# gau-nernst/llama-x

Hardware: AMD Instinct MI355X
Metric: train tokens/sec Llama-3.1-8B seq4096 at 1/2/4/8 MI355X; p50 step ms (higher is better)
Workload: dtype bf16; 1 GPU; Llama-3.1-8B text-only LoRA r=16 bf16, seq=4096, 1 sequence per GPU, causal mask, base+LM head frozen (BASELINE.json configs[1]); random-init weights at 8B dimensions; seq_len=4096, parallelism=dp1, launch=hipGraph replay (fwd+bwd+AdamW), lm_head_rows=labelled only

## Files before the change

include/llx.h:

```cpp
#ifndef LLX_H
#define LLX_H

#include <stdint.h>

#ifdef __cplusplus
extern "C" {
#endif

typedef void* llx_stream_t;

int llx_version(void);
const char* llx_last_error_string(void);
int llx_device_info(int device, char* name, int len);

int llx_rmsnorm_fwd(const void* x, const void* w, void* y, float* rstd, int64_t rows, int64_t dim, float eps, llx_stream_t s);
int llx_rmsnorm_fwd_quant(const void* x, const void* w, void* y, float* rstd, void* q, int64_t ldq, void* qscale, int64_t rows, int64_t dim,
                          float eps, llx_stream_t s);
int64_t llx_rmsnorm_bwd_workspace_bytes(int64_t rows, int64_t dim);
int llx_rmsnorm_bwd(const void* dy, const void* x, const void* w, const float* rstd, void* dx, void* dw ,
                    int dw_accumulate, void* workspace, const void* dres ,
                    int64_t rows, int64_t dim, llx_stream_t s);

int llx_gemm_nt_bf16(const void* A, int64_t lda, const void* B, int64_t ldb, void* C, int64_t ldc, int64_t M, int64_t N, int64_t K,
                     const void* A2, int64_t lda2, const void* B2, int64_t ldb2, int64_t K2, int epilogue, const void* E, int64_t lde,
                     llx_stream_t s);
int llx_gemm_nt_bf16_rows(const void* A, int64_t lda, const void* B, int64_t ldb, void* C, int64_t ldc, int64_t M, int64_t N, int64_t K,
                          const void* A2, int64_t lda2, const void* B2, int64_t ldb2, int64_t K2, int epilogue, const void* E, int64_t lde,
                          const int32_t* m_valid, llx_stream_t s);
int llx_gemm_nt_bf16_splitk(const void* A, int64_t lda, const void* B, int64_t ldb, float* partial, int64_t M, int64_t N, int64_t K, int splits,
                            const int32_t* m_valid, llx_stream_t s);
int llx_splitk_combine(const float* partial, int splits, int64_t M, int64_t N, const int32_t* inv, const float* scale, void* out, int64_t ld_out,
                       llx_stream_t s);
int llx_gemm_nt_bf16_rope(const void* A, int64_t lda, const void* B, int64_t ldb, void* C, int64_t ldc, int64_t M, int64_t N, int64_t K,
                          const void* A2, int64_t lda2, const void* B2, int64_t ldb2, int64_t K2, const float* rope_table, int64_t rope_S,
                          int64_t rope_cols, llx_stream_t s);

int llx_gemm_tn_bf16(const void* A, int64_t lda, const void* B, int64_t ldb, void* C, int64_t ldc, int64_t M, int64_t N1, int64_t N2,
                     llx_stream_t s);
int llx_gemm_tn_bf16_rows(const void* A, int64_t lda, const void* B, int64_t ldb, void* C, int64_t ldc, int64_t M, int64_t N1, int64_t N2,
                          const int32_t* m_valid, llx_stream_t s);

int llx_int8_mm_dequant(const void* A, int64_t lda, const void* B, int64_t ldb, void* C, int64_t ldc, int64_t M, int64_t N, int64_t K,
                        const void* a_scale, const void* b_scale, llx_stream_t s);
int llx_int8_mm_dequant_f32(const void* A, int64_t lda, const void* B, int64_t ldb, float* C, int64_t ldc, int64_t M, int64_t N, int64_t K,
                            const float* a_scale, const float* b_scale, llx_stream_t s);
int llx_int8_mm_dequant_ext(const void* A, int64_t lda, const void* B, int64_t ldb, void* C, int64_t ldc, int64_t M, int64_t N, int64_t K,
                            const void* a_scale, const void* b_scale, const void* A2, int64_t lda2, const void* B2, int64_t ldb2, int64_t K2,
                            int epilogue, const void* E, int64_t lde, const float* rope_table, int64_t rope_S, int64_t rope_cols,
                            llx_stream_t s);

int llx_quantize_int8_rowwise(const void* x, int64_t ldx, void* q, int64_t ldq, void* scale, int64_t rows, int64_t cols, int is_f32,
                              llx_stream_t s);

int64_t llx_attn_flags_bytes(int64_t B, int64_t S);
int llx_attn_tile_flags(const int* doc_ids, const int* prefix_len, void* flags, int64_t B, int64_t S, llx_stream_t s);
int llx_attn_fwd(const void* q, int64_t q_sb, int64_t q_ss, const void* k, int64_t k_sb, int64_t k_ss, const void* v, int64_t v_sb,
                 int64_t v_ss, void* o, int64_t o_sb, int64_t o_ss, float* lse, const int* doc_ids, const int* prefix_len,
                 const void* flags, int64_t B, int64_t S, int64_t H, int64_t KVH, int64_t head_dim, float scale, llx_stream_t s);
int64_t llx_attn_bwd_workspace_bytes(int64_t B, int64_t S, int64_t H, int64_t KVH);
int64_t llx_attn_bwd_ds_bytes(int64_t B, int64_t S, int64_t H);
int llx_attn_bwd(const void* q, int64_t q_sb, int64_t q_ss, const void* k, int64_t k_sb, int64_t k_ss, const void* v, int64_t v_sb,
                 int64_t v_ss, const void* o, int64_t o_sb, int64_t o_ss, const void* d_o, int64_t do_sb, int64_t do_ss, const float* lse,
                 float* delta , void* dq, int64_t dq_sb, int64_t dq_ss, void* dk, int64_t dk_sb, int64_t dk_ss,
                 void* dv, int64_t dv_sb, int64_t dv_ss, const int* doc_ids, const int* prefix_len, const void* flags,
                 const float* rope ,
                 void* ds ,
                 int64_t B, int64_t S, int64_t H, int64_t KVH, int64_t head_dim, float scale, llx_stream_t s);

int llx_attn_dense_fwd(const void* q, int64_t q_sb, int64_t q_sh, int64_t q_ss, const void* k, int64_t k_sb, int64_t k_sh, int64_t k_ss,
                       const void* v, int64_t v_sb, int64_t v_sh, int64_t v_ss, void* o, int64_t o_sb, int64_t o_sh, int64_t o_ss,
                       const void* mask, int64_t m_sb, int64_t m_sh, int64_t m_sq, int64_t B, int64_t H, int64_t KVH, int64_t Sq, int64_t Skv,
                       int64_t head_dim, float scale, llx_stream_t s);

int llx_gemv_bf16(const void* w0, int64_t ldw0, int64_t n0, const void* w1, int64_t ldw1, int64_t n1, const void* w2, int64_t ldw2, int64_t n2,
                  const void* x, int64_t ldx, int64_t M, int64_t K, const void* norm_w, float eps, int epilogue, void* out, int64_t ldo,
                  const void* res, int64_t ldr, const float* rope, int64_t n_q, int64_t n_k, void* k_cache, void* v_cache, int64_t c_sh,
                  int64_t c_ss, const int64_t* input_pos, const void* bext0, const void* bext1, const void* bext2, int64_t rank0, int64_t rank1,
                  int64_t rank2, const void* t, int64_t ldt, float lora_scale, llx_stream_t s);
int llx_mask_extent(const void* mask, int64_t row_stride, int64_t rows, int64_t Skv, int* extent, llx_stream_t s);
int llx_kv_scatter(const void* k, const void* v, int64_t s_sb, int64_t s_sh, int64_t s_ss, void* k_cache, void* v_cache, int64_t c_sb, int64_t c_sh,
                   int64_t c_ss, const int64_t* input_pos, int64_t B, int64_t KVH, int64_t L, int64_t Smax, int64_t head_dim, llx_stream_t s);
int64_t llx_attn_decode_workspace_bytes(int64_t B, int64_t H, int64_t M, int64_t nsplit);
int llx_attn_decode(const void* q, int64_t q_sb, int64_t q_sh, int64_t q_ss, const void* k_cache, const void* v_cache, int64_t c_sb, int64_t c_sh,
                    int64_t c_ss, void* o, int64_t o_sb, int64_t o_sh, int64_t o_ss, const void* mask, int64_t m_sb, int64_t m_sh, int64_t m_sq,
                    const int* extent, float* workspace, int64_t B, int64_t H, int64_t KVH, int64_t M, int64_t Skv, int64_t nsplit,
                    int64_t head_dim, float scale, llx_stream_t s);

int llx_rope(const void* x, int64_t x_sb, int64_t x_ss, void* y, int64_t y_sb, int64_t y_ss, const float* table, int64_t B, int64_t S,
             int64_t nheads, int64_t head_dim, int backward, llx_stream_t s);

int llx_swiglu_fwd(const void* g, int64_t g_ld, const void* u, int64_t u_ld, void* h, int64_t h_ld, int64_t rows, int64_t cols, llx_stream_t s);
int llx_swiglu_bwd(const void* dh, int64_t dh_ld, const void* g, int64_t g_ld, const void* u, int64_t u_ld, void* dg, int64_t dg_ld,
                   void* du, int64_t du_ld, int64_t rows, int64_t cols, llx_stream_t s);

int llx_embedding_fwd(const int64_t* ids, const void* table, void* out, int64_t n_tok, int64_t dim, int64_t vocab, int64_t tok_per_batch,
                      int64_t out_sb, int64_t out_ss, llx_stream_t s);
int llx_embedding_bwd(const int64_t* ids, const void* dy, float* dtable_f32, int64_t n_tok, int64_t dim, int64_t vocab,
                      int64_t tok_per_batch, int64_t dy_sb, int64_t dy_ss, llx_stream_t s);

int64_t llx_ce_workspace_bytes(int64_t T);
int llx_ce_fwd_bwd(const void* logits, int64_t ld, void* dlogits, int64_t dld, const int64_t* labels, float* loss, void* workspace,
                   int64_t T, int64_t V, llx_stream_t s);
int llx_head_compact_index(const int64_t* labels, int32_t* idx, int32_t* inv, int64_t* labels_c, int32_t* count, int64_t T, llx_stream_t s);
int llx_gather_rows(const void* src, int64_t ld_src, const int32_t* idx, const int32_t* count, void* dst, int64_t ld_dst, int64_t T, int64_t D,
                    llx_stream_t s);
int llx_scatter_rows(const void* src, int64_t ld_src, const int32_t* inv, const float* scale , void* dst, int64_t ld_dst,
                     int64_t T, int64_t D, llx_stream_t s);
int llx_ce_fwd_bwd_rows(const void* logits, int64_t ld, void* dlogits, int64_t dld, const int64_t* labels, float* loss, void* workspace,
                        int64_t T, int64_t V, const int32_t* rows, llx_stream_t s);
int llx_ce_fwd_bwd_part(const void* logits, int64_t ld, void* dlogits, int64_t dld, const int64_t* labels, float* loss, void* workspace, int64_t T,
                        int64_t V, int64_t row0, int64_t nrows, const int32_t* rows, int phase, llx_stream_t s);

int llx_skinny_nt(const void* X, int64_t ldx, const void* W, int64_t ldw, void* out, int64_t M, int64_t K, int64_t R,
                  const int32_t* kranges , llx_stream_t s);
int llx_skinny_nt_scaled(const void* X, int64_t ldx, const void* W, int64_t ldw, void* out, int64_t M, int64_t K, int64_t R,
                         const int32_t* kranges, const void* colscale, void* G, int64_t ldg, llx_stream_t s);
int llx_rmsnorm_skinny_nt(const void* x, const void* g, const void* W, int64_t ldw, void* y, float* rstd, void* t, int64_t M, int64_t D,
                          int64_t R, float eps, llx_stream_t s);
int64_t llx_skinny_tn_workspace_bytes(int64_t M, int64_t N, int64_t R);
int llx_skinny_tn(const void* U, const void* Y, int64_t ldy, void* out, int64_t out_ld, int64_t M, int64_t N, int64_t R, float scale,
                  int transpose_out, int accumulate, void* workspace,
                  const int32_t* segs , int seg_count, llx_stream_t s);
int llx_skinny_tn_partial(const void* U, const void* Y, int64_t ldy, int64_t M, int64_t N, int64_t R, void* workspace, const int32_t* segs,
                          int seg_count, llx_stream_t s);
int llx_skinny_tn_partial_many(int n, const void* const* U, const void* const* Y, const int64_t* ldy, const int64_t* M, const int64_t* N,
                               const int64_t* R, void* const* workspaces, const int32_t* const* segs, const int* seg_count, llx_stream_t s);
int64_t llx_skinny_u_workspace_bytes(int64_t M, int64_t N);
int llx_skinny_tn_partial_many_u(int n, const void* const* U, const void* const* Y, const int64_t* ldy, const int64_t* M, const int64_t* N,
                                 const int64_t* R, void* const* workspaces, const int32_t* const* segs, const int* seg_count,
                                 const void* const* Bt, const int64_t* ldb, void* const* upart, llx_stream_t s);
int llx_skinny_u_reduce(const void* upart, void* out, int64_t M, int64_t N, int64_t R, const int32_t* segs, int seg_count, llx_stream_t s);
int llx_skinny_tn_partial_many_us(int n, const void* const* U, const void* const* Y, const int64_t* ldy, const int64_t* M, const int64_t* N,
                                  const int64_t* R, void* const* workspaces, const int32_t* const* segs, const int* seg_count,
                                  const void* const* Bt, const int64_t* ldb, void* const* upart, const void* const* colscale,
                                  void* const* G, const int64_t* ldg, llx_stream_t s);
int llx_skinny_tn_reduce_many(int n, const void* const* workspaces, void* const* outs, const int64_t* out_ld, const int64_t* M, const int64_t* N,
                              const int64_t* R, const float* scale, const int* transpose_out, const int* accumulate,
                              const int32_t* const* segs, const int* seg_count, llx_stream_t s);
int llx_pad64(const void* in, int64_t ld, void* out, int64_t R, int64_t C, float scale, int transpose, llx_stream_t s);
int llx_lora_group_pack(const void* const* lora_a, const void* const* lora_b, const int64_t* Ns, const int64_t* ranks, int nm, int64_t K,
                        float scale, void* a_cat, void* b2, void* bT, void* a2t, llx_stream_t s);
int llx_lora_groups_pack(const void* const* lora_a, const void* const* lora_b, const int64_t* Ns, const int64_t* ranks, const int* nm,
                         const int64_t* K, const float* scale, void* const* a_cat, void* const* b2, void* const* bT, void* const* a2t, int ng,
                         llx_stream_t s);
int llx_lora_pack(const void* in, int64_t ld, void* out, int64_t out_ld, int64_t R, int64_t C, int64_t row_off, int64_t col_off, float scale,
                  int transpose, llx_stream_t s);

int llx_rownorm2(const void* W, int64_t ld, float* out, int64_t rows, int64_t cols, llx_stream_t s);
int llx_dora_colscale(const float* wn2, const void* G , const void* b2 , const void* AAt ,
                      const void* m , void* c , float* inv_norm , int64_t N, int64_t R, llx_stream_t s);
int64_t llx_colsum_mul_workspace_bytes(int64_t N);
int llx_colsum_mul(const void* a, int64_t lda, const void* b, int64_t ldb, const float* colscale , void* out ,
                   void* workspace, int64_t M, int64_t N, llx_stream_t s);
int llx_colscale_bias(const void* x, int64_t x_ld, void* y, int64_t y_ld, const void* colscale , const void* bias ,
                      int64_t rows, int64_t cols, llx_stream_t s);

int llx_mel_spectrogram(const float* audio, int64_t B, int64_t L, const float* twiddle, const float* window, const float* fbank, float* mel,
                        int64_t n_frames, int64_t hop, int64_t n_mels, llx_stream_t s);
int llx_logmel_cmn(const float* mel, void* feat , int64_t B, int64_t n_frames, int64_t n_mels, llx_stream_t s);
int llx_gelu_fwd(const void* z, int64_t z_ld, void* y, int64_t y_ld, int64_t rows, int64_t cols, llx_stream_t s);
int llx_gelu_bwd(const void* dy, int64_t dy_ld, const void* z, int64_t z_ld, void* dz, int64_t dz_ld, int64_t rows, int64_t cols, llx_stream_t s);
int llx_col2im3(const void* dA, void* dpad, int64_t M, int64_t C, int64_t P, int64_t stride, llx_stream_t s);
int llx_conv_w_reorder(const void* in, void* out, int64_t D, int64_t C, int to_gemm, llx_stream_t s);

int llx_scale(const void* x, int64_t x_ld, void* y, int64_t y_ld, const float* dev_scalar, float host_scale, const void* colscale,
              int64_t rows, int64_t cols, llx_stream_t s);
int llx_add(const void* x, const void* y, void* z, int64_t n, llx_stream_t s);
int llx_transpose(const void* in, int64_t in_ld, void* out, int64_t out_ld, int64_t R, int64_t C, int src_is_i8, llx_stream_t s);
int llx_i8_to_bf16(const void* in, void* out, int64_t n, llx_stream_t s);

#ifdef __cplusplus
}
#endif
#endif
```

llama-x_amd/csrc/common.h:

```cpp
#pragma once
#include <hip/hip_runtime.h>
#include <stdint.h>
#include <stdarg.h>
#include <stdio.h>

#define LLX_OK 0
#define LLX_ERR_ARG -1
#define LLX_ERR_LAUNCH -2
#define LLX_ERR_UNSUPPORTED -3

void llx_set_error(const char* fmt, ...);

#define LLX_REQUIRE(cond, ...)            \
  do {                                    \
    if (!(cond)) {                        \
      llx_set_error(__VA_ARGS__);         \
      return LLX_ERR_ARG;                 \
    }                                     \
  } while (0)

#define LLX_LAUNCH_CHECK(name)                                              \
  do {                                                                      \
    hipError_t e__ = hipGetLastError();                                     \
    if (e__ != hipSuccess) {                                                \
      llx_set_error("%s: launch failed: %s", name, hipGetErrorString(e__)); \
      return LLX_ERR_LAUNCH;                                                \
    }                                                                       \
  } while (0)

typedef uint16_t bf16_t;

typedef __attribute__((ext_vector_type(8))) __bf16 bf16x8_t;
typedef __attribute__((ext_vector_type(4))) float f32x4_t;
typedef __attribute__((ext_vector_type(16))) float f32x16_t;
typedef __attribute__((ext_vector_type(4))) int i32x4_t;
typedef __attribute__((ext_vector_type(16))) int i32x16_t;
typedef __attribute__((ext_vector_type(4))) short s16x4_t;
typedef __attribute__((ext_vector_type(4))) uint32_t u32x4_t;
typedef __attribute__((ext_vector_type(2))) uint32_t u32x2_t;

#define LLX_WAVE 64

__device__ __forceinline__ float bf2f(bf16_t v) { return __uint_as_float(((uint32_t)v) << 16); }
__device__ __forceinline__ bf16_t f2bf(float f) {
  __bf16 b = (__bf16)f;
  return __builtin_bit_cast(bf16_t, b);
}
__device__ __forceinline__ uint32_t pack_bf2(float lo, float hi) {
  return (uint32_t)f2bf(lo) | ((uint32_t)f2bf(hi) << 16);
}
__device__ __forceinline__ float bflo(uint32_t w) { return __uint_as_float(w << 16); }
__device__ __forceinline__ float bfhi(uint32_t w) { return __uint_as_float(w & 0xffff0000u); }

__device__ __forceinline__ float wave_sum(float v) {
#pragma unroll
  for (int o = 32; o > 0; o >>= 1) v += __shfl_xor(v, o, 64);
  return v;
}
__device__ __forceinline__ float wave_max(float v) {
#pragma unroll
  for (int o = 32; o > 0; o >>= 1) v = fmaxf(v, __shfl_xor(v, o, 64));
  return v;
}

__device__ __forceinline__ float block_sum(float v, float* red) {
  v = wave_sum(v);
  const int lane = threadIdx.x & 63, w = threadIdx.x >> 6, nw = (blockDim.x + 63) >> 6;
  __syncthreads();
  if (lane == 0) red[w] = v;
  __syncthreads();
  float t = 0.f;
  for (int i = 0; i < nw; ++i) t += red[i];
  return t;
}
__device__ __forceinline__ float block_max(float v, float* red) {
  v = wave_max(v);
  const int lane = threadIdx.x & 63, w = threadIdx.x >> 6, nw = (blockDim.x + 63) >> 6;
  __syncthreads();
  if (lane == 0) red[w] = v;
  __syncthreads();
  float t = red[0];
  for (int i = 1; i < nw; ++i) t = fmaxf(t, red[i]);
  return t;
}

static inline int64_t cdiv64(int64_t a, int64_t b) { return (a + b - 1) / b; }

__device__ __forceinline__ float sigmoidf_(float x) { return __builtin_amdgcn_rcpf(1.f + __expf(-x)); }
__device__ __forceinline__ u32x4_t swiglu_fwd8(const u32x4_t& gv, const u32x4_t& uv) {
  u32x4_t o;
#pragma unroll
  for (int e = 0; e < 4; ++e) {
    const float g0 = bflo(gv[e]), g1 = bfhi(gv[e]);
    const float s0 = bf2f(f2bf(g0 * sigmoidf_(g0))), s1 = bf2f(f2bf(g1 * sigmoidf_(g1)));
    o[e] = pack_bf2(s0 * bflo(uv[e]), s1 * bfhi(uv[e]));
  }
  return o;
}
__device__ __forceinline__ void swiglu_bwd8(const u32x4_t& dv, const u32x4_t& gv, const u32x4_t& uv, u32x4_t& og, u32x4_t& ou) {
#pragma unroll
  for (int e = 0; e < 4; ++e) {
    float dgs[2], dus[2];
#pragma unroll
    for (int p = 0; p < 2; ++p) {
      const float gg = p ? bfhi(gv[e]) : bflo(gv[e]);
      const float uu = p ? bfhi(uv[e]) : bflo(uv[e]);
      const float dd = p ? bfhi(dv[e]) : bflo(dv[e]);
      const float sg = sigmoidf_(gg);
      const float silu = bf2f(f2bf(gg * sg));
      dus[p] = dd * silu;
      const float ds = bf2f(f2bf(dd * uu));
      dgs[p] = ds * (sg * (1.f + gg * (1.f - sg)));
    }
    og[e] = pack_bf2(dgs[0], dgs[1]);
    ou[e] = pack_bf2(dus[0], dus[1]);
  }
}

__device__ __forceinline__ u32x4_t rope8(const u32x4_t& v, const f32x4_t& t0, const f32x4_t& t1, float sign) {
  const float cs[4] = {t0[0], t0[2], t1[0], t1[2]};
  const float sn[4] = {t0[1] * sign, t0[3] * sign, t1[1] * sign, t1[3] * sign};
  u32x4_t o;
#pragma unroll
  for (int e = 0; e < 4; ++e) {
    const float x0 = bflo(v[e]), x1 = bfhi(v[e]);
    o[e] = pack_bf2(x0 * cs[e] - x1 * sn[e], x1 * cs[e] + x0 * sn[e]);
  }
  return o;
}

__device__ __forceinline__ u32x4_t rope8(const u32x4_t& v, const float* __restrict__ tp, float sign) {
  const f32x4_t t0 = *reinterpret_cast<const f32x4_t*>(tp);
  const f32x4_t t1 = *reinterpret_cast<const f32x4_t*>(tp + 4);
  const float cs[4] = {t0[0], t0[2], t1[0], t1[2]};
  const float sn[4] = {t0[1] * sign, t0[3] * sign, t1[1] * sign, t1[3] * sign};
  u32x4_t o;
#pragma unroll
  for (int e = 0; e < 4; ++e) {
    const float x0 = bflo(v[e]), x1 = bfhi(v[e]);
    o[e] = pack_bf2(x0 * cs[e] - x1 * sn[e], x1 * cs[e] + x0 * sn[e]);
  }
  return o;
}

typedef __attribute__((ext_vector_type(8))) short llx_s16x8_t;
template <int OFF>
__device__ __forceinline__ void lds_tr_read(s16x4_t& dst, uint32_t addr) {
  asm volatile("ds_read_b64_tr_b16 %0, %1 offset:%2" : "=v"(dst) : "v"(addr), "n"(OFF));
}
__device__ __forceinline__ void lds_tr_read_rt(s16x4_t& dst, uint32_t addr, int off) {
  asm volatile("ds_read_b64_tr_b16 %0, %1 offset:%2" : "=v"(dst) : "v"(addr), "n"(off));
}
template <int N>
__device__ __forceinline__ void lds_tr_wait4(s16x4_t& a, s16x4_t& b, s16x4_t& c, s16x4_t& d) {
  asm volatile("s_waitcnt lgkmcnt(%4)" : "+v"(a), "+v"(b), "+v"(c), "+v"(d) : "n"(N));
  __builtin_amdgcn_sched_barrier(0);
}
template <int N>
__device__ __forceinline__ void lds_tr_wait8(s16x4_t (&c)[4], s16x4_t (&d)[4]) {
  asm volatile("s_waitcnt lgkmcnt(%8)" : "+v"(c[0]), "+v"(c[1]), "+v"(c[2]), "+v"(c[3]), "+v"(d[0]), "+v"(d[1]), "+v"(d[2]), "+v"(d[3]) : "n"(N));
  __builtin_amdgcn_sched_barrier(0);
}
__device__ __forceinline__ bf16x8_t frag_of(const s16x4_t& lo, const s16x4_t& hi) {
  const llx_s16x8_t v = {lo[0], lo[1], lo[2], lo[3], hi[0], hi[1], hi[2], hi[3]};
  return __builtin_bit_cast(bf16x8_t, v);
}
```

llama-x_amd/csrc/rmsnorm.hip:

```cpp
#include "common.h"

template <int NCH, bool QUANT = false, bool FULL = false>
__global__ __launch_bounds__(256) void rmsnorm_fwd_kernel(const bf16_t* __restrict__ x, const bf16_t* __restrict__ w,
                                                          bf16_t* __restrict__ y, float* __restrict__ rstd_out,
                                                          int64_t rows, int dim, float eps, int8_t* __restrict__ q = nullptr,
                                                          int64_t ldq = 0, bf16_t* __restrict__ qscale = nullptr) {
  const int lane = threadIdx.x & 63;
  const int64_t row = (int64_t)blockIdx.x * 4 + (threadIdx.x >> 6);
  if (row >= rows) return;
  const bf16_t* xr = x + row * dim;
  u32x4_t v[NCH];
  float ss = 0.f;
#pragma unroll
  for (int c = 0; c < NCH; ++c) {
    const int col = c * 512 + lane * 8;
    if (FULL || col < dim) {
      v[c] = *reinterpret_cast<const u32x4_t*>(xr + col);
#pragma unroll
      for (int e = 0; e < 4; ++e) {
        float a = bflo(v[c][e]), b = bfhi(v[c][e]);
        ss += a * a + b * b;
      }
    }
  }
// ... 8 lines not shown
    if (FULL || col < dim) {
      u32x4_t wv = *reinterpret_cast<const u32x4_t*>(w + col);
      u32x4_t o;
#pragma unroll
      for (int e = 0; e < 4; ++e) {
        float a = bflo(v[c][e]) * rstd * bflo(wv[e]);
        float b = bfhi(v[c][e]) * rstd * bfhi(wv[e]);
        o[e] = pack_bf2(a, b);
        if constexpr (QUANT) amax = fmaxf(amax, fmaxf(fabsf(bflo(o[e])), fabsf(bfhi(o[e]))));
      }
      *reinterpret_cast<u32x4_t*>(yr + col) = o;
      if constexpr (QUANT) v[c] = o;
    }
  }
  if constexpr (QUANT) {
    amax = wave_max(amax);
    const float scale = amax / 127.0f;
    const float div = fmaxf(scale, 1e-12f);
    if (lane == 0) qscale[row] = f2bf(scale);
    int8_t* qr = q + row * ldq;
#pragma unroll
    for (int c = 0; c < NCH; ++c) {
      const int col = c * 512 + lane * 8;
      if (FULL || col < dim) {
        u32x2_t o = {0u, 0u};
#pragma unroll
        for (int e = 0; e < 4; ++e) {
          const int a = (int)rintf(bflo(v[c][e]) / div), b = (int)rintf(bfhi(v[c][e]) / div);
          o[e >> 1] |= ((uint32_t)(a & 0xff) | ((uint32_t)(b & 0xff) << 8)) << ((e & 1) * 16);
        }
        *reinterpret_cast<u32x2_t*>(qr + col) = o;
      }
    }
  }
}

template <int NCH, bool FULL = false, int RES = -1>
__global__ __launch_bounds__(256) void rmsnorm_bwd_kernel(const bf16_t* __restrict__ dy, const bf16_t* __restrict__ x,
                                                          const bf16_t* __restrict__ w, const float* __restrict__ rstd,
                                                          bf16_t* __restrict__ dx, float* __restrict__ dw_partial,
                                                          const bf16_t* __restrict__ dres, int64_t rows, int dim, int rows_per_block) {
  extern __shared__ __attribute__((aligned(16))) float dwsh[];
  const bool has_res = RES < 0 ? dres != nullptr : RES == 1;
  const int lane = threadIdx.x & 63, wave = threadIdx.x >> 6;
  u32x4_t wp[NCH];
  float dwacc[NCH][8];
#pragma unroll
  for (int c = 0; c < NCH; ++c) {
    const int col = c * 512 + lane * 8;
#pragma unroll
    for (int e = 0; e < 8; ++e) dwacc[c][e] = 0.f;
    wp[c] = u32x4_t{0u, 0u, 0u, 0u};
    if (FULL || col < dim) wp[c] = *reinterpret_cast<const u32x4_t*>(w + col);
  }
  const int64_t r0 = (int64_t)blockIdx.x * rows_per_block;
  const int64_t r_end = (r0 + rows_per_block < rows) ? r0 + rows_per_block : rows;
  constexpr bool PIPE = NCH <= 8;
  struct RowRegs { u32x4_t x[NCH], d[NCH], r[NCH]; float rs; };
  auto load_row = [&](RowRegs& R, int64_t row) {
    R.rs = rstd[row];
#pragma unroll
    for (int c = 0; c < NCH; ++c) {
      const int col = c * 512 + lane * 8;
      if (FULL || col < dim) {
        R.x[c] = *reinterpret_cast<const u32x4_t*>(x + row * dim + col);
        R.d[c] = *reinterpret_cast<const u32x4_t*>(dy + row * dim + col);
        if (has_res) R.r[c] = *reinterpret_cast<const u32x4_t*>(dres + row * dim + col);
      }
    }
  };
  auto process_row = [&](RowRegs& R, int64_t row) {
    const float rs = R.rs;
    float dot = 0.f;
#pragma unroll
    for (int c = 0; c < NCH; ++c) {
      const int col = c * 512 + lane * 8;
      if (FULL || col < dim) {
#pragma unroll
        for (int e = 0; e < 4; ++e) {
          const float x0 = bflo(R.x[c][e]) * rs, x1 = bfhi(R.x[c][e]) * rs;
          const float d0 = bflo(R.d[c][e]), d1 = bfhi(R.d[c][e]);
          dwacc[c][2 * e] += d0 * x0; dwacc[c][2 * e + 1] += d1 * x1;
          dot += d0 * bflo(wp[c][e]) * x0 + d1 * bfhi(wp[c][e]) * x1;
        }
      }
    }
    dot = wave_sum(dot);
    const float m = dot / (float)dim;
#pragma unroll
    for (int c = 0; c < NCH; ++c) {
      const int col = c * 512 + lane * 8;
      if (FULL || col < dim) {
        u32x4_t o;
        asm volatile("" : "+v"(R.x[c]), "+v"(R.d[c]));
#pragma unroll
        for (int e = 0; e < 4; ++e) {
          const float x0 = bflo(R.x[c][e]) * rs, x1 = bfhi(R.x[c][e]) * rs;
          float a = rs * (bflo(R.d[c][e]) * bflo(wp[c][e]) - x0 * m);
          float b = rs * (bfhi(R.d[c][e]) * bfhi(wp[c][e]) - x1 * m);
          if (has_res) {
            a = bf2f(f2bf(a)) + bflo(R.r[c][e]);
            b = bf2f(f2bf(b)) + bfhi(R.r[c][e]);
          }
          o[e] = pack_bf2(a, b);
        }
        *reinterpret_cast<u32x4_t*>(dx + row * dim + col) = o;
      }
    }
  };
  {
    RowRegs A;
    int64_t row = r0 + wave;
    if constexpr (PIPE) {
      RowRegs B;
      if (row < r_end) load_row(A, row);
      while (row < r_end) {
        const bool n1 = row + 4 < r_end;
        if (n1) load_row(B, row + 4);
        process_row(A, row);
        if (!n1) break;
        row += 4;
        const bool n2 = row + 4 < r_end;
        if (n2) load_row(A, row + 4);
        process_row(B, row);
        if (!n2) break;
        row += 4;
      }
    } else {
      for (; row < r_end; row += 4) { load_row(A, row); process_row(A, row); }
    }
  }
  if (dw_partial) {
    for (int wsel = 0; wsel < 4; ++wsel) {
      if (wave == wsel) {
#pragma unroll
        for (int c = 0; c < NCH; ++c) {
          const int col = c * 512 + lane * 8;
          if (FULL || col < dim) {
#pragma unroll
            for (int e = 0; e < 8; ++e) dwsh[col + e] = (wsel == 0 ? 0.f : dwsh[col + e]) + dwacc[c][e];
          }
        }
      }
      __syncthreads();
    }
    for (int col = threadIdx.x * 4; col < dim; col += 256 * 4)
      *reinterpret_cast<f32x4_t*>(dw_partial + (int64_t)blockIdx.x * dim + col) = *reinterpret_cast<const f32x4_t*>(dwsh + col);
  }
}

__global__ __launch_bounds__(256) void colsum_partials_kernel(const float* __restrict__ partial, bf16_t* __restrict__ out, int nparts, int dim,
                                                              int accumulate) {
  __shared__ float red[16][17];
  const int c = threadIdx.x & 15, grp = threadIdx.x >> 4;
  const int col = blockIdx.x * 16 + c;
  float s = 0.f;
  if (col < dim)
    for (int p = grp; p < nparts; p += 16) s += partial[(int64_t)p * dim + col];
  red[grp][c] = s;
  __syncthreads();
  if (grp == 0 && col < dim) {
    s = 0.f;
#pragma unroll
    for (int g = 0; g < 16; ++g) s += red[g][c];
    if (accumulate) s += bf2f(out[col]);
    out[col] = f2bf(s);
  }
}

extern "C" int llx_rmsnorm_fwd(const void* x, const void* w, void* y, float* rstd, int64_t rows, int64_t dim, float eps,
                               hipStream_t stream) {
  LLX_REQUIRE(x && w && y, "llx_rmsnorm_fwd: null pointer");
  LLX_REQUIRE(rows >= 0 && dim > 0 && dim % 8 == 0 && dim <= 8192, "llx_rmsnorm_fwd: dim=%lld must be a multiple of 8 and <= 8192",
              (long long)dim);
  if (rows == 0) return LLX_OK;
  const dim3 grid((unsigned)cdiv64(rows, 4)), block(256);
  const int nch = (int)cdiv64(dim, 512);
#define L(N) hipLaunchKernelGGL((rmsnorm_fwd_kernel<N, false>), grid, block, 0, stream, (const bf16_t*)x, (const bf16_t*)w, (bf16_t*)y, rstd, rows, (int)dim, eps, (int8_t*)nullptr, (int64_t)0, (bf16_t*)nullptr)
#define LF(N) hipLaunchKernelGGL((rmsnorm_fwd_kernel<N, false, true>), grid, block, 0, stream, (const bf16_t*)x, (const bf16_t*)w, (bf16_t*)y, rstd, rows, (int)dim, eps, (int8_t*)nullptr, (int64_t)0, (bf16_t*)nullptr)
  if (dim == 4096) LF(8); else if (dim == 2048) LF(4); else if (dim == 8192) LF(16);
  else if (nch <= 1) L(1); else if (nch <= 2) L(2); else if (nch <= 4) L(4); else if (nch <= 8) L(8); else L(16);
#undef LF
#undef L
  LLX_LAUNCH_CHECK("llx_rmsnorm_fwd");
  return LLX_OK;
}

extern "C" int llx_rmsnorm_fwd_quant(const void* x, const void* w, void* y, float* rstd, void* q, int64_t ldq, void* qscale, int64_t rows,
                                     int64_t dim, float eps, hipStream_t stream) {
  LLX_REQUIRE(x && w && y && q && qscale, "llx_rmsnorm_fwd_quant: null pointer");
  LLX_REQUIRE(rows >= 0 && dim > 0 && dim % 8 == 0 && dim <= 8192 && ldq % 8 == 0 && (uintptr_t)q % 8 == 0,
              "llx_rmsnorm_fwd_quant: dim=%lld must be a multiple of 8 and <= 8192, q rows 8-byte aligned", (long long)dim);
  if (rows == 0) return LLX_OK;
  const dim3 grid((unsigned)cdiv64(rows, 4)), block(256);
  const int nch = (int)cdiv64(dim, 512);
#define L(N) hipLaunchKernelGGL((rmsnorm_fwd_kernel<N, true>), grid, block, 0, stream, (const bf16_t*)x, (const bf16_t*)w, (bf16_t*)y, rstd, rows, (int)dim, eps, (int8_t*)q, ldq, (bf16_t*)qscale)
#define LF(N) hipLaunchKernelGGL((rmsnorm_fwd_kernel<N, true, true>), grid, block, 0, stream, (const bf16_t*)x, (const bf16_t*)w, (bf16_t*)y, rstd, rows, (int)dim, eps, (int8_t*)q, ldq, (bf16_t*)qscale)
  if (dim == 4096) LF(8); else if (dim == 2048) LF(4); else if (dim == 8192) LF(16);
  else if (nch <= 1) L(1); else if (nch <= 2) L(2); else if (nch <= 4) L(4); else if (nch <= 8) L(8); else L(16);
#undef LF
#undef L
  LLX_LAUNCH_CHECK("llx_rmsnorm_fwd_quant");
  return LLX_OK;
}

#ifndef RMS_BWD_RPB
#define RMS_BWD_RPB 16
#endif
extern "C" int64_t llx_rmsnorm_bwd_workspace_bytes(int64_t rows, int64_t dim) {
  const int64_t rpb = RMS_BWD_RPB;
  return cdiv64(rows, rpb) * dim * 4;
}

extern "C" int llx_rmsnorm_bwd(const void* dy, const void* x, const void* w, const float* rstd, void* dx, void* dw,
                               int dw_accumulate, void* workspace, const void* dres, int64_t rows, int64_t dim, hipStream_t stream) {
  LLX_REQUIRE(dy && x && w && rstd && dx, "llx_rmsnorm_bwd: null pointer");
  LLX_REQUIRE(dim > 0 && dim % 8 == 0 && dim <= 8192, "llx_rmsnorm_bwd: dim=%lld must be a multiple of 8 and <= 8192", (long long)dim);
  LLX_REQUIRE(!dw || workspace, "llx_rmsnorm_bwd: workspace required when dw is requested");
  if (rows == 0) return LLX_OK;
  const int rpb = RMS_BWD_RPB;
  const int nblk = (int)cdiv64(rows, rpb);
  const int nch = (int)cdiv64(dim, 512);
  float* part = dw ? (float*)workspace : nullptr;
  const size_t lds = dw ? (size_t)dim * 4 : 0;
#define L(N) hipLaunchKernelGGL(rmsnorm_bwd_kernel<N>, dim3(nblk), dim3(256), lds, stream, (const bf16_t*)dy, (const bf16_t*)x, (const bf16_t*)w, rstd, (bf16_t*)dx, part, (const bf16_t*)dres, rows, (int)dim, rpb)
#define LF(N) if (dres) LFR(N, 1); else LFR(N, 0)
#define LFR(N, R) hipLaunchKernelGGL((rmsnorm_bwd_kernel<N, true, R>), dim3(nblk), dim3(256), lds, stream, (const bf16_t*)dy, (const bf16_t*)x, (const bf16_t*)w, rstd, (bf16_t*)dx, part, (const bf16_t*)dres, rows, (int)dim, rpb)
  if (dim == 4096) { LF(8); } else if (dim == 2048) { LF(4); } else if (dim == 8192) { LF(16); }
  else if (nch <= 1) L(1); else if (nch <= 2) L(2); else if (nch <= 4) L(4); else if (nch <= 8) L(8); else L(16);
#undef LFR
#undef LF
#undef L
  LLX_LAUNCH_CHECK("llx_rmsnorm_bwd");
  if (dw) {
    hipLaunchKernelGGL(colsum_partials_kernel, dim3((unsigned)cdiv64(dim, 16)), dim3(256), 0, stream, part, (bf16_t*)dw, nblk,
                       (int)dim, dw_accumulate);
    LLX_LAUNCH_CHECK("llx_rmsnorm_bwd(colsum)");
  }
  return LLX_OK;
}
```

llama-x_amd/csrc/skinny.hip:

```cpp
#include "common.h"

typedef __attribute__((address_space(3))) s16x4_t lds_s16x4;
typedef __attribute__((ext_vector_type(8))) short s16x8_t;

#define SK_PAD 64

#define SNT_WAVES 8
#define SNT_UNROLL 8

struct SkinnyRanges { int lo[4], hi[4]; };

__device__ __forceinline__ void snt_scaled_store(const bf16x8_t& a, const bf16_t* cs, bf16_t* g) {
  const u32x4_t x = __builtin_bit_cast(u32x4_t, a);
  const u32x4_t c = *reinterpret_cast<const u32x4_t*>(cs);
  u32x4_t o;
#pragma unroll
  for (int e = 0; e < 4; ++e) o[e] = pack_bf2(bflo(x[e]) * bflo(c[e]), bfhi(x[e]) * bfhi(c[e]));
  *reinterpret_cast<u32x4_t*>(g) = o;
}

template <int NB, bool RANGED, bool SCALE = false>
__global__ __launch_bounds__(SNT_WAVES * 64) void skinny_nt_kernel(const bf16_t* __restrict__ X, int64_t ldx, const bf16_t* __restrict__ W,
                                                                   int64_t ldw, bf16_t* __restrict__ out, int M, int K, int R, SkinnyRanges kr,
                                                                   const bf16_t* __restrict__ cs = nullptr, bf16_t* __restrict__ G = nullptr,
// ... 101 lines not shown
  else { if (nb == 1) L(1, false); else if (nb == 2) L(2, false); else L(4, false); }
#undef L
  LLX_LAUNCH_CHECK("llx_skinny_nt");
  return LLX_OK;
}

extern "C" int llx_skinny_nt_scaled(const void* X, int64_t ldx, const void* W, int64_t ldw, void* out, int64_t M, int64_t K, int64_t R,
                                    const int32_t* kranges, const void* colscale, void* G, int64_t ldg, hipStream_t stream) {
  LLX_REQUIRE(X && W && out && colscale && G, "llx_skinny_nt_scaled: null pointer");
  LLX_REQUIRE(M > 0 && K > 0 && K % 32 == 0 && R > 0 && R <= 64, "llx_skinny_nt_scaled: need K%%32==0 and 0<R<=64 (K=%lld R=%lld)", (long long)K, (long long)R);
  LLX_REQUIRE(ldx % 8 == 0 && ldw % 8 == 0 && ldg % 8 == 0 && ((uintptr_t)X | (uintptr_t)W | (uintptr_t)colscale | (uintptr_t)G) % 16 == 0 && (uintptr_t)out % 8 == 0,
              "llx_skinny_nt_scaled: alignment");
  const dim3 grid((unsigned)cdiv64(M, 16)), block(SNT_WAVES * 64);
  const int nb = (int)cdiv64(R, 16);
  SkinnyRanges kr;
  for (int i = 0; i < 4; ++i) {
    kr.lo[i] = kranges ? kranges[2 * i] : 0;
    kr.hi[i] = kranges ? kranges[2 * i + 1] : (int)K;
    LLX_REQUIRE(kr.lo[i] % 64 == 0 && (kr.hi[i] % 64 == 0 || kr.hi[i] == (int)K) && kr.lo[i] >= 0 && kr.hi[i] <= (int)K,
                "llx_skinny_nt_scaled: k range %d of a block-diagonal W must be a multiple of 64 inside [0, K]", i);
  }
#define L(N, RG) hipLaunchKernelGGL((skinny_nt_kernel<N, RG, true>), grid, block, 0, stream, (const bf16_t*)X, ldx, (const bf16_t*)W, ldw, (bf16_t*)out, (int)M, (int)K, (int)R, kr, (const bf16_t*)colscale, (bf16_t*)G, ldg)
  if (kranges) { if (nb == 1) L(1, true); else if (nb == 2) L(2, true); else L(4, true); }
  else { if (nb == 1) L(1, false); else if (nb == 2) L(2, false); else L(4, false); }
#undef L
  LLX_LAUNCH_CHECK("llx_skinny_nt_scaled");
  return LLX_OK;
}

#define TN_NT 256
#define TN_MS 32
#define TN_YROW (TN_NT * 2 + 16)
#define TN_UROW (SK_PAD * 2 + 16)

__device__ __forceinline__ bf16x8_t tr16_frag(const char* tile, int rowbytes, int c0, int lane) {
  const int g = lane >> 4, i = lane & 15, q = i >> 2, p = i & 3;
  const char* base = tile + (8 * g + q) * rowbytes + (c0 + 4 * p) * 2;
  s16x4_t lo = __builtin_amdgcn_ds_read_tr16_b64_v4i16((lds_s16x4*)base);
  s16x4_t hi = __builtin_amdgcn_ds_read_tr16_b64_v4i16((lds_s16x4*)(base + 4 * rowbytes));
  s16x8_t v = {lo[0], lo[1], lo[2], lo[3], hi[0], hi[1], hi[2], hi[3]};
  return __builtin_bit_cast(bf16x8_t, v);
}

struct TnSegs { int n_lo[4], n_hi[4], r_lo[4], r_hi[4]; int64_t off[4]; int count; int rb_lo[4], rb_hi[4]; };

template <int NB>
__device__ __forceinline__ void skinny_tn_block(const bf16_t* __restrict__ U, const bf16_t* __restrict__ Y, int64_t ldy, float* __restrict__ partial,
                                                int M, int N, int rows_per_split, const TnSegs& sg, int ctile, int split, int nbl, char* sY, char* sU,
                                                const bf16_t* __restrict__ Bt = nullptr, int64_t ldb = 0, float* __restrict__ upart = nullptr, int brows = 0,
                                                const bf16_t* __restrict__ cs = nullptr, bf16_t* __restrict__ G = nullptr, int64_t ldg = 0) {
  const int tid = threadIdx.x, lane = tid & 63;
  const int wave = __builtin_amdgcn_readfirstlane(tid >> 6);
  const int n0 = ctile * TN_NT;
  const int m_begin = split * rows_per_split, m_end = min(M, m_begin + rows_per_split);
  const bool u_on = upart != nullptr && wave < nbl && n0 + TN_NT > sg.rb_lo[wave] && n0 < sg.rb_hi[wave];
  bf16x8_t ub[8];
  if (u_on) {
    const bf16_t* brow = Bt + (int64_t)min(wave * 16 + (lane & 15), brows - 1) * ldb;
#pragma unroll
    for (int ks = 0; ks < 8; ++ks) ub[ks] = *reinterpret_cast<const bf16x8_t*>(brow + min(n0 + ks * 32 + 8 * (lane >> 4), N - 8));
  }
  f32x4_t acc[NB][4];
#pragma unroll
  for (int rb = 0; rb < NB; ++rb)
#pragma unroll
    for (int cb = 0; cb < 4; ++cb) acc[rb][cb] = f32x4_t{0.f, 0.f, 0.f, 0.f};

  u32x4_t yv[2][4], uv[2];
  auto load_step = [&](int set, int ms) {
#pragma unroll
    for (int i = 0; i < 4; ++i) {
      const int q = i * 256 + tid;
      const int row = ms + (q >> 5), col = n0 + (q & 31) * 8;
      yv[set][i] = (row < m_end && col < N) ? *reinterpret_cast<const u32x4_t*>(Y + (int64_t)row * ldy + col) : u32x4_t{0u, 0u, 0u, 0u};
    }
    const int row = ms + (tid >> 3);
    uv[set] = (row < m_end) ? *reinterpret_cast<const u32x4_t*>(U + (int64_t)row * SK_PAD + (tid & 7) * 8) : u32x4_t{0u, 0u, 0u, 0u};
  };
  auto step = [&](int set, int ms) {
    __syncthreads();
#pragma unroll
    for (int i = 0; i < 4; ++i) {
      const int q = i * 256 + tid;
      *reinterpret_cast<u32x4_t*>(sY + (q >> 5) * TN_YROW + (q & 31) * 16) = yv[set][i];
      if (G) {
        const int row = ms + (q >> 5), col = n0 + (q & 31) * 8;
        if (row < m_end && col < N) {
          const u32x4_t c = *reinterpret_cast<const u32x4_t*>(cs + col);
          u32x4_t o;
#pragma unroll
          for (int e = 0; e < 4; ++e) o[e] = pack_bf2(bflo(yv[set][i][e]) * bflo(c[e]), bfhi(yv[set][i][e]) * bfhi(c[e]));
          *reinterpret_cast<u32x4_t*>(G + (int64_t)row * ldg + col) = o;
        }
      }
    }
    *reinterpret_cast<u32x4_t*>(sU + (tid >> 3) * TN_UROW + (tid & 7) * 16) = uv[set];
    __syncthreads();
    if (ms + 2 * TN_MS < m_end) load_step(set, ms + 2 * TN_MS);
    bf16x8_t a[NB];
#pragma unroll
    for (int rb = 0; rb < NB; ++rb) a[rb] = tr16_frag(sU, TN_UROW, rb * 16, lane);
#pragma unroll
    for (int cb = 0; cb < 4; ++cb) {
      const bf16x8_t b = tr16_frag(sY, TN_YROW, wave * 64 + cb * 16, lane);
#pragma unroll
      for (int rb = 0; rb < NB; ++rb)
        if (n0 + TN_NT > sg.rb_lo[rb] && n0 < sg.rb_hi[rb]) acc[rb][cb] = __builtin_amdgcn_mfma_f32_16x16x32_bf16(a[rb], b, acc[rb][cb], 0, 0, 0);
    }
    if (u_on) {
#pragma unroll
      for (int rf = 0; rf < 2; ++rf) {
        f32x4_t ua0 = {0.f, 0.f, 0.f, 0.f}, ua1 = {0.f, 0.f, 0.f, 0.f};
        const char* yrow = sY + (rf * 16 + (lane & 15)) * TN_YROW + (lane >> 4) * 16;
#pragma unroll
        for (int ks = 0; ks < 8; ks += 2) {
          ua0 = __builtin_amdgcn_mfma_f32_16x16x32_bf16(ub[ks], *reinterpret_cast<const bf16x8_t*>(yrow + ks * 64), ua0, 0, 0, 0);
          ua1 = __builtin_amdgcn_mfma_f32_16x16x32_bf16(ub[ks + 1], *reinterpret_cast<const bf16x8_t*>(yrow + (ks + 1) * 64), ua1, 0, 0, 0);
        }
        const int row = ms + rf * 16 + (lane & 15);
        if (row < m_end) {
#pragma unroll
          for (int e = 0; e < 4; ++e) upart[((int64_t)ctile * SK_PAD + wave * 16 + (lane >> 4) * 4 + e) * M + row] = ua0[e] + ua1[e];
        }
      }
    }
  };
  if (m_begin < m_end) load_step(0, m_begin);
  if (m_begin + TN_MS < m_end) load_step(1, m_begin + TN_MS);
  for (int ms = m_begin; ms < m_end; ms += 2 * TN_MS) {
    step(0, ms);
    if (ms + TN_MS < m_end) step(1, ms + TN_MS);
  }
  const int fr = lane & 15, fq = lane >> 4;
#pragma unroll
  for (int rb = 0; rb < NB; ++rb)
#pragma unroll
    for (int cb = 0; cb < 4; ++cb) {
      const int n = n0 + wave * 64 + cb * 16 + fr;
      if (n < N && n0 + TN_NT > sg.rb_lo[rb] && n0 < sg.rb_hi[rb]) {
#pragma unroll
        for (int e = 0; e < 4; ++e) partial[((int64_t)split * (nbl * 16) + rb * 16 + fq * 4 + e) * N + n] = acc[rb][cb][e];
      }
    }
}

template <int NB>
__global__ __launch_bounds__(256) void skinny_tn_kernel(const bf16_t* __restrict__ U, const bf16_t* __restrict__ Y, int64_t ldy,
                                                        float* __restrict__ partial, int M, int N, int rows_per_split, TnSegs sg) {
  __shared__ __attribute__((aligned(16))) char sY[TN_MS * TN_YROW];
  __shared__ __attribute__((aligned(16))) char sU[TN_MS * TN_UROW];
  skinny_tn_block<NB>(U, Y, ldy, partial, M, N, rows_per_split, sg, blockIdx.x, blockIdx.y, NB, sY, sU);
}

#define TN_MANY 4
struct TnPart { const bf16_t* U; const bf16_t* Y; int64_t ldy; float* partial; int M, N, rows_per_split, ctiles, nblocks, nbl; TnSegs sg;
                const bf16_t* Bt; int64_t ldb; float* upart; int brows; const bf16_t* cs; bf16_t* G; int64_t ldg; };
struct TnPartMany { TnPart d[TN_MANY]; int n; };

template <int NB>
__global__ __launch_bounds__(256) void skinny_tn_many_kernel(const TnPartMany m) {
  __shared__ __attribute__((aligned(16))) char sY[TN_MS * TN_YROW];
  __shared__ __attribute__((aligned(16))) char sU[TN_MS * TN_UROW];
  int b = blockIdx.x, i = 0;
  while (i < m.n - 1 && b >= m.d[i].nblocks) { b -= m.d[i].nblocks; ++i; }
  const TnPart& d = m.d[i];
  skinny_tn_block<NB>(d.U, d.Y, d.ldy, d.partial, d.M, d.N, d.rows_per_split, d.sg, b % d.ctiles, b / d.ctiles, d.nbl, sY, sU, d.Bt, d.ldb, d.upart, d.brows, d.cs, d.G, d.ldg);
}


static int tn_splits(int64_t M, int64_t N) {
  const int64_t ntiles = cdiv64(N, TN_NT);
  constexpr int target = 384;
  int64_t want = cdiv64(target, ntiles);
  const int64_t max_split = cdiv64(M, 4 * TN_MS);
  if (want > max_split) want = max_split;
  if (want < 1) want = 1;
  return (int)want;
}

extern "C" int64_t llx_skinny_tn_workspace_bytes(int64_t M, int64_t N, int64_t R) {
  return (int64_t)tn_splits(M, N) * cdiv64(R, 16) * 16 * N * 4;
}

static int tn_fill_segs(TnSegs& sg, const int32_t* segs, int seg_count, int64_t N, int64_t R, int64_t* total_out) {
  sg.count = 0;
  for (int rb = 0; rb < 4; ++rb) { sg.rb_lo[rb] = 0; sg.rb_hi[rb] = (int)N; }
  int64_t total = 0;
  if (segs) {
    LLX_REQUIRE(seg_count >= 1 && seg_count <= 4, "llx_skinny_tn: 1..4 segments");
    for (int rb = 0; rb < 4; ++rb) { sg.rb_lo[rb] = (int)N; sg.rb_hi[rb] = 0; }
    for (int i = 0; i < seg_count; ++i) {
      sg.n_lo[i] = segs[4 * i]; sg.n_hi[i] = segs[4 * i + 1]; sg.r_lo[i] = segs[4 * i + 2]; sg.r_hi[i] = segs[4 * i + 3];
      LLX_REQUIRE(sg.n_lo[i] >= 0 && sg.n_lo[i] < sg.n_hi[i] && sg.n_hi[i] <= N && sg.r_lo[i] >= 0 && sg.r_lo[i] < sg.r_hi[i] && sg.r_hi[i] <= R,
                  "llx_skinny_tn: bad segment %d", i);
      LLX_REQUIRE(sg.n_lo[i] % TN_NT == 0 && (sg.n_hi[i] % TN_NT == 0 || sg.n_hi[i] == N), "llx_skinny_tn: segment %d: n bounds must be multiples of 256", i);
      sg.off[i] = total;
      total += (int64_t)(sg.n_hi[i] - sg.n_lo[i]) * (sg.r_hi[i] - sg.r_lo[i]);
      for (int rb = sg.r_lo[i] / 16; rb <= (sg.r_hi[i] - 1) / 16; ++rb) {
        if (sg.n_lo[i] < sg.rb_lo[rb]) sg.rb_lo[rb] = sg.n_lo[i];
        if (sg.n_hi[i] > sg.rb_hi[rb]) sg.rb_hi[rb] = sg.n_hi[i];
      }
    }
    sg.count = seg_count;
  }
  *total_out = total;
  return LLX_OK;
}

extern "C" int llx_skinny_tn_partial(const void* U, const void* Y, int64_t ldy, int64_t M, int64_t N, int64_t R, void* workspace,
                                     const int32_t* segs, int seg_count, hipStream_t stream) {
  LLX_REQUIRE(U && Y && workspace, "llx_skinny_tn: null pointer");
  LLX_REQUIRE(M > 0 && N > 0 && N % 8 == 0 && R > 0 && R <= 64 && ldy % 8 == 0, "llx_skinny_tn: need N%%8==0, ldy%%8==0, 0<R<=64");
  LLX_REQUIRE(((uintptr_t)U | (uintptr_t)Y) % 16 == 0, "llx_skinny_tn: unaligned pointer");
  const int nsplit = tn_splits(M, N);
  int rows_per_split = (int)cdiv64(cdiv64(M, nsplit), TN_MS) * TN_MS;
  const int nb = (int)cdiv64(R, 16);
  TnSegs sg;
  int64_t total = 0;
  const int rc = tn_fill_segs(sg, segs, seg_count, N, R, &total);
  if (rc != LLX_OK) return rc;
  const dim3 grid((unsigned)cdiv64(N, TN_NT), (unsigned)nsplit), block(256);
#define L(NBV) hipLaunchKernelGGL(skinny_tn_kernel<NBV>, grid, block, 0, stream, (const bf16_t*)U, (const bf16_t*)Y, ldy, (float*)workspace, (int)M, (int)N, rows_per_split, sg)
  if (nb == 1) L(1); else if (nb == 2) L(2); else if (nb == 3) L(3); else L(4);
#undef L
  LLX_LAUNCH_CHECK("llx_skinny_tn");
  return LLX_OK;
}

extern "C" int llx_skinny_tn_partial_many_u(int n, const void* const* U, const void* const* Y, const int64_t* ldy, const int64_t* M, const int64_t* N,
                                            const int64_t* R, void* const* workspaces, const int32_t* const* segs, const int* seg_count,
                                            const void* const* Bt, const int64_t* ldb, void* const* upart, hipStream_t stream);
extern "C" int llx_skinny_tn_partial_many(int n, const void* const* U, const void* const* Y, const int64_t* ldy, const int64_t* M, const int64_t* N,
                                          const int64_t* R, void* const* workspaces, const int32_t* const* segs, const int* seg_count,
                                          hipStream_t stream) {
  return llx_skinny_tn_partial_many_u(n, U, Y, ldy, M, N, R, workspaces, segs, seg_count, nullptr, nullptr, nullptr, stream);
}
extern "C" int64_t llx_skinny_u_workspace_bytes(int64_t M, int64_t N) { return cdiv64(N, TN_NT) * M * SK_PAD * 4; }
extern "C" int llx_skinny_tn_partial_many_us(int n, const void* const* U, const void* const* Y, const int64_t* ldy, const int64_t* M, const int64_t* N,
                                             const int64_t* R, void* const* workspaces, const int32_t* const* segs, const int* seg_count,
                                             const void* const* Bt, const int64_t* ldb, void* const* upart, const void* const* colscale,
                                             void* const* G, const int64_t* ldg, hipStream_t stream);
extern "C" int llx_skinny_tn_partial_many_u(int n, const void* const* U, const void* const* Y, const int64_t* ldy, const int64_t* M, const int64_t* N,
                                            const int64_t* R, void* const* workspaces, const int32_t* const* segs, const int* seg_count,
                                            const void* const* Bt, const int64_t* ldb, void* const* upart, hipStream_t stream) {
  return llx_skinny_tn_partial_many_us(n, U, Y, ldy, M, N, R, workspaces, segs, seg_count, Bt, ldb, upart, nullptr, nullptr, nullptr, stream);
}
extern "C" int llx_skinny_tn_partial_many_us(int n, const void* const* U, const void* const* Y, const int64_t* ldy, const int64_t* M, const int64_t* N,
                                             const int64_t* R, void* const* workspaces, const int32_t* const* segs, const int* seg_count,
                                             const void* const* Bt, const int64_t* ldb, void* const* upart, const void* const* colscale,
                                             void* const* G, const int64_t* ldg, hipStream_t stream) {
  LLX_REQUIRE(n >= 1 && n <= TN_MANY && U && Y && ldy && M && N && R && workspaces && segs && seg_count, "llx_skinny_tn_partial_many: bad arguments (1..4 products)");
  TnPartMany m;
  m.n = n;
  int total_blocks = 0;
  for (int i = 0; i < n; ++i) {
    TnPart& d = m.d[i];
    LLX_REQUIRE(U[i] && Y[i] && workspaces[i], "llx_skinny_tn_partial_many: null pointer (product %d)", i);
    LLX_REQUIRE(M[i] > 0 && N[i] > 0 && N[i] % 8 == 0 && R[i] > 0 && R[i] <= 64 && ldy[i] % 8 == 0, "llx_skinny_tn_partial_many: need N%%8==0, ldy%%8==0, 0<R<=64 (product %d)", i);
    LLX_REQUIRE(((uintptr_t)U[i] | (uintptr_t)Y[i]) % 16 == 0, "llx_skinny_tn_partial_many: unaligned pointer (product %d)", i);
    const int nsplit = tn_splits(M[i], N[i]);
    d.U = (const bf16_t*)U[i]; d.Y = (const bf16_t*)Y[i]; d.ldy = ldy[i]; d.partial = (float*)workspaces[i];
    d.M = (int)M[i]; d.N = (int)N[i];
    d.rows_per_split = (int)cdiv64(cdiv64(M[i], nsplit), TN_MS) * TN_MS;
    d.ctiles = (int)cdiv64(N[i], TN_NT);
    d.nblocks = d.ctiles * nsplit;
    d.nbl = (int)cdiv64(R[i], 16);
    int64_t total = 0;
    const int rc = tn_fill_segs(d.sg, segs[i], seg_count[i], N[i], R[i], &total);
    if (rc != LLX_OK) return rc;
    for (int rb = d.nbl; rb < 4; ++rb) { d.sg.rb_lo[rb] = d.N; d.sg.rb_hi[rb] = 0; }
    d.Bt = nullptr; d.ldb = 0; d.upart = nullptr; d.brows = (int)R[i];
    if (upart && upart[i]) {
      LLX_REQUIRE(Bt && ldb && Bt[i] && ldb[i] % 8 == 0 && (uintptr_t)Bt[i] % 16 == 0 && N[i] >= 8, "llx_skinny_tn_partial_many_u: Bt of product %d", i);
      d.Bt = (const bf16_t*)Bt[i]; d.ldb = ldb[i]; d.upart = (float*)upart[i];
    }
    d.cs = nullptr; d.G = nullptr; d.ldg = 0;
    if (G && G[i]) {
      LLX_REQUIRE(colscale && ldg && colscale[i] && ldg[i] % 8 == 0 && ((uintptr_t)colscale[i] | (uintptr_t)G[i]) % 16 == 0, "llx_skinny_tn_partial_many_us: scaled copy of product %d", i);
      d.cs = (const bf16_t*)colscale[i]; d.G = (bf16_t*)G[i]; d.ldg = ldg[i];
    }
    total_blocks += d.nblocks;
  }
  int nbmax = 1;
  for (int i = 0; i < n; ++i) nbmax = m.d[i].nbl > nbmax ? m.d[i].nbl : nbmax;
  const dim3 grid((unsigned)total_blocks), block(256);
  if (nbmax == 1) hipLaunchKernelGGL(skinny_tn_many_kernel<1>, grid, block, 0, stream, m);
  else if (nbmax == 2) hipLaunchKernelGGL(skinny_tn_many_kernel<2>, grid, block, 0, stream, m);
  else if (nbmax == 3) hipLaunchKernelGGL(skinny_tn_many_kernel<3>, grid, block, 0, stream, m);
  else hipLaunchKernelGGL(skinny_tn_many_kernel<4>, grid, block, 0, stream, m);
  LLX_LAUNCH_CHECK("llx_skinny_tn_partial_many");
  return LLX_OK;
}

__global__ __launch_bounds__(256) void skinny_u_reduce_kernel(const float* __restrict__ upart, bf16_t* __restrict__ out, int M, int R, TnSegs sg) {
  __shared__ float tile[4][65];
  const int m0 = blockIdx.x * 64, ml = threadIdx.x & 63, cl = threadIdx.x >> 6;
  const int c = blockIdx.y * 4 + cl;
  float sum = 0.f;
  if (c < R) {
    const int rb = c >> 4;
    const int t_lo = sg.rb_lo[rb] / TN_NT, t_hi = (sg.rb_hi[rb] + TN_NT - 1) / TN_NT;
    const int64_t stride = (int64_t)SK_PAD * M;
    const float* src = upart + (int64_t)c * M + min(m0 + ml, M - 1);
    int t = t_lo;
    for (; t + 8 <= t_hi; t += 8) {
      float v[8];
#pragma unroll
      for (int j = 0; j < 8; ++j) v[j] = src[(t + j) * stride];
#pragma unroll
      for (int j = 0; j < 8; ++j) sum += v[j];
    }
    for (; t < t_hi; ++t) sum += src[t * stride];
  }
  tile[cl][ml] = sum;
  __syncthreads();
  if (threadIdx.x < 64 && m0 + threadIdx.x < M) {
    u32x2_t pk;
    pk[0] = pack_bf2(tile[0][threadIdx.x], tile[1][threadIdx.x]);
    pk[1] = pack_bf2(tile[2][threadIdx.x], tile[3][threadIdx.x]);
    *reinterpret_cast<u32x2_t*>(out + (int64_t)(m0 + threadIdx.x) * SK_PAD + blockIdx.y * 4) = pk;
  }
}

extern "C" int llx_skinny_u_reduce(const void* upart, void* out, int64_t M, int64_t N, int64_t R, const int32_t* segs, int seg_count, hipStream_t stream) {
  LLX_REQUIRE(upart && out && M > 0 && N > 0 && R > 0 && R <= 64, "llx_skinny_u_reduce: bad arguments");
  TnSegs sg;
  int64_t total = 0;
  const int rc = tn_fill_segs(sg, segs, seg_count, N, R, &total);
  if (rc != LLX_OK) return rc;
  hipLaunchKernelGGL(skinny_u_reduce_kernel, dim3((unsigned)cdiv64(M, 64), SK_PAD / 4), dim3(256), 0, stream, (const float*)upart, (bf16_t*)out, (int)M, (int)R, sg);
  LLX_LAUNCH_CHECK("llx_skinny_u_reduce");
  return LLX_OK;
}

struct TnRed { const float* partial; bf16_t* out; int64_t out_ld, total; int nsplit, RP, R, N, transpose_out, accumulate, use_segs; float scale; TnSegs sg; };
struct TnRedMany { TnRed d[TN_MANY]; };

__global__ void skinny_tn_reduce_many_kernel(const TnRedMany m) {
  const TnRed& d = m.d[blockIdx.y];
  int64_t idx = (int64_t)blockIdx.x * blockDim.x + threadIdx.x;
  if (idx >= d.total) return;
  int r, n;
  bf16_t* dst;
  if (d.use_segs) {
    int s = 0;
    for (; s < d.sg.count; ++s) {
      const int64_t cnt = (int64_t)(d.sg.n_hi[s] - d.sg.n_lo[s]) * (d.sg.r_hi[s] - d.sg.r_lo[s]);
      if (idx < cnt) break;
      idx -= cnt;
    }
    if (s >= d.sg.count) return;
    const int rw = d.sg.r_hi[s] - d.sg.r_lo[s];
    n = d.sg.n_lo[s] + (int)(idx / rw);
    r = d.sg.r_lo[s] + (int)(idx % rw);
    dst = d.out + d.sg.off[s] + idx;
  } else {
    r = (int)(idx / d.N);
    n = (int)(idx % d.N);
    dst = d.transpose_out ? d.out + (int64_t)n * d.out_ld + r : d.out + (int64_t)r * d.out_ld + n;
  }
  float sum = 0.f;
  const float* src = d.partial + (int64_t)r * d.N + n;
  const int64_t stride = (int64_t)d.RP * d.N;
  int p = 0;
  for (; p + 8 <= d.nsplit; p += 8) {
    float v[8];
#pragma unroll
    for (int j = 0; j < 8; ++j) v[j] = src[(p + j) * stride];
#pragma unroll
    for (int j = 0; j < 8; ++j) sum += v[j];
  }
  if (p + 4 <= d.nsplit) {
    float v[4];
#pragma unroll
    for (int j = 0; j < 4; ++j) v[j] = src[(p + j) * stride];
#pragma unroll
    for (int j = 0; j < 4; ++j) sum += v[j];
    p += 4;
  }
  for (; p < d.nsplit; ++p) sum += src[p * stride];
  sum *= d.scale;
  if (d.accumulate) sum += bf2f(*dst);
  *dst = f2bf(sum);
}

extern "C" int llx_skinny_tn_reduce_many(int n, const void* const* workspaces, void* const* outs, const int64_t* out_ld, const int64_t* M,
                                         const int64_t* N, const int64_t* R, const float* scale, const int* transpose_out, const int* accumulate,
                                         const int32_t* const* segs, const int* seg_count, hipStream_t stream) {
  LLX_REQUIRE(n >= 1 && n <= TN_MANY && workspaces && outs && out_ld && M && N && R && scale && transpose_out && accumulate && segs && seg_count,
              "llx_skinny_tn_reduce_many: bad arguments (1..4 products)");
  TnRedMany m;
  int64_t most = 0;
  for (int i = 0; i < n; ++i) {
    TnRed& d = m.d[i];
    LLX_REQUIRE(workspaces[i] && outs[i] && M[i] > 0 && N[i] > 0 && R[i] > 0 && R[i] <= 64, "llx_skinny_tn_reduce_many: bad product %d", i);
    d.partial = (const float*)workspaces[i]; d.out = (bf16_t*)outs[i]; d.out_ld = out_ld[i];
    d.nsplit = tn_splits(M[i], N[i]); d.RP = (int)cdiv64(R[i], 16) * 16; d.R = (int)R[i]; d.N = (int)N[i];
    d.transpose_out = transpose_out[i]; d.accumulate = accumulate[i]; d.scale = scale[i];
    d.use_segs = segs[i] != nullptr;
    int64_t total = 0;
    const int rc = tn_fill_segs(d.sg, segs[i], seg_count[i], N[i], R[i], &total);
    if (rc != LLX_OK) return rc;
    d.total = d.use_segs ? total : R[i] * N[i];
    if (d.total > most) most = d.total;
  }
  hipLaunchKernelGGL(skinny_tn_reduce_many_kernel, dim3((unsigned)cdiv64(most, 256), (unsigned)n), dim3(256), 0, stream, m);
  LLX_LAUNCH_CHECK("llx_skinny_tn_reduce_many");
  return LLX_OK;
}

extern "C" int llx_skinny_tn(const void* U, const void* Y, int64_t ldy, void* out, int64_t out_ld, int64_t M, int64_t N, int64_t R,
                             float scale, int transpose_out, int accumulate, void* workspace, const int32_t* segs, int seg_count,
                             hipStream_t stream) {
  LLX_REQUIRE(out, "llx_skinny_tn: null pointer");
  int rc = llx_skinny_tn_partial(U, Y, ldy, M, N, R, workspace, segs, seg_count, stream);
  if (rc != LLX_OK) return rc;
  const void* ws[1] = {workspace};
  void* outs[1] = {out};
  return llx_skinny_tn_reduce_many(1, ws, outs, &out_ld, &M, &N, &R, &scale, &transpose_out, &accumulate, &segs, &seg_count, stream);
}

#define RSN_MAXPAIRS 8

template <int NB>
__global__ __launch_bounds__(SNT_WAVES * 64) void rmsnorm_skinny_nt_kernel(const bf16_t* __restrict__ X, const bf16_t* __restrict__ G,
                                                                           const bf16_t* __restrict__ W, int64_t ldw, bf16_t* __restrict__ Y,
                                                                           float* __restrict__ rstd_out, bf16_t* __restrict__ T, int M, int D,
                                                                           int R, float eps) {
  __shared__ float part[SNT_WAVES][16][SK_PAD];
  __shared__ float ssq[SNT_WAVES][16];
  const int lane = threadIdx.x & 63, wave = threadIdx.x >> 6;
  const int m0 = blockIdx.x * 16;
  const int fr = lane & 15, fq = lane >> 4;
  const int row = min(m0 + fr, M - 1);
  const int npw = D / (SNT_WAVES * 64);
  const bf16_t* xrow = X + (int64_t)row * D + wave * npw * 64 + 16 * fq;
  bf16x8_t a[RSN_MAXPAIRS][2];
  float ss = 0.f;
#pragma unroll
  for (int p = 0; p < RSN_MAXPAIRS; ++p) {
    if (p < npw) {
#pragma unroll
      for (int h = 0; h < 2; ++h) {
        a[p][h] = *reinterpret_cast<const bf16x8_t*>(xrow + p * 64 + 8 * h);
#pragma unroll
        for (int j = 0; j < 8; ++j) {
          const float v = (float)a[p][h][j];
          ss += v * v;
        }
      }
    }
  }
  const bf16_t* grow = G + wave * npw * 64 + 16 * fq;
  const bf16_t* wrow[NB];
#pragma unroll
  for (int nb = 0; nb < NB; ++nb) wrow[nb] = W + (int64_t)min(nb * 16 + fr, R - 1) * ldw + wave * npw * 64 + 16 * fq;
  bf16x8_t gv[RSN_MAXPAIRS][2];
#pragma unroll
  for (int p = 0; p < RSN_MAXPAIRS; ++p)
    if (p < npw) {
#pragma unroll
      for (int h = 0; h < 2; ++h) gv[p][h] = *reinterpret_cast<const bf16x8_t*>(grow + p * 64 + 8 * h);
    }
  constexpr int RSN_PRE = NB >= 3 ? 2 : 4;
  bf16x8_t bpre[RSN_PRE][2][NB];
#pragma unroll
  for (int p = 0; p < RSN_PRE; ++p)
    if (p < npw) {
#pragma unroll
      for (int h = 0; h < 2; ++h)
#pragma unroll
        for (int nb = 0; nb < NB; ++nb) bpre[p][h][nb] = *reinterpret_cast<const bf16x8_t*>(wrow[nb] + p * 64 + 8 * h);
    }
  ss += __shfl_xor(ss, 16, 64);
  ss += __shfl_xor(ss, 32, 64);
  if (fq == 0) ssq[wave][fr] = ss;
  __syncthreads();
  float tot = 0.f;
#pragma unroll
  for (int w = 0; w < SNT_WAVES; ++w) tot += ssq[w][fr];
  const float rstd = rsqrtf(tot / (float)D + eps);
  if (wave == 0 && fq == 0 && m0 + fr < M && rstd_out) rstd_out[m0 + fr] = rstd;
  bf16_t* yrow = Y + (int64_t)row * D + wave * npw * 64 + 16 * fq;
  f32x4_t acc[NB];
#pragma unroll
  for (int nb = 0; nb < NB; ++nb) acc[nb] = f32x4_t{0.f, 0.f, 0.f, 0.f};
#pragma unroll
  for (int p = 0; p < RSN_MAXPAIRS; ++p) {
    if (p < npw) {
#pragma unroll
      for (int h = 0; h < 2; ++h) {
        bf16x8_t y;
#pragma unroll
        for (int j = 0; j < 8; ++j) y[j] = (__bf16)((float)a[p][h][j] * rstd * (float)gv[p][h][j]);
        if (m0 + fr < M) *reinterpret_cast<bf16x8_t*>(yrow + p * 64 + 8 * h) = y;
#pragma unroll
        for (int nb = 0; nb < NB; ++nb) {
          bf16x8_t b;
          if (p < RSN_PRE) b = bpre[p < RSN_PRE ? p : 0][h][nb];
          else b = *reinterpret_cast<const bf16x8_t*>(wrow[nb] + p * 64 + 8 * h);
          acc[nb] = __builtin_amdgcn_mfma_f32_16x16x32_bf16(y, b, acc[nb], 0, 0, 0);
        }
      }
    }
  }
#pragma unroll
  for (int nb = 0; nb < NB; ++nb)
#pragma unroll
    for (int e = 0; e < 4; ++e) part[wave][fq * 4 + e][nb * 16 + fr] = acc[nb][e];
  __syncthreads();
  const int orow = threadIdx.x >> 5, c0 = (threadIdx.x & 31) * 2;
  if (m0 + orow < M) {
    float v[2];
#pragma unroll
    for (int e = 0; e < 2; ++e) {
      const int c = c0 + e;
      float s = 0.f;
      if (c < NB * 16 && c < R) {
#pragma unroll
        for (int w = 0; w < SNT_WAVES; ++w) s += part[w][orow][c];
      }
      v[e] = s;
    }
    *reinterpret_cast<uint32_t*>(T + (int64_t)(m0 + orow) * SK_PAD + c0) = pack_bf2(v[0], v[1]);
  }
}

extern "C" int llx_rmsnorm_skinny_nt(const void* x, const void* g, const void* W, int64_t ldw, void* y, float* rstd, void* t, int64_t M,
                                     int64_t D, int64_t R, float eps, hipStream_t stream) {
  LLX_REQUIRE(x && g && W && y && t, "llx_rmsnorm_skinny_nt: null pointer");
  LLX_REQUIRE(M > 0 && D > 0 && D % (SNT_WAVES * 64) == 0 && D <= SNT_WAVES * 64 * RSN_MAXPAIRS && R > 0 && R <= 64,
              "llx_rmsnorm_skinny_nt: need D a multiple of 512 and <= 4096, 0 < R <= 64 (D=%lld R=%lld)", (long long)D, (long long)R);
  LLX_REQUIRE(ldw % 8 == 0 && ((uintptr_t)x | (uintptr_t)g | (uintptr_t)W | (uintptr_t)y) % 16 == 0 && (uintptr_t)t % 8 == 0, "llx_rmsnorm_skinny_nt: alignment");
  const dim3 grid((unsigned)cdiv64(M, 16)), block(SNT_WAVES * 64);
  const int nb = (int)cdiv64(R, 16);
#define L(N) hipLaunchKernelGGL((rmsnorm_skinny_nt_kernel<N>), grid, block, 0, stream, (const bf16_t*)x, (const bf16_t*)g, (const bf16_t*)W, ldw, (bf16_t*)y, rstd, (bf16_t*)t, (int)M, (int)D, (int)R, eps)
  if (nb == 1) L(1); else if (nb == 2) L(2); else if (nb == 3) L(3); else L(4);
#undef L
  LLX_LAUNCH_CHECK("llx_rmsnorm_skinny_nt");
  return LLX_OK;
}
```

llama-x_amd/llx/_lib.py:

```python
from __future__ import annotations

import ctypes
import os
from ctypes import c_char_p, c_float, c_int, c_int64, c_void_p

import torch

_HERE = os.path.dirname(os.path.abspath(__file__))
LIB_PATH = os.environ.get("LLX_LIB_PATH") or os.path.join(_HERE, "libllx_hip.so")

_lib = None

_P, _I, _L, _F = c_void_p, c_int, c_int64, c_float
SIGNATURES: dict[str, tuple] = {
    "llx_version": (c_int, []),
    "llx_last_error_string": (c_char_p, []),
    "llx_device_info": (c_int, [c_int, c_char_p, c_int]),
    "llx_rmsnorm_fwd": (c_int, [_P, _P, _P, _P, _L, _L, _F, _P]),
    "llx_rmsnorm_fwd_quant": (c_int, [_P, _P, _P, _P, _P, _L, _P, _L, _L, _F, _P]),
    "llx_rmsnorm_bwd_workspace_bytes": (c_int64, [_L, _L]),
    "llx_rmsnorm_bwd": (c_int, [_P, _P, _P, _P, _P, _P, _I, _P, _P, _L, _L, _P]),
    "llx_attn_flags_bytes": (c_int64, [_L, _L]),
    "llx_attn_tile_flags": (c_int, [_P, _P, _P, _L, _L, _P]),
    "llx_attn_fwd": (c_int, [_P, _L, _L, _P, _L, _L, _P, _L, _L, _P, _L, _L, _P, _P, _P, _P, _L, _L, _L, _L, _L, _F, _P]),
    "llx_attn_dense_fwd": (c_int, [_P, _L, _L, _L, _P, _L, _L, _L, _P, _L, _L, _L, _P, _L, _L, _L, _P, _L, _L, _L, _L, _L, _L, _L, _L, _L, _F, _P]),
    "llx_gemv_bf16": (c_int, [_P, _L, _L, _P, _L, _L, _P, _L, _L, _P, _L, _L, _L, _P, _F, _I, _P, _L, _P, _L, _P, _L, _L, _P, _P, _L, _L, _P,
                              _P, _P, _P, _L, _L, _L, _P, _L, _F, _P]),
    "llx_mask_extent": (c_int, [_P, _L, _L, _L, _P, _P]),
    "llx_kv_scatter": (c_int, [_P, _P, _L, _L, _L, _P, _P, _L, _L, _L, _P, _L, _L, _L, _L, _L, _P]),
    "llx_attn_decode_workspace_bytes": (c_int64, [_L, _L, _L, _L]),
    "llx_attn_decode": (c_int, [_P, _L, _L, _L, _P, _P, _L, _L, _L, _P, _L, _L, _L, _P, _L, _L, _L, _P, _P, _L, _L, _L, _L, _L, _L, _L, _F, _P]),
    "llx_attn_bwd_workspace_bytes": (c_int64, [_L, _L, _L, _L]),
    "llx_attn_bwd_ds_bytes": (c_int64, [_L, _L, _L]),
    "llx_attn_bwd": (c_int, [_P, _L, _L, _P, _L, _L, _P, _L, _L, _P, _L, _L, _P, _L, _L, _P, _P, _P, _L, _L, _P, _L, _L, _P, _L, _L,
                             _P, _P, _P, _P, _P, _L, _L, _L, _L, _L, _F, _P]),
    "llx_embedding_fwd": (c_int, [_P, _P, _P, _L, _L, _L, _L, _L, _L, _P]),
    "llx_embedding_bwd": (c_int, [_P, _P, _P, _L, _L, _L, _L, _L, _L, _P]),
    "llx_rope": (c_int, [_P, _L, _L, _P, _L, _L, _P, _L, _L, _L, _L, _I, _P]),
    "llx_swiglu_fwd": (c_int, [_P, _L, _P, _L, _P, _L, _L, _L, _P]),
    "llx_swiglu_bwd": (c_int, [_P, _L, _P, _L, _P, _L, _P, _L, _P, _L, _L, _L, _P]),
    "llx_scale": (c_int, [_P, _L, _P, _L, _P, _F, _P, _L, _L, _P]),
    "llx_add": (c_int, [_P, _P, _P, _L, _P]),
    "llx_transpose": (c_int, [_P, _L, _P, _L, _L, _L, _I, _P]),
    "llx_i8_to_bf16": (c_int, [_P, _P, _L, _P]),
    "llx_quantize_int8_rowwise": (c_int, [_P, _L, _P, _L, _P, _L, _L, _I, _P]),
    "llx_int8_mm_dequant": (c_int, [_P, _L, _P, _L, _P, _L, _L, _L, _L, _P, _P, _P]),
    "llx_int8_mm_dequant_f32": (c_int, [_P, _L, _P, _L, _P, _L, _L, _L, _L, _P, _P, _P]),
    "llx_int8_mm_dequant_ext": (c_int, [_P, _L, _P, _L, _P, _L, _L, _L, _L, _P, _P, _P, _L, _P, _L, _L, _I, _P, _L, _P, _L, _L, _P]),
    "llx_mel_spectrogram": (c_int, [_P, _L, _L, _P, _P, _P, _P, _L, _L, _L, _P]),
    "llx_logmel_cmn": (c_int, [_P, _P, _L, _L, _L, _P]),
    "llx_gelu_fwd": (c_int, [_P, _L, _P, _L, _L, _L, _P]),
    "llx_gelu_bwd": (c_int, [_P, _L, _P, _L, _P, _L, _L, _L, _P]),
    "llx_col2im3": (c_int, [_P, _P, _L, _L, _L, _L, _P]),
    "llx_conv_w_reorder": (c_int, [_P, _P, _L, _L, _I, _P]),
    "llx_lora_group_pack": (c_int, [_P, _P, _P, _P, _I, _L, _F, _P, _P, _P, _P, _P]),
    "llx_lora_groups_pack": (c_int, [_P, _P, _P, _P, _P, _P, _P, _P, _P, _P, _P, _I, _P]),
    "llx_lora_pack": (c_int, [_P, _L, _P, _L, _L, _L, _L, _L, _F, _I, _P]),
    "llx_pad64": (c_int, [_P, _L, _P, _L, _L, _F, _I, _P]),
    "llx_rownorm2": (c_int, [_P, _L, _P, _L, _L, _P]),
    "llx_dora_colscale": (c_int, [_P, _P, _P, _P, _P, _P, _P, _L, _L, _P]),
    "llx_colsum_mul_workspace_bytes": (c_int64, [_L]),
    "llx_colsum_mul": (c_int, [_P, _L, _P, _L, _P, _P, _P, _L, _L, _P]),
    "llx_colscale_bias": (c_int, [_P, _L, _P, _L, _P, _P, _L, _L, _P]),
    "llx_ce_workspace_bytes": (c_int64, [_L]),
    "llx_ce_fwd_bwd": (c_int, [_P, _L, _P, _L, _P, _P, _P, _L, _L, _P]),
    "llx_ce_fwd_bwd_rows": (c_int, [_P, _L, _P, _L, _P, _P, _P, _L, _L, _P, _P]),
    "llx_ce_fwd_bwd_part": (c_int, [_P, _L, _P, _L, _P, _P, _P, _L, _L, _L, _L, _P, _I, _P]),
    "llx_head_compact_index": (c_int, [_P, _P, _P, _P, _P, _L, _P]),
    "llx_gather_rows": (c_int, [_P, _L, _P, _P, _P, _L, _L, _L, _P]),
    "llx_scatter_rows": (c_int, [_P, _L, _P, _P, _P, _L, _L, _L, _P]),
    "llx_skinny_nt": (c_int, [_P, _L, _P, _L, _P, _L, _L, _L, _P, _P]),
    "llx_skinny_nt_scaled": (c_int, [_P, _L, _P, _L, _P, _L, _L, _L, _P, _P, _P, _L, _P]),
    "llx_rmsnorm_skinny_nt": (c_int, [_P, _P, _P, _L, _P, _P, _P, _L, _L, _L, _F, _P]),
    "llx_skinny_tn_workspace_bytes": (c_int64, [_L, _L, _L]),
    "llx_skinny_tn": (c_int, [_P, _P, _L, _P, _L, _L, _L, _L, _F, _I, _I, _P, _P, _I, _P]),
    "llx_skinny_tn_partial": (c_int, [_P, _P, _L, _L, _L, _L, _P, _P, _I, _P]),
    "llx_skinny_tn_partial_many": (c_int, [_I, _P, _P, _P, _P, _P, _P, _P, _P, _P, _P]),
    "llx_skinny_u_workspace_bytes": (_L, [_L, _L]),
    "llx_skinny_tn_partial_many_u": (c_int, [_I, _P, _P, _P, _P, _P, _P, _P, _P, _P, _P, _P, _P, _P]),
    "llx_skinny_u_reduce": (c_int, [_P, _P, _L, _L, _L, _P, _I, _P]),
    "llx_skinny_tn_partial_many_us": (c_int, [_I, _P, _P, _P, _P, _P, _P, _P, _P, _P, _P, _P, _P, _P, _P, _P, _P]),
    "llx_skinny_tn_reduce_many": (c_int, [_I, _P, _P, _P, _P, _P, _P, _P, _P, _P, _P, _P, _P]),
    "llx_gemm_nt_bf16": (c_int, [_P, _L, _P, _L, _P, _L, _L, _L, _L, _P, _L, _P, _L, _L, _I, _P, _L, _P]),
    "llx_gemm_nt_bf16_splitk": (c_int, [_P, _L, _P, _L, _P, _L, _L, _L, _I, _P, _P]),
    "llx_splitk_combine": (c_int, [_P, _I, _L, _L, _P, _P, _P, _L, _P]),
    "llx_gemm_nt_bf16_rows": (c_int, [_P, _L, _P, _L, _P, _L, _L, _L, _L, _P, _L, _P, _L, _L, _I, _P, _L, _P, _P]),
    "llx_gemm_tn_bf16": (c_int, [_P, _L, _P, _L, _P, _L, _L, _L, _L, _P]),
    "llx_gemm_tn_bf16_rows": (c_int, [_P, _L, _P, _L, _P, _L, _L, _L, _L, _P, _P]),
    "llx_gemm_nt_bf16_rope": (c_int, [_P, _L, _P, _L, _P, _L, _L, _L, _L, _P, _L, _P, _L, _L, _P, _L, _L, _P]),
}

DEBUG_SIGNATURES: dict[str, tuple] = {
    "llx_debug_attn_fwd_occupancy": (c_int, []),
    "llx_debug_attn_bwd_set_stamps": (c_int, [_P]),
    "llx_debug_attn_fwd_stamps": (c_int, [_P, _P, _P, _P, _L, _L, _L, _P, _P]),
}


class LlxError(RuntimeError):
    pass


def load():
    global _lib
    if _lib is not None:
        return _lib
    if not os.path.exists(LIB_PATH):
        raise LlxError(
            f"{LIB_PATH} is missing: build it with `python -c 'import __graft_entry__ as g; g.build()'` "
            "(or `make -C llama-x_amd/csrc`). There is no fallback path."
        )
    lib = ctypes.CDLL(LIB_PATH)
    for name, (res, args) in {**SIGNATURES, **DEBUG_SIGNATURES}.items():
        fn = getattr(lib, name)
        fn.restype = res
        fn.argtypes = args
    _lib = lib
    return lib


def check(rc: int, what: str = ""):
    if rc != 0:
        msg = load().llx_last_error_string()
        raise LlxError(f"{what} failed (code {rc}): {msg.decode() if msg else '?'}")


_raw_stream = getattr(torch._C, "_cuda_getCurrentRawStream", None)


def stream() -> c_void_p:
    if _raw_stream is not None:
        return c_void_p(_raw_stream(torch.cuda.current_device()))
    return c_void_p(torch.cuda.current_stream().cuda_stream)


def ptr(t) -> c_void_p:
    if t is None:
        return c_void_p(0)
    return c_void_p(t.data_ptr())


def require_cuda(*tensors):
    for t in tensors:
        if t is not None and not t.is_cuda:
            raise LlxError("llx ops run on the HIP device only (tensor on %s); there is no CPU path" % t.device)
```

llama-x_amd/llx/dp.py:

```python
from __future__ import annotations

import torch
import torch.distributed as dist
from torch import nn


class GradBuckets:
    def __init__(self, model: nn.Module, n_buckets: int = 4, process_group=None, force: bool = False, overlap: bool = True,
                 groups: "list[list[nn.Parameter]] | None" = None):
        self.pg = process_group
        self.world = dist.get_world_size(process_group) if dist.is_initialized() else 1
        self.active = self.world > 1 or force
        self.arena = getattr(model, "_llx_arena", None)
        params = [p for p in model.parameters() if p.requires_grad]
        self._params = params
        if not self.active:
            self.buckets, self._handles, self._hooks, self.sync_enabled, self.hook_launches = [], [], [], True, 0
            self.group_of_bucket = []
            return
        self.buckets: list[dict] = []
        self.group_of_bucket: list[int] = []
        if groups is not None:
            seen = {id(p) for g in groups for p in g}
            assert seen == {id(p) for p in params}, "groups must cover exactly the trainable parameters"
            for gi, g in enumerate(groups):
                by_kind: dict = {}
                for p in g:
                    by_kind.setdefault((p.dtype, self._in_arena(p)), []).append(p)
                for ps in by_kind.values():
                    self.buckets.append(self._make(ps))
                    self.group_of_bucket.append(gi)
        else:
            params = list(reversed(params))
            total = sum(p.numel() for p in params)
            target = (total + n_buckets - 1) // max(1, n_buckets)
            cur, cur_n = [], 0
            for p in params:
                if cur and (p.dtype != cur[0].dtype or self._in_arena(p) != self._in_arena(cur[0])
                            or (cur_n + p.numel() > target and len(self.buckets) < n_buckets - 1)):
                    self.buckets.append(self._make(cur))
                    cur, cur_n = [], 0
                cur.append(p)
                cur_n += p.numel()
            if cur:
                self.buckets.append(self._make(cur))
        self._handles = []
        self._hooks = []
        self.hook_launches = 0
        if overlap:
            for bi, b in enumerate(self.buckets):
                for p in b["params"]:
                    self._hooks.append(p.register_post_accumulate_grad_hook(self._make_hook(bi)))
        self.sync_enabled = True

    def _in_arena(self, p) -> bool:
        return self.arena is not None and self.arena.contains(p)

    def _make(self, params):
        dtype, device = params[0].dtype, params[0].device
        assert all(p.dtype == dtype for p in params), "a bucket holds one dtype"
        if self._in_arena(params[0]):
            flats = self.arena.ranges(params)
            return {"params": params, "flat": flats[0], "flats": flats, "pending": len(params), "arena": True}
        flat = torch.zeros(sum(p.numel() for p in params), dtype=dtype, device=device)
        off = 0
        for p in params:
            p.grad = flat[off : off + p.numel()].view_as(p)
            off += p.numel()
        return {"params": params, "flat": flat, "flats": [flat], "pending": len(params), "arena": False}

    def _make_hook(self, bi: int):
        def hook(param):
            if not self.sync_enabled:
                return
            b = self.buckets[bi]
            b["pending"] -= 1
            if b["pending"] == 0 and not (b["flat"].is_cuda and torch.cuda.is_current_stream_capturing()):
                self.hook_launches += 1
                self._launch(b)

        return hook

    def prescale(self, b):
        if not b.get("scaled"):
            if b["arena"]:
                self.arena.settle(b["params"])
            if self.world > 1:
                for f in b["flats"]:
                    f.div_(self.world)
        b["scaled"] = True

    def _launch(self, b):
        b["launched"] = True
        self.prescale(b)
        if dist.is_initialized():
            for f in b["flats"]:
                self._handles.append(dist.all_reduce(f, op=dist.ReduceOp.SUM, group=self.pg, async_op=True))

    def launch_group(self, gi: int):
        if not (self.active and self.sync_enabled):
            return
        for b, g in zip(self.buckets, self.group_of_bucket):
            if g == gi and not b.get("launched"):
                self._launch(b)

    def finish(self):
        if self.active and self.sync_enabled:
            for b in self.buckets:
                if not b.get("launched"):
                    self._launch(b)
        elif self.arena is not None and not self.active:
            self.arena.settle()
        for h in self._handles:
            h.wait()
        self._handles.clear()
        for b in self.buckets:
            b["pending"] = len(b["params"])
            b["launched"] = False
            b["scaled"] = False

    def zero_grad(self):
        if not self.active:
            for p in self._params:
                p.grad = None
            return
        for b in self.buckets:
            if b["arena"]:
                for p in b["params"]:
                    p.grad = None
            else:
                b["flat"].zero_()


class StagedStep:

    def __init__(self, model: nn.Module, stages, stage_params, optim, *, graph: bool = True, process_group=None, force: bool = False):
        self.stages, self.optim, self.use_graph = list(stages), optim, graph
        groups = [list(ps) for ps in reversed(list(stage_params))]
        self.buckets = GradBuckets(model, groups=groups, process_group=process_group, force=force, overlap=False)
        self.n = len(self.stages)
        self._graphs = None

    def _forward(self, inputs):
        self._ins, self._outs = [], []
        h = self.stages[0](*inputs)
        self._outs.append(h)
        for st in self.stages[1:]:
            hin = h.detach().requires_grad_(h.requires_grad)
            self._ins.append(hin)
            h = st(hin)
            self._outs.append(h)
        return h

    def _backward_stage(self, i: int):
        out = self._outs[i]
        if i == self.n - 1:
            out.backward()
        elif out.requires_grad:
            out.backward(self._ins[i].grad)
        if self.buckets.active:
            for b, g in zip(self.buckets.buckets, self.buckets.group_of_bucket):
                if g == self.n - 1 - i:
                    self.buckets.prescale(b)

    def _eager(self, inputs):
        self.buckets.zero_grad()
        loss = self._forward(inputs)
        for i in reversed(range(self.n)):
            self._backward_stage(i)
            self.buckets.launch_group(self.n - 1 - i)
        self.buckets.finish()
        self.optim.step()
        return loss.detach()

    def capture(self, *static_inputs):
        if not self.use_graph:
            return
        side = torch.cuda.Stream()
        side.wait_stream(torch.cuda.current_stream())
        with torch.cuda.stream(side):
            for _ in range(2):
                self._eager(static_inputs)
        torch.cuda.current_stream().wait_stream(side)
        kw = dict(capture_error_mode="thread_local")
        gf = torch.cuda.CUDAGraph()
        with torch.cuda.graph(gf, **kw):
            self.buckets.zero_grad()
            self._loss = self._forward(static_inputs)
        pool = gf.pool()
        gb = []
        for i in reversed(range(self.n)):
            for b in self.buckets.buckets:
                b["scaled"] = False
            g = torch.cuda.CUDAGraph()
            with torch.cuda.graph(g, pool=pool, **kw):
                self._backward_stage(i)
            gb.append(g)
        go = torch.cuda.CUDAGraph()
        with torch.cuda.graph(go, pool=pool, **kw):
            self.optim.step()
        self._graphs = (gf, gb, go)

    def __call__(self, *inputs):
        if self._graphs is None:
            return self._eager(inputs)
        gf, gb, go = self._graphs
        gf.replay()
        for k, g in enumerate(gb):
            g.replay()
            for b, gi in zip(self.buckets.buckets, self.buckets.group_of_bucket):
                if gi == k:
                    b["scaled"] = True
            self.buckets.launch_group(k)
        self.buckets.finish()
        go.replay()
        return self._loss


def llama_stages(model, n_stages: int, *, labels, block_mask=None, audio=None):
    L = len(model.layers)
    n_stages = max(1, min(n_stages, L))
    bounds = [round(i * L / n_stages) for i in range(n_stages + 1)]
    state = {}

    def first(tokens):
        x, n_drop = model._embed(tokens, audio) if audio is not None else model._embed(tokens)
        state["rope"], state["drop"] = model.rope[: x.shape[1]], n_drop
        x = model._run_layers(x, state["rope"], bounds[0], bounds[1], block_mask=block_mask)
        return head(x) if n_stages == 1 else x

    def head(x):
        if state["drop"]:
            x = x[:, state["drop"] :]
        return model._head(x, labels)

    def middle(lo, hi, last):
        def run(x):
# ... 18 lines not shown
```

llama-x_amd/llx/kernels.py:

```python
from __future__ import annotations

import ctypes
import math
import os
from dataclasses import dataclass
from typing import Optional, Sequence

import torch
from torch import Tensor

from . import _lib as L

BF16 = torch.bfloat16
EPI_NONE, EPI_RESIDUAL, EPI_BIAS, EPI_BIAS_GELU, EPI_COLSCALE = 0, 1, 2, 3, 4
EPI_SWIGLU_BWD = 6
EPI_SWIGLU_FWD = 7
SK_PAD = 64
GEMM_TRACE = None
ATTN_TRACE = None


def _lib():
    return L.load()


def gemm_kernel_launches(M: int, N: int, epilogue: int) -> int:
    gm, gn = -(-M // 256), -(-N // 256)
    tail = (gm * gn) % 256
    split = epilogue != EPI_SWIGLU_FWD and N % 256 == 0 and gm * gn > 256 and 0 < tail <= 128 and tail % gm == 0
    return 2 if split else 1


def _rows2d(x: Tensor) -> Tensor:
    if x.dim() == 2:
        return x if x.stride(1) == 1 else x.contiguous()
    y = x.reshape(-1, x.shape[-1])
    return y if y.stride(1) == 1 else y.contiguous()


def _chk_bf16(*ts):
    for t in ts:
        if t is not None:
            assert t.dtype is BF16, f"llx kernels compute in bf16 (got {t.dtype})"
    L.require_cuda(*ts)


def rmsnorm_fwd(x: Tensor, w: Tensor, eps: float, quant: bool = False):
    _chk_bf16(x, w)
    x2 = _rows2d(x)
    assert x2.stride(0) == x2.shape[1], "rmsnorm input rows must be dense"
    rows, dim = x2.shape
    assert w.shape == (dim,) and w.is_contiguous()
    y = torch.empty_like(x2)
    rstd = torch.empty(rows, device=x.device, dtype=torch.float32)
    if quant:
        q = torch.empty(rows, dim, device=x.device, dtype=torch.int8)
        qs = torch.empty(rows, device=x.device, dtype=BF16)
        L.check(_lib().llx_rmsnorm_fwd_quant(L.ptr(x2), L.ptr(w), L.ptr(y), L.ptr(rstd), L.ptr(q), dim, L.ptr(qs), rows, dim, eps, L.stream()),
                "llx_rmsnorm_fwd_quant")
        return y.view(x.shape), rstd, q, qs
    L.check(_lib().llx_rmsnorm_fwd(L.ptr(x2), L.ptr(w), L.ptr(y), L.ptr(rstd), rows, dim, eps, L.stream()), "llx_rmsnorm_fwd")
    return y.view(x.shape), rstd


def rmsnorm_skinny_ok(dim: int) -> bool:
    return dim % 512 == 0 and dim <= 4096


def rmsnorm_skinny_nt(x: Tensor, w: Tensor, eps: float, a_cat: Tensor) -> tuple[Tensor, Tensor, Tensor]:
    _chk_bf16(x, w, a_cat)
    x2 = _rows2d(x)
    rows, dim = x2.shape
    assert x2.stride(0) == dim and w.shape == (dim,) and w.is_contiguous() and rmsnorm_skinny_ok(dim)
    assert a_cat.dim() == 2 and a_cat.shape[1] == dim and a_cat.stride(1) == 1 and a_cat.shape[0] <= SK_PAD
    y = torch.empty_like(x2)
    rstd = torch.empty(rows, device=x.device, dtype=torch.float32)
    t = torch.empty(rows, SK_PAD, device=x.device, dtype=BF16)
    L.check(_lib().llx_rmsnorm_skinny_nt(L.ptr(x2), L.ptr(w), L.ptr(a_cat), a_cat.stride(0), L.ptr(y), L.ptr(rstd), L.ptr(t), rows, dim,
                                         a_cat.shape[0], eps, L.stream()), "llx_rmsnorm_skinny_nt")
    return y.view(x.shape), rstd, t


def rmsnorm_bwd(dy: Tensor, x: Tensor, w: Tensor, rstd: Tensor, need_dw: bool, dres: Optional[Tensor] = None,
                dw_out: Optional[Tensor] = None) -> tuple[Tensor, Optional[Tensor]]:
    _chk_bf16(dy, x, w, dres)
    x2, dy2 = _rows2d(x), _rows2d(dy)
    if dy2.stride(0) != dy2.shape[1]:
        dy2 = dy2.contiguous()
    rows, dim = x2.shape
    dx = torch.empty_like(x2)
    dw = ws = None
    if need_dw:
        dw = dw_out if dw_out is not None else torch.empty(dim, device=x.device, dtype=BF16)
        assert dw.shape == (dim,) and dw.is_contiguous() and dw.dtype is BF16
        ws = torch.empty(_lib().llx_rmsnorm_bwd_workspace_bytes(rows, dim), device=x.device, dtype=torch.uint8)
    if dres is not None:
        dres = _rows2d(dres)
        assert dres.shape == x2.shape and dres.stride(0) == dim
    L.check(_lib().llx_rmsnorm_bwd(L.ptr(dy2), L.ptr(x2), L.ptr(w), L.ptr(rstd), L.ptr(dx), L.ptr(dw), 0, L.ptr(ws), L.ptr(dres), rows, dim,
                                   L.stream()), "llx_rmsnorm_bwd")
    return dx.view(x.shape), dw


def gemm_nt(a: Tensor, b: Tensor, *, out: Optional[Tensor] = None, a2: Optional[Tensor] = None, b2: Optional[Tensor] = None,
            epilogue: int = EPI_NONE, e: Optional[Tensor] = None, rope: Optional[tuple[Tensor, int, int]] = None,
            k2_eff: Optional[float] = None, m_valid: Optional[Tensor] = None, m_expect: Optional[float] = None) -> Tensor:
    _chk_bf16(a, b, a2, b2, e, out)
    assert a.dim() == 2 and b.dim() == 2 and a.shape[1] == b.shape[1], (a.shape, b.shape)
    assert a.stride(1) == 1 and b.stride(1) == 1
    M, K = a.shape
    N = b.shape[0]
    if epilogue == EPI_SWIGLU_BWD:
        assert out is not None and e is not None and out.shape == (M, 2 * N) and e.shape == (M, 2 * N) and out.stride(1) == 1 and e.stride(1) == 1
    else:
        if out is None:
            out = torch.empty(M, N, device=a.device, dtype=BF16)
        assert out.shape == (M, N) and out.stride(1) == 1
    K2 = 0
    if a2 is not None:
        assert b2 is not None and a2.shape[0] == M and b2.shape[0] == N and a2.shape[1] == b2.shape[1]
        assert a2.stride(1) == 1 and b2.stride(1) == 1
        K2 = a2.shape[1]
    lde = 0
    if epilogue == EPI_RESIDUAL:
        assert e is not None and e.shape == (M, N) and e.stride(1) == 1
        lde = e.stride(0)
    elif epilogue == EPI_SWIGLU_BWD:
        lde = e.stride(0)
    elif epilogue == EPI_SWIGLU_FWD:
        assert e is not None and N % 256 == 0 and e.shape == (M, N // 2) and e.stride(1) == 1
        lde = e.stride(0)
    elif epilogue != EPI_NONE:
        assert e is not None and e.shape == (N,) and e.is_contiguous()
    ev = None
    if GEMM_TRACE is not None:
        ev = (torch.cuda.Event(enable_timing=True), torch.cuda.Event(enable_timing=True))
        ev[0].record()
    if rope is not None:
        table, rs, rc = rope
        assert epilogue == EPI_NONE and table.dtype is torch.float32 and table.is_contiguous() and table.shape[0] >= rs and table.shape[1:] == (64, 2)
        L.check(_lib().llx_gemm_nt_bf16_rope(L.ptr(a), a.stride(0), L.ptr(b), b.stride(0), L.ptr(out), out.stride(0), M, N, K,
                                             L.ptr(a2), a2.stride(0) if a2 is not None else 0, L.ptr(b2), b2.stride(0) if b2 is not None else 0, K2,
                                             L.ptr(table), rs, rc, L.stream()), "llx_gemm_nt_bf16_rope")
    elif m_valid is not None:
        assert m_valid.dtype is torch.int32 and m_valid.numel() == 1 and m_valid.device == a.device
        L.check(_lib().llx_gemm_nt_bf16_rows(L.ptr(a), a.stride(0), L.ptr(b), b.stride(0), L.ptr(out), out.stride(0), M, N, K,
                                             L.ptr(a2), a2.stride(0) if a2 is not None else 0, L.ptr(b2), b2.stride(0) if b2 is not None else 0, K2,
                                             epilogue, L.ptr(e), lde, L.ptr(m_valid), L.stream()), "llx_gemm_nt_bf16_rows")
    else:
        L.check(_lib().llx_gemm_nt_bf16(L.ptr(a), a.stride(0), L.ptr(b), b.stride(0), L.ptr(out), out.stride(0), M, N, K,
                                        L.ptr(a2), a2.stride(0) if a2 is not None else 0, L.ptr(b2), b2.stride(0) if b2 is not None else 0, K2,
                                        epilogue, L.ptr(e), lde, L.stream()), "llx_gemm_nt_bf16")
    if ev is not None:
        ev[1].record()
        kk = K + (K2 if k2_eff is None else min(float(k2_eff), K2))
        Mw = M if m_expect is None else float(m_expect)
        GEMM_TRACE.append((ev[0], ev[1], 2.0 * Mw * N * kk, 2.0 * (Mw * kk + N * kk + Mw * N * (2 if epilogue == EPI_RESIDUAL else 1)), "bf16",
                           gemm_kernel_launches(M, N, 8 if rope is not None else epilogue)))
    return out


def gemm_nt_splitk(a: Tensor, b: Tensor, splits: int, *, m_valid: Optional[Tensor] = None, inv: Optional[Tensor] = None,
                   dev_scalar: Optional[Tensor] = None, m_expect: Optional[float] = None) -> Tensor:
    _chk_bf16(a, b)
    assert a.dim() == 2 and b.dim() == 2 and a.shape[1] == b.shape[1] and a.stride(1) == 1 and b.stride(1) == 1
    M, K = a.shape
    N = b.shape[0]
    part = torch.empty(splits, M, N, device=a.device, dtype=torch.float32)
    ev = None
    if GEMM_TRACE is not None:
        ev = (torch.cuda.Event(enable_timing=True), torch.cuda.Event(enable_timing=True))
        ev[0].record()
    L.check(_lib().llx_gemm_nt_bf16_splitk(L.ptr(a), a.stride(0), L.ptr(b), b.stride(0), L.ptr(part), M, N, K, splits, L.ptr(m_valid), L.stream()),
            "llx_gemm_nt_bf16_splitk")
    if ev is not None:
        ev[1].record()
        Mw = M if m_expect is None else float(m_expect)
        GEMM_TRACE.append((ev[0], ev[1], 2.0 * Mw * N * K, 2.0 * (Mw * K + N * K) + 4.0 * splits * Mw * N, "bf16", 1))
    out = torch.empty(M, N, device=a.device, dtype=BF16)
    assert inv is None or (inv.dtype is torch.int32 and inv.numel() == M)
    assert dev_scalar is None or (dev_scalar.dtype is torch.float32 and dev_scalar.numel() == 1)
    L.check(_lib().llx_splitk_combine(L.ptr(part), splits, M, N, L.ptr(inv), L.ptr(dev_scalar), L.ptr(out), N, L.stream()), "llx_splitk_combine")
    return out


def transpose(x: Tensor, pad_to: int = 1) -> Tensor:
    L.require_cuda(x)
    assert x.dim() == 2 and x.stride(1) == 1 and x.dtype in (BF16, torch.int8)
    R, C = x.shape
    Rp = (R + pad_to - 1) // pad_to * pad_to
    out = (torch.zeros if Rp != R else torch.empty)(C, Rp, device=x.device, dtype=BF16)
    L.check(_lib().llx_transpose(L.ptr(x), x.stride(0), L.ptr(out), Rp, R, C, int(x.dtype is torch.int8), L.stream()), "llx_transpose")
    return out


def pad64(x: Tensor, scale_: float = 1.0, transposed: bool = False) -> Tensor:
    _chk_bf16(x)
    assert x.dim() == 2 and x.stride(1) == 1
    R, C = (x.shape[1], x.shape[0]) if transposed else x.shape
    out = torch.empty(R, SK_PAD, device=x.device, dtype=BF16)
    L.check(_lib().llx_pad64(L.ptr(x), x.stride(0), L.ptr(out), R, C, scale_, int(transposed), L.stream()), "llx_pad64")
    return out


def lora_pack(x: Tensor, out: Tensor, row_off: int, col_off: int, scale_: float = 1.0, transposed: bool = False) -> None:
    _chk_bf16(x, out)
    assert x.dim() == 2 and x.stride(1) == 1 and out.dim() == 2 and out.stride(1) == 1
    R, C = x.shape
    rr, cc = (C, R) if transposed else (R, C)
    assert row_off + rr <= out.shape[0] and col_off + cc <= out.shape[1], (x.shape, out.shape, row_off, col_off, transposed)
    L.check(_lib().llx_lora_pack(L.ptr(x), x.stride(0), L.ptr(out), out.stride(0), R, C, row_off, col_off, scale_, int(transposed), L.stream()),
            "llx_lora_pack")


def lora_group_pack(lora_as: list, lora_bs: list, K_in: int, scale_: float):
    nm = len(lora_as)
    Ns = [b.shape[0] for b in lora_bs]
    ranks = [a.shape[0] for a in lora_as]
    for a, b in zip(lora_as, lora_bs):
        _chk_bf16(a, b)
        assert a.is_contiguous() and b.is_contiguous() and a.shape[1] == K_in and b.shape[1] == a.shape[0]
    N, R = sum(Ns), sum(ranks)
    dev = lora_as[0].device
    buf = torch.empty(R * K_in + N * SK_PAD + R * N + K_in * SK_PAD, device=dev, dtype=BF16)
    a_cat = buf[: R * K_in].view(R, K_in)
    o = R * K_in
    b2 = buf[o : o + N * SK_PAD].view(N, SK_PAD)
    o += N * SK_PAD
    bT = buf[o : o + R * N].view(R, N)
    o += R * N
    a2t = buf[o:].view(K_in, SK_PAD)
    PA = (ctypes.c_void_p * nm)(*[a.data_ptr() for a in lora_as])
    PB = (ctypes.c_void_p * nm)(*[b.data_ptr() for b in lora_bs])
    NS = (ctypes.c_int64 * nm)(*Ns)
    RS = (ctypes.c_int64 * nm)(*ranks)
    L.check(_lib().llx_lora_group_pack(PA, PB, NS, RS, nm, K_in, scale_, L.ptr(a_cat), L.ptr(b2), L.ptr(bT), L.ptr(a2t), L.stream()),
            "llx_lora_group_pack")
    return a_cat, b2, bT, a2t


def lora_groups_pack(groups: list) -> list:
    ng = len(groups)
    assert 1 <= ng <= 4
    sizes, metas = [], []
    for las, lbs, K_in, _ in groups:
        for a, b in zip(las, lbs):
            _chk_bf16(a, b)
            assert a.is_contiguous() and b.is_contiguous() and a.shape[1] == K_in and b.shape[1] == a.shape[0]
        N, R = sum(b.shape[0] for b in lbs), sum(a.shape[0] for a in las)
        metas.append((N, R, K_in))
        sizes.append(R * K_in + N * SK_PAD + R * N + K_in * SK_PAD)
# ... 377 lines not shown
    if epilogue == GV_RESIDUAL:
        assert res is not None and res.shape == (M, N) and res.stride(1) == 1 and res.dtype is BF16
    bs, ranks, t, ldt, lscale = [None] * 3, [0] * 3, None, 0, 0.0
    if lora is not None:
        b_list, t, lscale = lora
        assert len(b_list) == len(ws) and t.dtype is BF16 and t.shape[0] == M and t.stride(1) == 1
        for i, b in enumerate(b_list):
            assert b.dtype is BF16 and b.is_contiguous() and b.shape[0] == ns[i]
            bs[i], ranks[i] = b, b.shape[1]
        assert t.shape[1] == sum(ranks)
        ldt = t.stride(0)
    L.check(_lib().llx_gemv_bf16(wp[0], lw[0], ns[0], wp[1], lw[1], ns[1], wp[2], lw[2], ns[2], L.ptr(x), x.stride(0), M, Kd, L.ptr(nw), eps, epilogue,
                                 L.ptr(out), out.stride(0), L.ptr(res), res.stride(0) if res is not None else 0, L.ptr(rope), n_q, n_k, L.ptr(kc), L.ptr(vc),
                                 c_sh, c_ss, L.ptr(pos), L.ptr(bs[0]), L.ptr(bs[1]), L.ptr(bs[2]), ranks[0], ranks[1], ranks[2], L.ptr(t), ldt, float(lscale),
                                 L.stream()), "llx_gemv_bf16")
    return out


def mask_extent(mask: Tensor) -> Tensor:
    L.require_cuda(mask)
    assert mask.dtype is torch.bool
    m2 = mask.reshape(-1, mask.shape[-1])
    if m2.stride(1) != 1:
        m2 = m2.contiguous()
    ext = torch.empty(1, device=mask.device, dtype=torch.int32)
    L.check(_lib().llx_mask_extent(L.ptr(m2), m2.stride(0), m2.shape[0], m2.shape[1], L.ptr(ext), L.stream()), "llx_mask_extent")
    return ext


def kv_scatter(k: Tensor, v: Tensor, k_cache: Tensor, v_cache: Tensor, input_pos: Tensor) -> None:
    _chk_bf16(k, v, k_cache, v_cache)
    L.require_cuda(input_pos)
    B, KVH, Lq, hd = k.shape
    assert v.shape == k.shape and k.stride() == v.stride() and k.stride(3) == 1 and k_cache.stride() == v_cache.stride() and k_cache.stride(3) == 1
    assert k_cache.shape[0] == B and k_cache.shape[1] == KVH and k_cache.shape[3] == hd and input_pos.shape == (Lq,)
    pos = input_pos.to(torch.int64).contiguous()
    L.check(_lib().llx_kv_scatter(L.ptr(k), L.ptr(v), k.stride(0), k.stride(1), k.stride(2), L.ptr(k_cache), L.ptr(v_cache), k_cache.stride(0),
                                  k_cache.stride(1), k_cache.stride(2), L.ptr(pos), B, KVH, Lq, k_cache.shape[2], hd, L.stream()), "llx_kv_scatter")


_DECODE_WS: dict = {}
_DECODE_WGS = 512


def attn_decode(q: Tensor, k_cache: Tensor, v_cache: Tensor, mask: Tensor, extent: Optional[Tensor] = None, out: Optional[Tensor] = None) -> Tensor:
    _chk_bf16(q, k_cache, v_cache)
    L.require_cuda(mask)
    B, H, M, hd = q.shape
    KVH, Skv = k_cache.shape[1], k_cache.shape[2]
    assert mask.dtype is torch.bool and mask.shape[-2:] == (M, Skv) and k_cache.stride() == v_cache.stride()
    m = mask
    while m.dim() < 4:
        m = m.unsqueeze(0)
    if m.stride(3) != 1:
        m = m.contiguous()
    m_sb = m.stride(0) if m.shape[0] != 1 else 0
    m_sh = m.stride(1) if m.shape[1] != 1 else 0
    nsplit = max(1, min(-(-Skv // 32), -(-_DECODE_WGS // (B * KVH)), 128))
    nbytes = _lib().llx_attn_decode_workspace_bytes(B, H, M, nsplit)
    key = (q.device, torch.cuda.current_stream(q.device).cuda_stream)
    ws = _DECODE_WS.get(key)
    if ws is None or ws.numel() * 4 < nbytes:
        ws = _DECODE_WS[key] = torch.empty(nbytes // 4, device=q.device, dtype=torch.float32)
    if out is None:
        out = torch.empty(B, M, H * hd, device=q.device, dtype=BF16)
    o4 = out.view(B, M, H, hd)
    L.check(_lib().llx_attn_decode(L.ptr(q), q.stride(0), q.stride(1), q.stride(2), L.ptr(k_cache), L.ptr(v_cache), k_cache.stride(0), k_cache.stride(1),
                                   k_cache.stride(2), L.ptr(out), o4.stride(0), o4.stride(2), o4.stride(1), L.ptr(m), m_sb, m_sh, m.stride(2), L.ptr(extent),
                                   L.ptr(ws), B, H, KVH, M, Skv, nsplit, hd, 1.0 / math.sqrt(hd), L.stream()), "llx_attn_decode")
    return out


def head_compact_index(labels: Tensor) -> tuple[Tensor, Tensor, Tensor, Tensor]:
    L.require_cuda(labels)
    labels = labels.reshape(-1).contiguous()
    assert labels.dtype is torch.int64
    T = labels.numel()
    idx = torch.empty(T, device=labels.device, dtype=torch.int32)
    inv = torch.empty(T, device=labels.device, dtype=torch.int32)
    labels_c = torch.empty(T, device=labels.device, dtype=torch.int64)
    count = torch.empty(1, device=labels.device, dtype=torch.int32)
    L.check(_lib().llx_head_compact_index(L.ptr(labels), L.ptr(idx), L.ptr(inv), L.ptr(labels_c), L.ptr(count), T, L.stream()), "llx_head_compact_index")
    return idx, inv, labels_c, count


def gather_rows(src: Tensor, idx: Tensor, count: Tensor) -> Tensor:
    _chk_bf16(src)
    assert src.dim() == 2 and src.stride(1) == 1 and idx.dtype is torch.int32 and idx.numel() == src.shape[0]
    T, D = src.shape
    dst = torch.empty(T, D, device=src.device, dtype=BF16)
    L.check(_lib().llx_gather_rows(L.ptr(src), src.stride(0), L.ptr(idx), L.ptr(count), L.ptr(dst), D, T, D, L.stream()), "llx_gather_rows")
    return dst


def scatter_rows(src: Tensor, inv: Tensor, dev_scalar: Optional[Tensor] = None) -> Tensor:
    _chk_bf16(src)
    assert src.dim() == 2 and src.stride(1) == 1 and inv.dtype is torch.int32 and inv.numel() == src.shape[0]
    assert dev_scalar is None or (dev_scalar.dtype is torch.float32 and dev_scalar.numel() == 1)
    T, D = src.shape
    dst = torch.empty(T, D, device=src.device, dtype=BF16)
    L.check(_lib().llx_scatter_rows(L.ptr(src), src.stride(0), L.ptr(inv), L.ptr(dev_scalar), L.ptr(dst), D, T, D, L.stream()), "llx_scatter_rows")
    return dst


def ce_fwd_bwd(logits: Tensor, labels: Tensor, write_grad: bool, rows: Optional[Tensor] = None) -> tuple[Tensor, Optional[Tensor]]:
    _chk_bf16(logits)
    L.require_cuda(labels)
    lg = _rows2d(logits)
    T, V = lg.shape
    labels = labels.reshape(-1).contiguous()
    assert labels.dtype is torch.int64 and labels.numel() == T
    loss = torch.empty((), device=logits.device, dtype=torch.float32)
    ws = torch.empty(_lib().llx_ce_workspace_bytes(T), device=logits.device, dtype=torch.uint8)
    if rows is not None:
        L.check(_lib().llx_ce_fwd_bwd_rows(L.ptr(lg), lg.stride(0), L.ptr(lg) if write_grad else None, lg.stride(0), L.ptr(labels), L.ptr(loss),
                                           L.ptr(ws), T, V, L.ptr(rows), L.stream()), "llx_ce_fwd_bwd_rows")
    else:
        L.check(_lib().llx_ce_fwd_bwd(L.ptr(lg), lg.stride(0), L.ptr(lg) if write_grad else None, lg.stride(0), L.ptr(labels), L.ptr(loss),
                                      L.ptr(ws), T, V, L.stream()), "llx_ce_fwd_bwd")
    return loss, (lg if write_grad else None)


def ce_chunk(logits: Tensor, labels_all: Tensor, ws: Tensor, loss: Tensor, row0: int, write_grad: bool, rows: Optional[Tensor], first: bool,
             last: bool) -> Optional[Tensor]:
    _chk_bf16(logits)
    n, V = logits.shape
    T = labels_all.numel()
    L.check(_lib().llx_ce_fwd_bwd_part(L.ptr(logits), logits.stride(0), L.ptr(logits) if write_grad else None, logits.stride(0), L.ptr(labels_all),
                                       L.ptr(loss), L.ptr(ws), T, V, row0, n, L.ptr(rows), (1 if first else 0) | (2 if last else 0), L.stream()),
            "llx_ce_fwd_bwd_part")
    return logits if write_grad else None


def skinny_nt(x: Tensor, w: Tensor, kranges: Optional[Sequence[int]] = None, colscale: Optional[Tensor] = None):
    _chk_bf16(x, w, colscale)
    assert x.dim() == 2 and w.dim() == 2 and x.shape[1] == w.shape[1] and x.stride(1) == 1 and w.stride(1) == 1
    M, K = x.shape
    R = w.shape[0]
    out = torch.empty(M, SK_PAD, device=x.device, dtype=BF16)
    kr = None
    if kranges is not None:
        assert len(kranges) == 8
        kr = (ctypes.c_int32 * 8)(*[int(v) for v in kranges])
    if colscale is not None:
        assert colscale.shape == (K,) and colscale.is_contiguous()
        g = torch.empty(M, K, device=x.device, dtype=BF16)
        L.check(_lib().llx_skinny_nt_scaled(L.ptr(x), x.stride(0), L.ptr(w), w.stride(0), L.ptr(out), M, K, R, kr, L.ptr(colscale), L.ptr(g), K,
                                            L.stream()), "llx_skinny_nt_scaled")
        return out, g
    L.check(_lib().llx_skinny_nt(L.ptr(x), x.stride(0), L.ptr(w), w.stride(0), L.ptr(out), M, K, R, kr, L.stream()), "llx_skinny_nt")
    return out


@dataclass
class TnQueued:
    ws: Tensor
    out: Tensor
    out_ld: int
    M: int
    N: int
    R: int
    scale: float
    transpose_out: int
    accumulate: int
    segs: Optional[ctypes.Array]
    n_segs: int
    upart: Optional[Tensor] = None


def skinny_tn(u: Tensor, y: Tensor, R: int, scale_: float, out: Tensor, transpose_out: bool, accumulate: bool = False,
              segs: Optional[Sequence[tuple[int, int, int, int]]] = None, pending: Optional[list] = None,
              u_from: Optional[Tensor] = None, scaled: Optional[tuple[Tensor, Tensor]] = None) -> Tensor:
    _chk_bf16(u, y, out)
    M, N = y.shape
    assert u.shape == (M, SK_PAD) and u.is_contiguous() and y.stride(1) == 1 and out.stride(-1) == 1
    sp, ns = None, 0
    if segs is not None:
        ns = len(segs)
        assert 1 <= ns <= 4 and out.is_contiguous() and out.numel() == sum((b - a) * (d - c) for a, b, c, d in segs)
        sp = (ctypes.c_int32 * (4 * ns))(*[int(v) for sgm in segs for v in sgm])
    else:
        assert out.shape == ((N, R) if transpose_out else (R, N))
    ws = torch.empty(_lib().llx_skinny_tn_workspace_bytes(M, N, R), device=y.device, dtype=torch.uint8)
    out_ld = out.stride(0) if out.dim() == 2 else 0
    if pending is None:
        assert u_from is None and scaled is None, "the fused u / scaled-copy outputs need the queued (pending=) form"
        L.check(_lib().llx_skinny_tn(L.ptr(u), L.ptr(y), y.stride(0), L.ptr(out), out_ld, M, N, R, scale_, int(transpose_out), int(accumulate),
                                     L.ptr(ws), sp, ns, L.stream()), "llx_skinny_tn")
        return out
    q = TnQueued(ws, out, out_ld, M, N, R, scale_, int(transpose_out), int(accumulate), sp, ns)
    if u_from is None:
        assert scaled is None
        L.check(_lib().llx_skinny_tn_partial(L.ptr(u), L.ptr(y), y.stride(0), M, N, R, L.ptr(ws), sp, ns, L.stream()), "llx_skinny_tn_partial")
    else:
        assert u_from.dtype is BF16 and u_from.dim() == 2 and u_from.shape == (R, N) and u_from.stride(1) == 1
        q.upart = torch.empty(_lib().llx_skinny_u_workspace_bytes(M, N) // 4, device=y.device, dtype=torch.float32)
        cs = g = None
        if scaled is not None:
            cs, g = scaled
            assert cs.dtype is BF16 and cs.numel() == N and g.shape == (M, N) and g.stride(1) == 1
        one = lambda ctype, v: (ctype * 1)(v)
        ptr = lambda t: one(ctypes.c_void_p, t.data_ptr() if t is not None else None)
        L.check(_lib().llx_skinny_tn_partial_many_us(1, ptr(u), ptr(y), one(ctypes.c_int64, y.stride(0)), one(ctypes.c_int64, M), one(ctypes.c_int64, N),
                                                     one(ctypes.c_int64, R), ptr(ws), one(ctypes.c_void_p, ctypes.cast(sp, ctypes.c_void_p).value if sp is not None else None),
                                                     one(ctypes.c_int, ns), ptr(u_from), one(ctypes.c_int64, u_from.stride(0)), ptr(q.upart), ptr(cs), ptr(g),
                                                     one(ctypes.c_int64, g.stride(0) if g is not None else 0), L.stream()), "llx_skinny_tn_partial_many")
    pending.append(q)
    if len(pending) == 4:
        skinny_tn_flush(pending)
    return out


def skinny_u_reduce(q: TnQueued) -> Tensor:
    assert q.upart is not None, "the product must have been queued with u_from"
    out = torch.empty(q.M, SK_PAD, device=q.upart.device, dtype=BF16)
    L.check(_lib().llx_skinny_u_reduce(L.ptr(q.upart), L.ptr(out), q.M, q.N, q.R, q.segs, q.n_segs, L.stream()), "llx_skinny_u_reduce")
    return out


def skinny_tn_flush(pending: list) -> None:
    while pending:
        chunk, pending[:] = pending[:4], pending[4:]
        n = len(chunk)
        WS = (ctypes.c_void_p * n)(*[q.ws.data_ptr() for q in chunk])
        OUT = (ctypes.c_void_p * n)(*[q.out.data_ptr() for q in chunk])
        LD = (ctypes.c_int64 * n)(*[q.out_ld for q in chunk])
        MM = (ctypes.c_int64 * n)(*[q.M for q in chunk])
        NN = (ctypes.c_int64 * n)(*[q.N for q in chunk])
        RR = (ctypes.c_int64 * n)(*[q.R for q in chunk])
        SC = (ctypes.c_float * n)(*[q.scale for q in chunk])
        TR = (ctypes.c_int * n)(*[q.transpose_out for q in chunk])
        AC = (ctypes.c_int * n)(*[q.accumulate for q in chunk])
        SG = (ctypes.c_void_p * n)(*[ctypes.cast(q.segs, ctypes.c_void_p).value if q.segs is not None else None for q in chunk])
        NS = (ctypes.c_int * n)(*[q.n_segs for q in chunk])
        L.check(_lib().llx_skinny_tn_reduce_many(n, WS, OUT, LD, MM, NN, RR, SC, TR, AC, SG, NS, L.stream()), "llx_skinny_tn_reduce_many")
```

llama-x_amd/llx/ops.py:

```python
from __future__ import annotations

import os

from typing import Optional, Sequence

import torch
from torch import Tensor, nn
from torch.autograd import Function

from . import kernels as K
from ._lib import LlxError

BF16 = torch.bfloat16


def _cached_multi(tensors: Sequence[Tensor], tag: str, build):
    store = tensors[0].__dict__.setdefault("_llx_cache", {})
    key = tuple((t._version, str(t.device)) for t in tensors)
    hit = store.get(tag)
    if hit is not None and hit[0] == key:
        return hit[1]
    val = build()
    store[tag] = (key, val)
    return val


def _cached(t: Tensor, tag: str, build):
    return _cached_multi([t], tag, build)


def weight_t(w: Tensor) -> Tensor:
    return _cached(w, "wt", lambda: K.transpose(w.detach()))


class LinearPlan:

    def __init__(self, m: nn.Linear):
        from subclasses.int8 import Int8LinearWeight

        self.N, self.K = m.out_features, m.in_features
        self.weight = m.weight
        self.bias = m.bias
        self.rank = int(getattr(m, "rank", 0) or 0)
        self.lora_a = getattr(m, "lora_a", None) if self.rank > 0 else None
        self.lora_b = getattr(m, "lora_b", None) if self.rank > 0 else None
        self.scale = float(getattr(m, "scale", 1.0))
        self.dora_m = getattr(m, "m", None) if self.rank > 0 else None
        self.int8 = isinstance(self.weight, Int8LinearWeight)
        self.dynamic = bool(self.int8 and self.weight.dynamic_int8_act)
        if self.dora_m is not None and self.int8:
            raise LlxError("DoRA on an Int8LinearWeight is not supported (nor by the reference: no dispatch for weight + delta)")
        if self.rank > 64:
            raise LlxError(f"LoRA rank {self.rank} > 64 is not supported by the skinny kernels")
        if self.rank > 0 and self.lora_a.dtype is not BF16:
            raise LlxError("LoRA factors must be bf16")

    def tensors(self) -> list[Tensor]:
        ts = []
        if not self.int8:
            ts.append(self.weight)
        if self.bias is not None:
            ts.append(self.bias)
        if self.rank > 0:
            ts += [self.lora_a, self.lora_b]
        if self.dora_m is not None:
            ts.append(self.dora_m)
        return ts

    def forward(self, x: Tensor, out: Optional[Tensor] = None, residual: Optional[Tensor] = None, gelu: bool = False):
        t = b2 = None
        if self.rank > 0:
            t = K.skinny_nt(x, self.lora_a.detach())
            b2 = K.pad64(self.lora_b.detach(), self.scale)
        if self.dora_m is not None:
            if gelu:
                raise LlxError("DoRA + GELU epilogue is not supported")
            w = self.weight.detach()
            c, inv = dora_colscale([self], w, self.lora_a.detach(), b2)
            z = K.gemm_nt(x, w, a2=t, b2=b2, k2_eff=self.rank)
            direct = residual is None
            y = K.colscale_bias(z, c, self.bias.detach() if self.bias is not None else None, out=out if direct else None)
            if residual is not None:
                y = K.add(y, residual, out=out)
            return y, (t, z, c, inv)
        if self.int8:
            from subclasses.int8 import int8_linear_forward

            if self.bias is not None or gelu:
                raise LlxError("int8 linear with bias is not on the fused path")
            direct = self.rank == 0 and residual is None
            y = int8_linear_forward(x, self.weight, out=out if direct else None)
            if self.rank > 0:
                y = K.gemm_nt(t, b2, out=out if residual is None else None, epilogue=K.EPI_RESIDUAL, e=y, k2_eff=0)
            if residual is not None:
                y = K.add(y, residual, out=out)
            return y, t
        w = self.weight.detach()
        if self.bias is not None:
            if residual is not None:
                raise LlxError("bias + residual epilogue is not supported")
            y = K.gemm_nt(x, w, out=out, a2=t, b2=b2, epilogue=K.EPI_BIAS_GELU if gelu else K.EPI_BIAS, e=self.bias.detach(), k2_eff=self.rank)
        elif residual is not None:
            y = K.gemm_nt(x, w, out=out, a2=t, b2=b2, epilogue=K.EPI_RESIDUAL, e=residual, k2_eff=self.rank)
        else:
            y = K.gemm_nt(x, w, out=out, a2=t, b2=b2, k2_eff=self.rank)
        return y, t

    def backward(self, dy: Tensor, x: Tensor, t: Optional[Tensor], needs: Sequence[bool], need_dx: bool = True,
                 dx_out: Optional[Tensor] = None, dx_accum: bool = False):
        grads: list[Optional[Tensor]] = []
        ni = iter(needs)
        u = None
        dy_out, gm = dy, None
        if self.dora_m is not None:
            t, z, c, inv = t
            if needs[-1]:
                gm = K.colsum_mul(dy, z, inv)
            dy = K.scale(dy, colscale=c)
        if self.rank > 0:
            u = K.skinny_nt(dy, K.transpose(self.lora_b.detach()))
        if not self.int8:
            grads.append(K.gemm_tn(dy, x) if next(ni) else None)
        if self.bias is not None:
            grads.append(K.colsum(dy_out) if next(ni) else None)
        if self.rank > 0:
            need_a, need_b = next(ni), next(ni)
            ga = gb = None
            if need_a:
                ga = _grad_dst([self.lora_a], (self.rank, self.K))
                if ga is None:
                    ga = torch.empty(self.rank, self.K, device=dy.device, dtype=BF16)
                K.skinny_tn(u, x, self.rank, self.scale, ga, transpose_out=False)
            if need_b:
                gb = _grad_dst([self.lora_b], (self.N, self.rank))
                if gb is None:
                    gb = torch.empty(self.N, self.rank, device=dy.device, dtype=BF16)
                K.skinny_tn(t, dy, self.rank, self.scale, gb, transpose_out=True)
            grads += [ga, gb]
        if self.dora_m is not None:
            grads.append(gm)
        dx = None
        if need_dx:
            b2 = K.pad64(self.lora_a.detach(), self.scale, transposed=True) if self.rank > 0 else None
            if self.int8:
                from subclasses.int8 import int8_weight_t

                g = K.scale(dy, colscale=self.weight.scale)
                wt = int8_weight_t(self.weight)
            else:
                g = dy
                wt = weight_t(self.weight)
            if dx_accum:
                dx = K.gemm_nt(g, wt, out=dx_out, a2=u, b2=b2, epilogue=K.EPI_RESIDUAL, e=dx_out, k2_eff=self.rank)
            else:
                dx = K.gemm_nt(g, wt, out=dx_out, a2=u, b2=b2, k2_eff=self.rank)
        return dx, grads


def dora_colscale(members: Sequence[LinearPlan], w_cat: Tensor, a_cat: Tensor, b2: Tensor) -> tuple[Tensor, Tensor]:
    N, R = w_cat.shape[0], a_cat.shape[0]
    wn2 = _cached_multi([m.weight for m in members], "wn2", lambda: K.rownorm2(w_cat))
    G = K.skinny_nt(w_cat, a_cat)
    AAt = K.skinny_nt(a_cat, a_cat)
    c = torch.empty(N, device=w_cat.device, dtype=BF16)
    inv = torch.empty(N, device=w_cat.device, dtype=torch.float32)
    off = 0
    for m in members:
        sl = slice(off, off + m.N)
        K.dora_colscale(wn2[sl], G[sl], b2[sl], AAt, m.dora_m.detach(), c[sl], inv[sl], R)
        off += m.N
    return c, inv


class GroupPlan:

    def __init__(self, mods: Sequence[nn.Linear]):
        self.members = [LinearPlan(m) for m in mods]
        m0 = self.members[0]
        self.K = m0.K
        self.Ns = [m.N for m in self.members]
        self.N = sum(self.Ns)
        self.n_off = [sum(self.Ns[:i]) for i in range(len(self.Ns))]
        self.ranks = [m.rank for m in self.members]
        self.R = sum(self.ranks)
        self.r_off = [sum(self.ranks[:i]) for i in range(len(self.ranks))]
        same_kind = all((m.int8, m.dynamic) == (m0.int8, m0.dynamic) for m in self.members)
        same_scale = len({m.scale for m in self.members if m.rank > 0}) <= 1
        lora_all_or_none = all(r > 0 for r in self.ranks) or self.R == 0
        dora_all_or_none = len({m.dora_m is not None for m in self.members}) == 1
        self.dora = all(m.dora_m is not None for m in self.members)
        self.fused = (same_kind and same_scale and lora_all_or_none and dora_all_or_none and self.R <= 64
                      and all(m.bias is None for m in self.members) and all(m.K == self.K for m in self.members))
        self.int8, self.dynamic = m0.int8, m0.dynamic
        self.packed = None
        self.scale = next((m.scale for m in self.members if m.rank > 0), 1.0)
        self.k2_fwd = sum(n * r for n, r in zip(self.Ns, self.ranks)) / self.N

    def tensors(self) -> list[Tensor]:
        return [t for m in self.members for t in m.tensors()]

    def _weights(self):
        return [(m.weight.int_data if m.int8 else m.weight) for m in self.members]

    def w_cat(self) -> Tensor:
        ws = self._weights()
        if self.int8 and self.dynamic:
            return _cached_multi(ws, "cat_i8", lambda: torch.cat([w.detach() for w in ws], 0))
        if self.int8:
            return _cached_multi(ws, "cat_bf16", lambda: K.i8_to_bf16(torch.cat([w.detach() for w in ws], 0)))
        return _cached_multi(ws, "cat", lambda: torch.cat([w.detach() for w in ws], 0) if len(ws) > 1 else ws[0].detach())

    def wt_cat(self) -> Tensor:
        ws = self._weights()
        return _cached_multi(ws, "cat_t", lambda: K.transpose(torch.cat([w.detach() for w in ws], 0) if len(ws) > 1 else ws[0].detach()))

    def scale_cat(self) -> Tensor:
        ss = [m.weight.scale for m in self.members]
        return _cached_multi(ss, "cat_scale", lambda: torch.cat(ss, 0) if len(ss) > 1 else ss[0])

    def forward(self, x: Tensor, out: Optional[Tensor] = None, residual: Optional[Tensor] = None, swiglu_h: Optional[Tensor] = None,
                rope: Optional[tuple[Tensor, int, int]] = None, xq: Optional[tuple[Tensor, Tensor]] = None, t_pre: Optional[Tensor] = None):
        if out is None:
            out = torch.empty(x.shape[0], self.N, device=x.device, dtype=BF16)
        return out, self._forward(x, out, residual, swiglu_h, rope, xq, t_pre)

    def norm_can_make_t(self, dim: int) -> bool:
        return self.fused and self.R > 0 and self.packed is not None and K.rmsnorm_skinny_ok(dim)

    def wants_quantized_input(self) -> bool:
        return self.fused and self.int8 and self.dynamic

    def rope_fusable(self) -> bool:
        return self.fused and (not self.int8 or self.dynamic) and not self.dora

    def swiglu_fusable(self) -> bool:
        return self.fused and (not self.int8 or self.dynamic) and not self.dora and len(self.members) == 2 and self.Ns[0] % 128 == 0

    def _forward(self, x: Tensor, out: Tensor, residual: Optional[Tensor], swiglu_h: Optional[Tensor] = None,
                 rope: Optional[tuple[Tensor, int, int]] = None, xq: Optional[tuple[Tensor, Tensor]] = None, t_pre: Optional[Tensor] = None):
        if not self.fused:
            assert residual is None or len(self.members) == 1
            return [m.forward(x, out=out[:, o : o + n], residual=residual)[1] for m, o, n in zip(self.members, self.n_off, self.Ns)]
        t = b2 = None
        if self.R > 0:
            a_cat, b2, bT, a2t = self.packed or K.lora_group_pack([m.lora_a.detach() for m in self.members],
                                                                  [m.lora_b.detach() for m in self.members], self.K, self.scale)
            t = (t_pre if t_pre is not None else K.skinny_nt(x, a_cat), bT, a2t)
        if self.dora:
            assert swiglu_h is None and rope is None
            c, inv = dora_colscale(self.members, self.w_cat(), a_cat, b2)
            z = K.gemm_nt(x, self.w_cat(), a2=t[0], b2=b2, k2_eff=self.k2_fwd)
            K.scale(z, colscale=c, out=out)
            if residual is not None:
                K.add(out, residual, out=out)
            return (*t, z, c, inv)
        if not self.int8:
            if residual is not None:
                K.gemm_nt(x, self.w_cat(), out=out, a2=t[0] if t else None, b2=b2, epilogue=K.EPI_RESIDUAL, e=residual, k2_eff=self.k2_fwd)
            elif swiglu_h is not None:
                K.gemm_nt(x, self.w_cat(), out=out, a2=t[0] if t else None, b2=b2, epilogue=K.EPI_SWIGLU_FWD, e=swiglu_h, k2_eff=self.k2_fwd)
            else:
                K.gemm_nt(x, self.w_cat(), out=out, a2=t[0] if t else None, b2=b2, rope=rope, k2_eff=self.k2_fwd)
            return t
        if self.dynamic:
            from subclasses.int8 import quantize_int8_rowwise
            from subclasses.int8_mm import _launch as i8_gemm

            xi, xs = xq if xq is not None else quantize_int8_rowwise(x)
            a2, bb = (t[0], b2) if self.R > 0 else (None, None)
            if residual is not None:
                i8_gemm(xi, self.w_cat(), xs, self.scale_cat(), out=out, a2=a2, b2=bb, epilogue=K.EPI_RESIDUAL, e=residual)
            elif swiglu_h is not None:
                i8_gemm(xi, self.w_cat(), xs, self.scale_cat(), out=out, a2=a2, b2=bb, epilogue=K.EPI_SWIGLU_FWD, e=swiglu_h)
            else:
                i8_gemm(xi, self.w_cat(), xs, self.scale_cat(), out=out, a2=a2, b2=bb, rope=rope)
            return t
        else:
            direct = self.R == 0 and residual is None
            y0 = K.gemm_nt(x, self.w_cat(), out=out if direct else None, epilogue=K.EPI_COLSCALE, e=self.scale_cat())
        if self.R > 0:
            y0 = K.gemm_nt(t[0], b2, out=out if residual is None else None, epilogue=K.EPI_RESIDUAL, e=y0, k2_eff=0)
        if residual is not None:
            K.add(y0, residual, out=out)
        return t

    def _tn_segs(self) -> Optional[list[tuple[int, int, int, int]]]:
        if getattr(self, "_segs", None) is None:
            segs = [(no, no + n, ro, ro + r) for ro, r, no, n in zip(self.r_off, self.ranks, self.n_off, self.Ns) if r > 0]
            ok = 1 <= len(segs) <= 4 and all(a % 256 == 0 and (b % 256 == 0 or b == self.N) for a, b, _, _ in segs)
            self._segs = segs if ok else False
        return self._segs or None

    def _kranges(self) -> Optional[list[int]]:
        if getattr(self, "_kr", None) is None and len(self.members) == 1:
            self._kr = False
        if getattr(self, "_kr", None) is None:
            kr: list[int] = []
            for nb in range(4):
                lo, hi = None, None
                for ro, r, no, n in zip(self.r_off, self.ranks, self.n_off, self.Ns):
                    if r > 0 and ro < 16 * nb + 16 and ro + r > 16 * nb:
                        lo = no if lo is None else min(lo, no)
                        hi = no + n if hi is None else max(hi, no + n)
                kr += [lo or 0, hi or 0] if lo is not None else [0, 0]
            ok = all(v % 64 == 0 for v in kr)
            self._kr = kr if ok else False
        return self._kr or None

    def backward(self, dy: Tensor, x: Tensor, saved, needs: Sequence[bool], need_dx: bool, dx_out: Optional[Tensor] = None,
                 swiglu: Optional[tuple[Tensor, Tensor]] = None, pending: Optional[list] = None):
        if not self.fused:
            grads, dx, first = [], None, True
            ni = 0
            for m, o, n, t in zip(self.members, self.n_off, self.Ns, saved):
                cnt = len(m.tensors())
                d, g = m.backward(dy[:, o : o + n], x, t, needs[ni : ni + cnt], need_dx, dx_out, not first)
                ni += cnt
                grads += g
                dx = d if d is not None else dx
                first = False
            return dx, grads
        gM = None
        ni = iter(needs)
        need = []
        for m in self.members:
            cnt = len(m.tensors())
            need.append([next(ni) for _ in range(cnt)])
        ia = -3 if self.dora else -2
        dy_out = dy
        z = inv = None
        if self.dora:
            t, bT, a2t, z, c, inv = saved
            dy = K.scale(dy_out, colscale=c)
        else:
            t, bT, a2t = saved if saved is not None else (None, None, None)
        u = gA = gBt = g_scaled = None
        gB_views: Optional[list[Optional[Tensor]]] = None
        need_a, need_b = self.R > 0 and any(nd[ia] for nd in need), self.R > 0 and any(nd[ia + 1] for nd in need)
        if self.dora and any(nd[-1] for nd in need):
            gM = K.colsum_mul(dy_out, z, inv)
        if need_b:
            segs = self._tn_segs()
            if segs is not None:
                flat = _grad_dst([m.lora_b for m in self.members if m.rank > 0])
                if flat is None:
                    flat = torch.empty(sum((b - a) * (d - c_) for a, b, c_, d in segs), device=dy.device, dtype=BF16)
                sc = None
                if self.int8 and need_dx:
                    g_scaled = torch.empty_like(dy)
                    sc = (self.scale_cat(), g_scaled)
                K.skinny_tn(t, dy, self.R, self.scale, flat, transpose_out=True, segs=segs, pending=pending, u_from=bT, scaled=sc)
                u = K.skinny_u_reduce(pending[-1])
                gB_views, off = [], 0
                for m_, (a, b, c_, d) in zip([m for m in self.members if m.rank > 0], segs):
                    gB_views.append(flat[off : off + (b - a) * (d - c_)].view(b - a, d - c_))
                    off += (b - a) * (d - c_)
            else:
                gBt = torch.empty(self.N, self.R, device=dy.device, dtype=BF16)
                K.skinny_tn(t, dy, self.R, self.scale, gBt, transpose_out=True)
        if self.R > 0:
            if u is not None:
                pass
            elif self.int8 and need_dx:
                u, g_scaled = K.skinny_nt(dy, bT, self._kranges(), colscale=self.scale_cat())
            else:
                u = K.skinny_nt(dy, bT, self._kranges())
            if need_a:
                gA = _grad_dst([m.lora_a for m in self.members if m.rank > 0], (self.R, self.K))
                if gA is None:
                    gA = torch.empty(self.R, self.K, device=dy.device, dtype=BF16)
                K.skinny_tn(u, x, self.R, self.scale, gA, transpose_out=False, pending=pending)
        dx = None
        if need_dx:
            if self.int8:
                g = g_scaled if g_scaled is not None else K.scale(dy, colscale=self.scale_cat())
            else:
                g = dy
            if swiglu is not None:
                dx = K.gemm_nt(g, self.wt_cat(), out=swiglu[1], a2=u, b2=a2t if self.R > 0 else None, epilogue=K.EPI_SWIGLU_BWD, e=swiglu[0], k2_eff=self.R)
            else:
                dx = K.gemm_nt(g, self.wt_cat(), out=dx_out, a2=u, b2=a2t if self.R > 0 else None, k2_eff=self.R)
        grads: list[Optional[Tensor]] = []
        gb_i = 0
        for m, nd, ro, no, n in zip(self.members, need, self.r_off, self.n_off, self.Ns):
            j = 0
            if not m.int8:
                grads.append(K.gemm_tn(dy[:, no : no + n], x) if nd[j] else None)
                j += 1
            if m.rank > 0:
                grads.append(gA[ro : ro + m.rank] if nd[j] else None)
                if gB_views is not None:
                    grads.append(gB_views[gb_i] if nd[j + 1] else None)
                    gb_i += 1
                else:
                    grads.append(gBt[no : no + n, ro : ro + m.rank].contiguous() if nd[j + 1] else None)
                j += 2
            if m.dora_m is not None:
                grads.append(gM[no : no + n] if nd[j] else None)
        return dx, grads


def _grad_dst(params: Sequence[Optional[Tensor]], shape: Optional[tuple] = None) -> Optional[Tensor]:
    g0 = first = end = None
    for p in params:
        slot = getattr(p, "_llx_slot", None)
        if slot is None or p.grad is not None or getattr(p, "_llx_claimed", False):
            return None
        G, off, n = slot
        if g0 is None:
            g0, first = G, off
        elif G is not g0 or off != end:
            return None
        end = off + n
    if g0 is None:
        return None
    for p in params:
        p._llx_claimed = True
    out = g0[first:end]
    return out.view(shape) if shape is not None else out


def _enc(o, flat: list):
    if isinstance(o, Tensor):
        flat.append(o)
        return ("t", len(flat) - 1)
    if isinstance(o, (tuple, list)):
        return ("l", [_enc(x, flat) for x in o])
    return ("c", o)


def _dec(sp, flat):
    kind, v = sp
    if kind == "t":
        return flat[v]
    if kind == "l":
        return tuple(_dec(x, flat) for x in v)
    return v


def _save(ctx, *objs) -> None:
    flat: list[Tensor] = []
    ctx._llx_spec = [_enc(o, flat) for o in objs]
    ctx.save_for_backward(*flat)


def _load(ctx) -> list:
    flat = ctx.saved_tensors
    return [_dec(sp, flat) for sp in ctx._llx_spec]


def prepack(plans: Sequence[GroupPlan]) -> None:
    todo = [p for p in plans if p.fused and p.R > 0]
    for i in range(0, len(todo), 4):
        chunk = todo[i : i + 4]
        if len(chunk) < 2:
            break
        imgs = K.lora_groups_pack([([m.lora_a.detach() for m in p.members], [m.lora_b.detach() for m in p.members], p.K, p.scale) for p in chunk])
        for p, im in zip(chunk, imgs):
            p.packed = im


def _norm_prologue(meta, plan: GroupPlan, x2: Tensor, norm_w: Optional[Tensor]):
    if not meta.fuse_norm:
        return x2, None, None, None
    if plan.wants_quantized_input():
        xn, rstd, *xq = K.rmsnorm_fwd(x2, norm_w.detach(), meta.eps, quant=True)
        return xn, rstd, xq, None
    if plan.norm_can_make_t(x2.shape[1]):
        xn, rstd, t_pre = K.rmsnorm_skinny_nt(x2, norm_w.detach(), meta.eps, plan.packed[0])
        return xn, rstd, None, t_pre
    xn, rstd = K.rmsnorm_fwd(x2, norm_w.detach(), meta.eps)
    return xn, rstd, None, None


def _norm_epilogue(dxn: Optional[Tensor], x2: Tensor, norm_w: Optional[Tensor], rstd: Optional[Tensor], need_dnw: bool,
                   dres: Optional[Tensor] = None, fuse_norm: bool = True):
    if dxn is None:
        return None, None
    if fuse_norm:
        return K.rmsnorm_bwd(dxn, x2, norm_w.detach(), rstd, need_dnw, dres, dw_out=_grad_dst([norm_w]))
    return (K.add(dxn, dres) if dres is not None else dxn), None


def _plans_tensors(plans: Sequence[LinearPlan]) -> tuple[list[Tensor], list[int]]:
    ts, counts = [], []
    for p in plans:
        t = p.tensors()
        ts += t
        counts.append(len(t))
    return ts, counts


class LinearFn(Function):
    @staticmethod
    def forward(ctx, x: Tensor, plan: LinearPlan, *tensors):
        K.L.require_cuda(x)
        x2 = K._rows2d(x)
        y, t = plan.forward(x2)
        ctx.plan = plan
        _save(ctx, x2, t)
        ctx.xshape = x.shape
        return y.view(*x.shape[:-1], plan.N)

    @staticmethod
    def backward(ctx, dy: Tensor):
        plan: LinearPlan = ctx.plan
        dy2 = K._rows2d(dy)
        needs = ctx.needs_input_grad[2:]
        x2, t = _load(ctx)
        dx, grads = plan.backward(dy2, x2, t, needs, need_dx=ctx.needs_input_grad[0])
        return (dx.view(ctx.xshape) if dx is not None else None, None, *grads)


def linear(x: Tensor, m: nn.Linear) -> Tensor:
    plan = LinearPlan(m)
    return LinearFn.apply(x, plan, *plan.tensors())


class RMSNormFn(Function):
    @staticmethod
    def forward(ctx, x: Tensor, w: Tensor, eps: float):
        y, rstd = K.rmsnorm_fwd(x.contiguous(), w.detach(), eps)
        ctx.save_for_backward(x, w, rstd)
        return y

    @staticmethod
    def backward(ctx, dy: Tensor):
        x, w, rstd = ctx.saved_tensors
        dx, dw = K.rmsnorm_bwd(dy.contiguous(), x.contiguous(), w.detach(), rstd, ctx.needs_input_grad[1], dw_out=_grad_dst([w]))
        return dx, dw, None


def rmsnorm(x: Tensor, w: Tensor, eps: float) -> Tensor:
    return RMSNormFn.apply(x, w, eps)


class AttnBlockMeta:
    def __init__(self, qkv: GroupPlan, wo: GroupPlan, num_heads, num_kv_heads, head_dim, mask, eps, fuse_norm, fuse_residual):
        self.qkv, self.wo = qkv, wo
        self.H, self.KVH, self.hd = num_heads, num_kv_heads, head_dim
        self.mask, self.eps = mask, eps
        self.fuse_norm, self.fuse_residual = fuse_norm, fuse_residual


class AttnBlockFn(Function):
    @staticmethod
    def forward(ctx, x: Tensor, rope: Tensor, norm_w: Optional[Tensor], meta: AttnBlockMeta, *tensors):
        K.L.require_cuda(x)
        B, S, D = x.shape
        H, KVH, hd = meta.H, meta.KVH, meta.hd
        x2 = K._rows2d(x.contiguous())
        xn, rstd, xq, t_pre = _norm_prologue(meta, meta.qkv, x2, norm_w)
        W = (H + 2 * KVH) * hd
        qkv = torch.empty(B * S, W, device=x.device, dtype=BF16)
        fuse_rope = meta.qkv.rope_fusable()
        _, tqkv = meta.qkv.forward(xn, qkv, rope=(rope, S, (H + KVH) * hd) if fuse_rope else None, xq=xq, t_pre=t_pre)
        qkv3 = qkv.view(B, S, W)
        if not fuse_rope:
            K.rope_(qkv3, rope, H + KVH)
        q = qkv3[..., : H * hd].unflatten(-1, (H, hd))
        k = qkv3[..., H * hd : (H + KVH) * hd].unflatten(-1, (KVH, hd))
        v = qkv3[..., (H + KVH) * hd :].unflatten(-1, (KVH, hd))
        o, lse = K.attn_fwd(q, k, v, meta.mask)
        o2 = o.view(B * S, H * hd)
        y, to = meta.wo.forward(o2, None, x2 if meta.fuse_residual else None)
        ctx.meta = meta
        _save(ctx, x, rope, norm_w, x2, xn if meta.fuse_norm else None, rstd, qkv3, o, lse, tqkv, to)
        return y.view(B, S, D)

    @staticmethod
    def backward(ctx, dy: Tensor):
        meta: AttnBlockMeta = ctx.meta
        x, rope, norm_w, x2, xn, rstd, qkv3, o, lse, tqkv, to = _load(ctx)
        if xn is None:
            xn = x2
        B, S, D = x.shape
        H, KVH, hd = meta.H, meta.KVH, meta.hd
        dy2 = K._rows2d(dy.contiguous())
        needs = list(ctx.needs_input_grad[4:])
        n_qkv = len(meta.qkv.tensors())
        nqkv, no = needs[:n_qkv], needs[n_qkv:]
        pend = []
        do2, g_o = meta.wo.backward(dy2, o.view(B * S, H * hd), to, no, True, pending=pend)
        W = (H + 2 * KVH) * hd
        dqkv = torch.empty(B, S, W, device=x.device, dtype=BF16)
        q = qkv3[..., : H * hd].unflatten(-1, (H, hd))
        k = qkv3[..., H * hd : (H + KVH) * hd].unflatten(-1, (KVH, hd))
        v = qkv3[..., (H + KVH) * hd :].unflatten(-1, (KVH, hd))
        dq = dqkv[..., : H * hd].unflatten(-1, (H, hd))
        dk = dqkv[..., H * hd : (H + KVH) * hd].unflatten(-1, (KVH, hd))
        dv = dqkv[..., (H + KVH) * hd :].unflatten(-1, (KVH, hd))
        K.attn_bwd(q, k, v, o, do2.view(B, S, H, hd), lse, dq, dk, dv, meta.mask, rope=rope)
        d2 = dqkv.view(B * S, W)
        need_dx = ctx.needs_input_grad[0]
        need_dxn = need_dx or (meta.fuse_norm and ctx.needs_input_grad[2])
        dxn = torch.empty(B * S, D, device=x.device, dtype=BF16) if need_dxn else None
        _, g_qkv = meta.qkv.backward(d2, xn, tqkv, nqkv, need_dxn, dxn, pending=pend)
        K.skinny_tn_flush(pend)
        dx, dnw = _norm_epilogue(dxn, x2, norm_w, rstd, ctx.needs_input_grad[2], dy2 if (need_dx and meta.fuse_residual) else None, meta.fuse_norm)
        return (dx.view(B, S, D) if (dx is not None and need_dx) else None, None, dnw, None, *g_qkv, *g_o)


_HEAD_COMPACT = os.environ.get("LLX_HEAD_COMPACT", "1") != "0"
_HEAD_SPLITK = max(1, int(os.environ.get("LLX_HEAD_SPLITK", "4")))
_HEAD_CHUNK_FORCED = "LLX_HEAD_CHUNK_ROWS" in os.environ
_HEAD_CHUNK_ROWS = max(256, int(os.environ.get("LLX_HEAD_CHUNK_ROWS", "8192")) // 256 * 256)


class MLPBlockMeta:
    def __init__(self, w13: GroupPlan, w2: GroupPlan, eps, fuse_norm, fuse_residual):
        self.w13, self.w2 = w13, w2
        self.eps, self.fuse_norm, self.fuse_residual = eps, fuse_norm, fuse_residual


class MLPBlockFn(Function):
    @staticmethod
    def forward(ctx, x: Tensor, norm_w: Optional[Tensor], meta: MLPBlockMeta, *tensors):
        K.L.require_cuda(x)
        shape = x.shape
        x2 = K._rows2d(x.contiguous())
        xn, rstd, xq, t_pre = _norm_prologue(meta, meta.w13, x2, norm_w)
        T, I = x2.shape[0], meta.w13.Ns[0]
        gu = torch.empty(T, 2 * I, device=x.device, dtype=BF16)
        if meta.w13.swiglu_fusable():
            h = torch.empty(T, I, device=x.device, dtype=BF16)
            _, t13 = meta.w13.forward(xn, gu, swiglu_h=h, xq=xq, t_pre=t_pre)
        else:
            _, t13 = meta.w13.forward(xn, gu, xq=xq, t_pre=t_pre)
            h = K.swiglu_fwd(gu[:, :I], gu[:, I:])
        y, t2 = meta.w2.forward(h, None, x2 if meta.fuse_residual else None)
        ctx.meta = meta
        _save(ctx, x, norm_w, x2, xn if meta.fuse_norm else None, rstd, gu, h, t13, t2)
        return y.view(shape)

    @staticmethod
    def backward(ctx, dy: Tensor):
        meta: MLPBlockMeta = ctx.meta
        x, norm_w, x2, xn, rstd, gu, h, t13, t2 = _load(ctx)
        if xn is None:
            xn = x2
        T, I = x2.shape[0], meta.w13.Ns[0]
        dy2 = K._rows2d(dy.contiguous())
        needs = list(ctx.needs_input_grad[3:])
        n_13 = len(meta.w13.tensors())
        n13, n2 = needs[:n_13], needs[n_13:]
        dgu = torch.empty(T, 2 * I, device=x.device, dtype=BF16)
        pend = []
        if meta.w2.fused:
            _, g_2 = meta.w2.backward(dy2, h, t2, n2, True, swiglu=(gu, dgu), pending=pend)
        else:
            dh, g_2 = meta.w2.backward(dy2, h, t2, n2, True)
            K.swiglu_bwd(dh, gu[:, :I], gu[:, I:], dgu[:, :I], dgu[:, I:])
        need_dx = ctx.needs_input_grad[0]
        need_dxn = need_dx or (meta.fuse_norm and ctx.needs_input_grad[1])
        dxn = torch.empty_like(x2) if need_dxn else None
        _, g_13 = meta.w13.backward(dgu, xn, t13, n13, need_dxn, dxn, pending=pend)
        K.skinny_tn_flush(pend)
        dx, dnw = _norm_epilogue(dxn, x2, norm_w, rstd, ctx.needs_input_grad[1], dy2 if (need_dx and meta.fuse_residual) else None, meta.fuse_norm)
        return (dx.view(x.shape) if (dx is not None and need_dx) else None, dnw, None, *g_13, *g_2)


class HeadLossFn(Function):

    @staticmethod
    def forward(ctx, x: Tensor, norm_w: Tensor, labels: Tensor, eps: float, plan: LinearPlan, *tensors):
        K.L.require_cuda(x, labels)
        x2 = K._rows2d(x.contiguous())
        xn, rstd = K.rmsnorm_fwd(x2, norm_w.detach(), eps)
        need_grad = any(ctx.needs_input_grad)
        ctx.plan, ctx.eps = plan, eps
        plain = not plan.int8 and plan.rank == 0 and plan.bias is None and plan.dora_m is None
        ctx.plain_head = plain and not any(ctx.needs_input_grad[5:])
        ctx.plain_trainable = plain and not ctx.plain_head and _HEAD_COMPACT
        ctx.compact = _HEAD_COMPACT and plain
        ctx.m_expect = None
        T, V = x2.shape[0], plan.N
        chunk = _HEAD_CHUNK_ROWS if (_HEAD_CHUNK_FORCED or T * V * 2 >= 2**32) else 0
        if chunk and T > chunk:
            if not ctx.plain_head:
                raise LlxError(f"LM head over {T} rows x {V} vocabulary entries exceeds one logits buffer (4 GiB) and a trainable / adapted / "
                               "quantised head is not chunked: freeze the plain head or lower the number of positions per step")
            inv = cnt = None
            rows_in, labels_in = xn, labels.reshape(-1).contiguous()
            if ctx.compact:
                idx, inv, labels_in, cnt = K.head_compact_index(labels)
                rows_in = K.gather_rows(xn, idx, cnt)
            w = plan.weight.detach()
            ws = torch.empty(T + 2, device=x.device, dtype=torch.float32)
            loss = torch.empty((), device=x.device, dtype=torch.float32)
            parts = []
            for r0 in range(0, T, chunk):
                r1 = min(T, r0 + chunk)
                cnt_c = torch.clamp(cnt - r0, min=0, max=r1 - r0).to(torch.int32) if cnt is not None else None
                lg = torch.empty(r1 - r0, V, device=x.device, dtype=BF16)
                K.gemm_nt(rows_in[r0:r1], w, out=lg, m_valid=cnt_c)
                parts.append((K.ce_chunk(lg, labels_in, ws, loss, r0, need_grad, cnt, r0 == 0, r1 == T), cnt_c))
            ctx.chunk = chunk
            _save(ctx, x, norm_w, x2, None, rstd, tuple(p[0] for p in parts), (inv, cnt, tuple(p[1] for p in parts)))
            return loss
        ctx.chunk = 0
        if ctx.compact:
            idx, inv, labels_c, cnt = K.head_compact_index(labels)
            xc = K.gather_rows(xn, idx, cnt)
            w = plan.weight.detach()
            logits = torch.empty(xc.shape[0], w.shape[0], device=x.device, dtype=BF16)
            ctx.m_expect = float(cnt.item()) if K.GEMM_TRACE is not None else None
            K.gemm_nt(xc, w, out=logits, m_valid=cnt, m_expect=ctx.m_expect)
            loss, dlogits = K.ce_fwd_bwd(logits, labels_c, write_grad=need_grad, rows=cnt)
            _save(ctx, x, norm_w, x2, xc if ctx.plain_trainable else None, rstd, dlogits, (inv, cnt))
            return loss
        logits, t = plan.forward(xn)
        loss, dlogits = K.ce_fwd_bwd(logits, labels, write_grad=need_grad)
        _save(ctx, x, norm_w, x2, xn, rstd, dlogits, t)
        return loss

    @staticmethod
    def backward(ctx, gout: Tensor):
        plan: LinearPlan = ctx.plan
        x, norm_w, x2, xn, rstd, dlogits, t = _load(ctx)
        needs = ctx.needs_input_grad[5:]
        g32 = gout.detach().to(torch.float32).reshape(1)
        if ctx.plain_head or ctx.plain_trainable:
            if ctx.chunk:
                inv, cnt, cnts = t
                dx = dnw = None
                if ctx.needs_input_grad[0] or ctx.needs_input_grad[1]:
                    wt = weight_t(plan.weight)
                    T = x2.shape[0]
                    split = wt.shape[1] % (64 * _HEAD_SPLITK) == 0
                    dxc = torch.empty(T, wt.shape[0], device=x.device, dtype=BF16)
                    for i, (dl, cnt_c) in enumerate(zip(dlogits, cnts)):
                        r0 = i * ctx.chunk
                        part = K.gemm_nt_splitk(dl, wt, _HEAD_SPLITK, m_valid=cnt_c) if split else K.gemm_nt(dl, wt, m_valid=cnt_c)
                        dxc[r0 : r0 + dl.shape[0]].copy_(part)
                    dxn = K.scatter_rows(dxc, inv, g32) if inv is not None else K.scale(dxc, dev_scalar=g32)
                    dx, dnw = _norm_epilogue(dxn, x2, norm_w, rstd, ctx.needs_input_grad[1])
                return (dx.view(x.shape) if dx is not None else None, dnw, None, None, None, *([None] * len(needs)))
            inv, cnt = t if ctx.compact else (None, None)
            dx = dnw = None
            if ctx.needs_input_grad[0] or ctx.needs_input_grad[1]:
                wt = weight_t(plan.weight)
                if wt.shape[1] % (64 * _HEAD_SPLITK) == 0:
                    dxn = K.gemm_nt_splitk(dlogits, wt, _HEAD_SPLITK, m_valid=cnt, inv=inv, dev_scalar=g32, m_expect=ctx.m_expect)
                elif ctx.compact:
                    dxn = K.scatter_rows(K.gemm_nt(dlogits, wt, m_valid=cnt, m_expect=ctx.m_expect), inv, g32)
                else:
                    dxn = K.scale(K.gemm_nt(dlogits, wt), dev_scalar=g32)
                dx, dnw = _norm_epilogue(dxn, x2, norm_w, rstd, ctx.needs_input_grad[1])
            gw = None
            if ctx.plain_trainable:
                gw = K.scale(K.gemm_tn(dlogits, xn, m_valid=cnt, m_expect=ctx.m_expect), dev_scalar=g32)
            return (dx.view(x.shape) if dx is not None else None, dnw, None, None, None, *([gw] + [None] * (len(needs) - 1) if needs else []))
        dxn, grads = plan.backward(dlogits, xn, t, needs, need_dx=ctx.needs_input_grad[0] or ctx.needs_input_grad[1])
        grads = [None if g is None else K.scale(g, dev_scalar=g32) for g in grads]
        if dxn is not None:
            K.scale(dxn, dev_scalar=g32, out=dxn)
        dx, dnw = _norm_epilogue(dxn, x2, norm_w, rstd, ctx.needs_input_grad[1])
        return (dx.view(x.shape) if dx is not None else None, dnw, None, None, None, *grads)
```

Before: 32000 tokens/s.

## Defer LoRA and RMSNorm weight-grad reductions into a cross-layer batched tail queue

Adds a persistent tail queue that defers skinny TN LoRA gradient reductions and RMSNorm dw column-sum reductions across autograd functions. They are then flushed in one batched reduce kernel that handles both product reductions and column sums, with a flattened block index over entries. The batch limit on partial and reduce kernels rises from 4 to 8/10 entries, and partial entries are sorted by rows_per_split. This is meant to cut many small reduce launches and tail effects per layer, at the cost of extra autograd callback and flush bookkeeping and a risk of ordering bugs when grad buffers are reused.

```diff
diff --git a/include/llx.h b/include/llx.h
--- a/include/llx.h
+++ b/include/llx.h
@@ -20,6 +20,9 @@
 int llx_rmsnorm_bwd(const void* dy, const void* x, const void* w, const float* rstd, void* dx, void* dw ,
                     int dw_accumulate, void* workspace, const void* dres ,
                     int64_t rows, int64_t dim, llx_stream_t s);
+int64_t llx_rmsnorm_bwd_partial_count(int64_t rows);
+int llx_rmsnorm_bwd_partials(const void* dy, const void* x, const void* w, const float* rstd, void* dx, void* workspace,
+                             const void* dres , int64_t rows, int64_t dim, llx_stream_t s);
 
 int llx_gemm_nt_bf16(const void* A, int64_t lda, const void* B, int64_t ldb, void* C, int64_t ldc, int64_t M, int64_t N, int64_t K,
                      const void* A2, int64_t lda2, const void* B2, int64_t ldb2, int64_t K2, int epilogue, const void* E, int64_t lde,
@@ -137,6 +140,10 @@
 int llx_skinny_tn_reduce_many(int n, const void* const* workspaces, void* const* outs, const int64_t* out_ld, const int64_t* M, const int64_t* N,
                               const int64_t* R, const float* scale, const int* transpose_out, const int* accumulate,
                               const int32_t* const* segs, const int* seg_count, llx_stream_t s);
+int llx_skinny_tn_reduce_many_cs(int n, const void* const* workspaces, void* const* outs, const int64_t* out_ld, const int64_t* M,
+                                 const int64_t* N, const int64_t* R, const float* scale, const int* transpose_out, const int* accumulate,
+                                 const int32_t* const* segs, const int* seg_count, int ncs, const void* const* cs_partial,
+                                 void* const* cs_out, const int64_t* cs_nparts, const int64_t* cs_dim, const int* cs_accumulate, llx_stream_t s);
 int llx_pad64(const void* in, int64_t ld, void* out, int64_t R, int64_t C, float scale, int transpose, llx_stream_t s);
 int llx_lora_group_pack(const void* const* lora_a, const void* const* lora_b, const int64_t* Ns, const int64_t* ranks, int nm, int64_t K,
                         float scale, void* a_cat, void* b2, void* bT, void* a2t, llx_stream_t s);
diff --git a/llama-x_amd/csrc/common.h b/llama-x_amd/csrc/common.h
--- a/llama-x_amd/csrc/common.h
+++ b/llama-x_amd/csrc/common.h
@@ -86,6 +86,24 @@
 
 static inline int64_t cdiv64(int64_t a, int64_t b) { return (a + b - 1) / b; }
 
+__device__ __forceinline__ void colsum_partials_block(const float* __restrict__ partial, bf16_t* __restrict__ out, int nparts, int dim,
+                                                      int accumulate, int blk, float (*red)[17]) {
+  const int c = threadIdx.x & 15, grp = threadIdx.x >> 4;
+  const int col = blk * 16 + c;
+  float s = 0.f;
+  if (col < dim)
+    for (int p = grp; p < nparts; p += 16) s += partial[(int64_t)p * dim + col];
+  red[grp][c] = s;
+  __syncthreads();
+  if (grp == 0 && col < dim) {
+    s = 0.f;
+#pragma unroll
+    for (int g = 0; g < 16; ++g) s += red[g][c];
+    if (accumulate) s += bf2f(out[col]);
+    out[col] = f2bf(s);
+  }
+}
+
 __device__ __forceinline__ float sigmoidf_(float x) { return __builtin_amdgcn_rcpf(1.f + __expf(-x)); }
 __device__ __forceinline__ u32x4_t swiglu_fwd8(const u32x4_t& gv, const u32x4_t& uv) {
   u32x4_t o;
diff --git a/llama-x_amd/csrc/rmsnorm.hip b/llama-x_amd/csrc/rmsnorm.hip
--- a/llama-x_amd/csrc/rmsnorm.hip
+++ b/llama-x_amd/csrc/rmsnorm.hip
@@ -184,20 +184,7 @@
 __global__ __launch_bounds__(256) void colsum_partials_kernel(const float* __restrict__ partial, bf16_t* __restrict__ out, int nparts, int dim,
                                                               int accumulate) {
   __shared__ float red[16][17];
-  const int c = threadIdx.x & 15, grp = threadIdx.x >> 4;
-  const int col = blockIdx.x * 16 + c;
-  float s = 0.f;
-  if (col < dim)
-    for (int p = grp; p < nparts; p += 16) s += partial[(int64_t)p * dim + col];
-  red[grp][c] = s;
-  __syncthreads();
-  if (grp == 0 && col < dim) {
-    s = 0.f;
-#pragma unroll
-    for (int g = 0; g < 16; ++g) s += red[g][c];
-    if (accumulate) s += bf2f(out[col]);
-    out[col] = f2bf(s);
-  }
+  colsum_partials_block(partial, out, nparts, dim, accumulate, blockIdx.x, red);
 }
 
 extern "C" int llx_rmsnorm_fwd(const void* x, const void* w, void* y, float* rstd, int64_t rows, int64_t dim, float eps,
@@ -244,17 +231,15 @@
   return cdiv64(rows, rpb) * dim * 4;
 }
 
-extern "C" int llx_rmsnorm_bwd(const void* dy, const void* x, const void* w, const float* rstd, void* dx, void* dw,
-                               int dw_accumulate, void* workspace, const void* dres, int64_t rows, int64_t dim, hipStream_t stream) {
-  LLX_REQUIRE(dy && x && w && rstd && dx, "llx_rmsnorm_bwd: null pointer");
-  LLX_REQUIRE(dim > 0 && dim % 8 == 0 && dim <= 8192, "llx_rmsnorm_bwd: dim=%lld must be a multiple of 8 and <= 8192", (long long)dim);
-  LLX_REQUIRE(!dw || workspace, "llx_rmsnorm_bwd: workspace required when dw is requested");
-  if (rows == 0) return LLX_OK;
+extern "C" int64_t llx_rmsnorm_bwd_partial_count(int64_t rows) { return cdiv64(rows, (int64_t)RMS_BWD_RPB); }
+
+static int rmsnorm_bwd_launch(const char* name, const void* dy, const void* x, const void* w, const float* rstd, void* dx, bool want_dw,
+                              void* workspace, const void* dres, int64_t rows, int64_t dim, hipStream_t stream) {
   const int rpb = RMS_BWD_RPB;
   const int nblk = (int)cdiv64(rows, rpb);
   const int nch = (int)cdiv64(dim, 512);
-  float* part = dw ? (float*)workspace : nullptr;
-  const size_t lds = dw ? (size_t)dim * 4 : 0;
+  float* part = want_dw ? (float*)workspace : nullptr;
+  const size_t lds = want_dw ? (size_t)dim * 4 : 0;
 #define L(N) hipLaunchKernelGGL(rmsnorm_bwd_kernel<N>, dim3(nblk), dim3(256), lds, stream, (const bf16_t*)dy, (const bf16_t*)x, (const bf16_t*)w, rstd, (bf16_t*)dx, part, (const bf16_t*)dres, rows, (int)dim, rpb)
 #define LF(N) if (dres) LFR(N, 1); else LFR(N, 0)
 #define LFR(N, R) hipLaunchKernelGGL((rmsnorm_bwd_kernel<N, true, R>), dim3(nblk), dim3(256), lds, stream, (const bf16_t*)dy, (const bf16_t*)x, (const bf16_t*)w, rstd, (bf16_t*)dx, part, (const bf16_t*)dres, rows, (int)dim, rpb)
@@ -263,11 +248,30 @@
 #undef LFR
 #undef LF
 #undef L
-  LLX_LAUNCH_CHECK("llx_rmsnorm_bwd");
+  LLX_LAUNCH_CHECK(name);
+  return LLX_OK;
+}
+
+extern "C" int llx_rmsnorm_bwd(const void* dy, const void* x, const void* w, const float* rstd, void* dx, void* dw,
+                               int dw_accumulate, void* workspace, const void* dres, int64_t rows, int64_t dim, hipStream_t stream) {
+  LLX_REQUIRE(dy && x && w && rstd && dx, "llx_rmsnorm_bwd: null pointer");
+  LLX_REQUIRE(dim > 0 && dim % 8 == 0 && dim <= 8192, "llx_rmsnorm_bwd: dim=%lld must be a multiple of 8 and <= 8192", (long long)dim);
+  LLX_REQUIRE(!dw || workspace, "llx_rmsnorm_bwd: workspace required when dw is requested");
+  if (rows == 0) return LLX_OK;
+  const int rc = rmsnorm_bwd_launch("llx_rmsnorm_bwd", dy, x, w, rstd, dx, dw != nullptr, workspace, dres, rows, dim, stream);
+  if (rc != LLX_OK) return rc;
   if (dw) {
-    hipLaunchKernelGGL(colsum_partials_kernel, dim3((unsigned)cdiv64(dim, 16)), dim3(256), 0, stream, part, (bf16_t*)dw, nblk,
-                       (int)dim, dw_accumulate);
+    hipLaunchKernelGGL(colsum_partials_kernel, dim3((unsigned)cdiv64(dim, 16)), dim3(256), 0, stream, (const float*)workspace, (bf16_t*)dw,
+                       (int)llx_rmsnorm_bwd_partial_count(rows), (int)dim, dw_accumulate);
     LLX_LAUNCH_CHECK("llx_rmsnorm_bwd(colsum)");
   }
   return LLX_OK;
 }
+
+extern "C" int llx_rmsnorm_bwd_partials(const void* dy, const void* x, const void* w, const float* rstd, void* dx, void* workspace,
+                                        const void* dres, int64_t rows, int64_t dim, hipStream_t stream) {
+  LLX_REQUIRE(dy && x && w && rstd && dx && workspace, "llx_rmsnorm_bwd_partials: null pointer");
+  LLX_REQUIRE(rows > 0 && dim > 0 && dim % 8 == 0 && dim <= 8192, "llx_rmsnorm_bwd_partials: rows > 0, dim=%lld must be a multiple of 8 and <= 8192",
+              (long long)dim);
+  return rmsnorm_bwd_launch("llx_rmsnorm_bwd_partials", dy, x, w, rstd, dx, true, workspace, dres, rows, dim, stream);
+}
diff --git a/llama-x_amd/csrc/skinny.hip b/llama-x_amd/csrc/skinny.hip
--- a/llama-x_amd/csrc/skinny.hip
+++ b/llama-x_amd/csrc/skinny.hip
@@ -277,7 +277,7 @@
   skinny_tn_block<NB>(U, Y, ldy, partial, M, N, rows_per_split, sg, blockIdx.x, blockIdx.y, NB, sY, sU);
 }
 
-#define TN_MANY 4
+#define TN_MANY 8
 struct TnPart { const bf16_t* U; const bf16_t* Y; int64_t ldy; float* partial; int M, N, rows_per_split, ctiles, nblocks, nbl; TnSegs sg;
                 const bf16_t* Bt; int64_t ldb; float* upart; int brows; const bf16_t* cs; bf16_t* G; int64_t ldg; };
 struct TnPartMany { TnPart d[TN_MANY]; int n; };
@@ -374,7 +374,8 @@
                                              const int64_t* R, void* const* workspaces, const int32_t* const* segs, const int* seg_count,
                                              const void* const* Bt, const int64_t* ldb, void* const* upart, const void* const* colscale,
                                              void* const* G, const int64_t* ldg, hipStream_t stream) {
-  LLX_REQUIRE(n >= 1 && n <= TN_MANY && U && Y && ldy && M && N && R && workspaces && segs && seg_count, "llx_skinny_tn_partial_many: bad arguments (1..4 products)");
+  LLX_REQUIRE(n >= 1 && n <= TN_MANY && U && Y && ldy && M && N && R && workspaces && segs && seg_count, "llx_skinny_tn_partial_many: bad arguments (1..8 products)");
+  static_assert(sizeof(TnPartMany) <= 2048, "kernel arguments of skinny_tn_many_kernel");
   TnPartMany m;
   m.n = n;
   int total_blocks = 0;
@@ -406,6 +407,12 @@
     }
     total_blocks += d.nblocks;
   }
+  for (int i = 1; i < n; ++i) {
+    const TnPart t = m.d[i];
+    int j = i;
+    for (; j > 0 && m.d[j - 1].rows_per_split < t.rows_per_split; --j) m.d[j] = m.d[j - 1];
+    m.d[j] = t;
+  }
   int nbmax = 1;
   for (int i = 0; i < n; ++i) nbmax = m.d[i].nbl > nbmax ? m.d[i].nbl : nbmax;
   const dim3 grid((unsigned)total_blocks), block(256);
@@ -458,12 +465,21 @@
   return LLX_OK;
 }
 
-struct TnRed { const float* partial; bf16_t* out; int64_t out_ld, total; int nsplit, RP, R, N, transpose_out, accumulate, use_segs; float scale; TnSegs sg; };
-struct TnRedMany { TnRed d[TN_MANY]; };
-
-__global__ void skinny_tn_reduce_many_kernel(const TnRedMany m) {
-  const TnRed& d = m.d[blockIdx.y];
-  int64_t idx = (int64_t)blockIdx.x * blockDim.x + threadIdx.x;
+#define TN_RED_MANY 10
+struct TnRed { const float* partial; bf16_t* out; int64_t out_ld, total; int nsplit, RP, R, N, transpose_out, accumulate, use_segs, colsum; float scale; TnSegs sg; };
+struct TnRedMany { TnRed d[TN_RED_MANY]; int first[TN_RED_MANY + 1]; int n; };
+
+__global__ __launch_bounds__(256) void skinny_tn_reduce_many_kernel(const TnRedMany m) {
+  __shared__ float red[16][17];
+  int i = 0;
+  while (i < m.n - 1 && (int)blockIdx.x >= m.first[i + 1]) ++i;
+  const TnRed& d = m.d[i];
+  const int blk = (int)blockIdx.x - m.first[i];
+  if (d.colsum) {
+    colsum_partials_block(d.partial, d.out, d.nsplit, d.N, d.accumulate, blk, red);
+    return;
+  }
+  int64_t idx = (int64_t)blk * blockDim.x + threadIdx.x;
   if (idx >= d.total) return;
   int r, n;
   bf16_t* dst;
@@ -509,29 +525,57 @@
   *dst = f2bf(sum);
 }
 
-extern "C" int llx_skinny_tn_reduce_many(int n, const void* const* workspaces, void* const* outs, const int64_t* out_ld, const int64_t* M,
-                                         const int64_t* N, const int64_t* R, const float* scale, const int* transpose_out, const int* accumulate,
-                                         const int32_t* const* segs, const int* seg_count, hipStream_t stream) {
-  LLX_REQUIRE(n >= 1 && n <= TN_MANY && workspaces && outs && out_ld && M && N && R && scale && transpose_out && accumulate && segs && seg_count,
-              "llx_skinny_tn_reduce_many: bad arguments (1..4 products)");
+extern "C" int llx_skinny_tn_reduce_many_cs(int n, const void* const* workspaces, void* const* outs, const int64_t* out_ld, const int64_t* M,
+                                            const int64_t* N, const int64_t* R, const float* scale, const int* transpose_out, const int* accumulate,
+                                            const int32_t* const* segs, const int* seg_count, int ncs, const void* const* cs_partial,
+                                            void* const* cs_out, const int64_t* cs_nparts, const int64_t* cs_dim, const int* cs_accumulate,
+                                            hipStream_t stream) {
+  LLX_REQUIRE(n >= 0 && ncs >= 0 && n + ncs >= 1 && n + ncs <= TN_RED_MANY, "llx_skinny_tn_reduce_many: bad arguments (1..10 entries)");
+  LLX_REQUIRE(n == 0 || (workspaces && outs && out_ld && M && N && R && scale && transpose_out && accumulate && segs && seg_count),
+              "llx_skinny_tn_reduce_many: null product array");
+  LLX_REQUIRE(ncs == 0 || (cs_partial && cs_out && cs_nparts && cs_dim && cs_accumulate), "llx_skinny_tn_reduce_many_cs: null column-sum array");
+  static_assert(sizeof(TnRedMany) <= 3072, "kernel arguments of skinny_tn_reduce_many_kernel");
   TnRedMany m;
-  int64_t most = 0;
+  int64_t blocks = 0;
   for (int i = 0; i < n; ++i) {
     TnRed& d = m.d[i];
     LLX_REQUIRE(workspaces[i] && outs[i] && M[i] > 0 && N[i] > 0 && R[i] > 0 && R[i] <= 64, "llx_skinny_tn_reduce_many: bad product %d", i);
     d.partial = (const float*)workspaces[i]; d.out = (bf16_t*)outs[i]; d.out_ld = out_ld[i];
     d.nsplit = tn_splits(M[i], N[i]); d.RP = (int)cdiv64(R[i], 16) * 16; d.R = (int)R[i]; d.N = (int)N[i];
     d.transpose_out = transpose_out[i]; d.accumulate = accumulate[i]; d.scale = scale[i];
-    d.use_segs = segs[i] != nullptr;
+    d.use_segs = segs[i] != nullptr; d.colsum = 0;
     int64_t total = 0;
     const int rc = tn_fill_segs(d.sg, segs[i], seg_count[i], N[i], R[i], &total);
     if (rc != LLX_OK) return rc;
     d.total = d.use_segs ? total : R[i] * N[i];
-    if (d.total > most) most = d.total;
-  }
-  hipLaunchKernelGGL(skinny_tn_reduce_many_kernel, dim3((unsigned)cdiv64(most, 256), (unsigned)n), dim3(256), 0, stream, m);
+    m.first[i] = (int)blocks;
+    blocks += cdiv64(d.total, 256);
+  }
+  for (int j = 0; j < ncs; ++j) {
+    TnRed& d = m.d[n + j];
+    LLX_REQUIRE(cs_partial[j] && cs_out[j] && cs_nparts[j] > 0 && cs_dim[j] > 0 && cs_nparts[j] < (1 << 30) && cs_dim[j] < (1 << 30),
+                "llx_skinny_tn_reduce_many_cs: bad column sum %d", j);
+    d = TnRed{};
+    d.partial = (const float*)cs_partial[j]; d.out = (bf16_t*)cs_out[j];
+    d.nsplit = (int)cs_nparts[j]; d.N = (int)cs_dim[j]; d.accumulate = cs_accumulate[j]; d.colsum = 1;
+    d.total = cs_dim[j];
+    m.first[n + j] = (int)blocks;
+    blocks += cdiv64(cs_dim[j], 16);
+  }
+  LLX_REQUIRE(blocks < (1ll << 31), "llx_skinny_tn_reduce_many: too many blocks");
+  m.n = n + ncs;
+  for (int i = m.n; i <= TN_RED_MANY; ++i) m.first[i] = (int)blocks;
+  hipLaunchKernelGGL(skinny_tn_reduce_many_kernel, dim3((unsigned)blocks), dim3(256), 0, stream, m);
   LLX_LAUNCH_CHECK("llx_skinny_tn_reduce_many");
   return LLX_OK;
+}
+
+extern "C" int llx_skinny_tn_reduce_many(int n, const void* const* workspaces, void* const* outs, const int64_t* out_ld, const int64_t* M,
+                                         const int64_t* N, const int64_t* R, const float* scale, const int* transpose_out, const int* accumulate,
+                                         const int32_t* const* segs, const int* seg_count, hipStream_t stream) {
+  LLX_REQUIRE(n >= 1, "llx_skinny_tn_reduce_many: bad arguments (1..10 products)");
+  return llx_skinny_tn_reduce_many_cs(n, workspaces, outs, out_ld, M, N, R, scale, transpose_out, accumulate, segs, seg_count, 0, nullptr, nullptr,
+                                      nullptr, nullptr, nullptr, stream);
 }
 
 extern "C" int llx_skinny_tn(const void* U, const void* Y, int64_t ldy, void* out, int64_t out_ld, int64_t M, int64_t N, int64_t R,
diff --git a/llama-x_amd/llx/_lib.py b/llama-x_amd/llx/_lib.py
--- a/llama-x_amd/llx/_lib.py
+++ b/llama-x_amd/llx/_lib.py
@@ -20,6 +20,8 @@
     "llx_rmsnorm_fwd_quant": (c_int, [_P, _P, _P, _P, _P, _L, _P, _L, _L, _F, _P]),
     "llx_rmsnorm_bwd_workspace_bytes": (c_int64, [_L, _L]),
     "llx_rmsnorm_bwd": (c_int, [_P, _P, _P, _P, _P, _P, _I, _P, _P, _L, _L, _P]),
+    "llx_rmsnorm_bwd_partial_count": (c_int64, [_L]),
+    "llx_rmsnorm_bwd_partials": (c_int, [_P, _P, _P, _P, _P, _P, _P, _L, _L, _P]),
     "llx_attn_flags_bytes": (c_int64, [_L, _L]),
     "llx_attn_tile_flags": (c_int, [_P, _P, _P, _L, _L, _P]),
     "llx_attn_fwd": (c_int, [_P, _L, _L, _P, _L, _L, _P, _L, _L, _P, _L, _L, _P, _P, _P, _P, _L, _L, _L, _L, _L, _F, _P]),
@@ -81,6 +83,7 @@
     "llx_skinny_u_reduce": (c_int, [_P, _P, _L, _L, _L, _P, _I, _P]),
     "llx_skinny_tn_partial_many_us": (c_int, [_I, _P, _P, _P, _P, _P, _P, _P, _P, _P, _P, _P, _P, _P, _P, _P, _P]),
     "llx_skinny_tn_reduce_many": (c_int, [_I, _P, _P, _P, _P, _P, _P, _P, _P, _P, _P, _P, _P]),
+    "llx_skinny_tn_reduce_many_cs": (c_int, [_I, _P, _P, _P, _P, _P, _P, _P, _P, _P, _P, _P, _I, _P, _P, _P, _P, _P, _P]),
     "llx_gemm_nt_bf16": (c_int, [_P, _L, _P, _L, _P, _L, _L, _L, _L, _P, _L, _P, _L, _L, _I, _P, _L, _P]),
     "llx_gemm_nt_bf16_splitk": (c_int, [_P, _L, _P, _L, _P, _L, _L, _L, _I, _P, _P]),
     "llx_splitk_combine": (c_int, [_P, _I, _L, _L, _P, _P, _P, _L, _P]),
diff --git a/llama-x_amd/llx/dp.py b/llama-x_amd/llx/dp.py
--- a/llama-x_amd/llx/dp.py
+++ b/llama-x_amd/llx/dp.py
@@ -83,6 +83,9 @@
 
     def prescale(self, b):
         if not b.get("scaled"):
+            from . import ops
+
+            ops.tail_flush()
             if b["arena"]:
                 self.arena.settle(b["params"])
             if self.world > 1:
diff --git a/llama-x_amd/llx/kernels.py b/llama-x_amd/llx/kernels.py
--- a/llama-x_amd/llx/kernels.py
+++ b/llama-x_amd/llx/kernels.py
@@ -82,7 +82,7 @@
 
 
 def rmsnorm_bwd(dy: Tensor, x: Tensor, w: Tensor, rstd: Tensor, need_dw: bool, dres: Optional[Tensor] = None,
-                dw_out: Optional[Tensor] = None) -> tuple[Tensor, Optional[Tensor]]:
+                dw_out: Optional[Tensor] = None, pending: Optional["TailQueue"] = None) -> tuple[Tensor, Optional[Tensor]]:
     _chk_bf16(dy, x, w, dres)
     x2, dy2 = _rows2d(x), _rows2d(dy)
     if dy2.stride(0) != dy2.shape[1]:
@@ -97,6 +97,11 @@
     if dres is not None:
         dres = _rows2d(dres)
         assert dres.shape == x2.shape and dres.stride(0) == dim
+    if need_dw and pending is not None and rows > 0:
+        L.check(_lib().llx_rmsnorm_bwd_partials(L.ptr(dy2), L.ptr(x2), L.ptr(w), L.ptr(rstd), L.ptr(dx), L.ptr(ws), L.ptr(dres), rows, dim,
+                                                L.stream()), "llx_rmsnorm_bwd_partials")
+        pending.push(ColsumQueued(ws, dw.view(dim), _lib().llx_rmsnorm_bwd_partial_count(rows), dim, 0))
+        return dx.view(x.shape), dw
     L.check(_lib().llx_rmsnorm_bwd(L.ptr(dy2), L.ptr(x2), L.ptr(w), L.ptr(rstd), L.ptr(dx), L.ptr(dw), 0, L.ptr(ws), L.ptr(dres), rows, dim,
                                    L.stream()), "llx_rmsnorm_bwd")
     return dx.view(x.shape), dw
@@ -780,6 +785,10 @@
     return out
 
 
+TN_FIRST_MAX = 8
+TN_REDUCE_MAX = 10
+
+
 @dataclass
 class TnQueued:
     ws: Tensor
@@ -794,11 +803,32 @@
     segs: Optional[ctypes.Array]
     n_segs: int
     upart: Optional[Tensor] = None
+    u: Optional[Tensor] = None
+    y: Optional[Tensor] = None
+
+
+@dataclass
+class ColsumQueued:
+    ws: Tensor
+    out: Tensor
+    nparts: int
+    dim: int
+    accumulate: int
+
+
+class TailQueue(list):
+    cap = TN_REDUCE_MAX
+    must_flush = False
+
+    def push(self, q) -> None:
+        if len(self) >= self.cap:
+            skinny_tn_flush(self)
+        self.append(q)
 
 
 def skinny_tn(u: Tensor, y: Tensor, R: int, scale_: float, out: Tensor, transpose_out: bool, accumulate: bool = False,
               segs: Optional[Sequence[tuple[int, int, int, int]]] = None, pending: Optional[list] = None,
-              u_from: Optional[Tensor] = None, scaled: Optional[tuple[Tensor, Tensor]] = None) -> Tensor:
+              u_from: Optional[Tensor] = None, scaled: Optional[tuple[Tensor, Tensor]] = None, defer: bool = False) -> Tensor:
     _chk_bf16(u, y, out)
     M, N = y.shape
     assert u.shape == (M, SK_PAD) and u.is_contiguous() and y.stride(1) == 1 and out.stride(-1) == 1
@@ -816,8 +846,11 @@
         L.check(_lib().llx_skinny_tn(L.ptr(u), L.ptr(y), y.stride(0), L.ptr(out), out_ld, M, N, R, scale_, int(transpose_out), int(accumulate),
                                      L.ptr(ws), sp, ns, L.stream()), "llx_skinny_tn")
         return out
-    q = TnQueued(ws, out, out_ld, M, N, R, scale_, int(transpose_out), int(accumulate), sp, ns)
-    if u_from is None:
+    q = TnQueued(ws, out.view(out.shape) if isinstance(pending, TailQueue) else out, out_ld, M, N, R, scale_, int(transpose_out), int(accumulate), sp, ns)
+    if defer:
+        assert u_from is None and scaled is None and isinstance(pending, TailQueue), "only a plain product can wait in a TailQueue"
+        q.u, q.y = u, y
+    elif u_from is None:
         assert scaled is None
         L.check(_lib().llx_skinny_tn_partial(L.ptr(u), L.ptr(y), y.stride(0), M, N, R, L.ptr(ws), sp, ns, L.stream()), "llx_skinny_tn_partial")
     else:
@@ -833,10 +866,26 @@
                                                      one(ctypes.c_int64, R), ptr(ws), one(ctypes.c_void_p, ctypes.cast(sp, ctypes.c_void_p).value if sp is not None else None),
                                                      one(ctypes.c_int, ns), ptr(u_from), one(ctypes.c_int64, u_from.stride(0)), ptr(q.upart), ptr(cs), ptr(g),
                                                      one(ctypes.c_int64, g.stride(0) if g is not None else 0), L.stream()), "llx_skinny_tn_partial_many")
+    if isinstance(pending, TailQueue):
+        pending.push(q)
+        return out
     pending.append(q)
     if len(pending) == 4:
         skinny_tn_flush(pending)
     return out
+
+
+def _tn_first_many(chunk: list) -> None:
+    n = len(chunk)
+    arr = lambda ctype, vals: (ctype * n)(*vals)
+    L.check(_lib().llx_skinny_tn_partial_many(n, arr(ctypes.c_void_p, [q.u.data_ptr() for q in chunk]), arr(ctypes.c_void_p, [q.y.data_ptr() for q in chunk]),
+                                              arr(ctypes.c_int64, [q.y.stride(0) for q in chunk]), arr(ctypes.c_int64, [q.M for q in chunk]),
+                                              arr(ctypes.c_int64, [q.N for q in chunk]), arr(ctypes.c_int64, [q.R for q in chunk]),
+                                              arr(ctypes.c_void_p, [q.ws.data_ptr() for q in chunk]),
+                                              arr(ctypes.c_void_p, [ctypes.cast(q.segs, ctypes.c_void_p).value if q.segs is not None else None for q in chunk]),
+                                              arr(ctypes.c_int, [q.n_segs for q in chunk]), L.stream()), "llx_skinny_tn_partial_many")
+    for q in chunk:
+        q.u = q.y = None
 
 
 def skinny_u_reduce(q: TnQueued) -> Tensor:
@@ -847,18 +896,25 @@
 
 
 def skinny_tn_flush(pending: list) -> None:
+    cap = getattr(pending, "cap", 4)
+    if isinstance(pending, TailQueue):
+        pending.must_flush = False
     while pending:
-        chunk, pending[:] = pending[:4], pending[4:]
-        n = len(chunk)
-        WS = (ctypes.c_void_p * n)(*[q.ws.data_ptr() for q in chunk])
-        OUT = (ctypes.c_void_p * n)(*[q.out.data_ptr() for q in chunk])
-        LD = (ctypes.c_int64 * n)(*[q.out_ld for q in chunk])
-        MM = (ctypes.c_int64 * n)(*[q.M for q in chunk])
-        NN = (ctypes.c_int64 * n)(*[q.N for q in chunk])
-        RR = (ctypes.c_int64 * n)(*[q.R for q in chunk])
-        SC = (ctypes.c_float * n)(*[q.scale for q in chunk])
-        TR = (ctypes.c_int * n)(*[q.transpose_out for q in chunk])
-        AC = (ctypes.c_int * n)(*[q.accumulate for q in chunk])
-        SG = (ctypes.c_void_p * n)(*[ctypes.cast(q.segs, ctypes.c_void_p).value if q.segs is not None else None for q in chunk])
-        NS = (ctypes.c_int * n)(*[q.n_segs for q in chunk])
-        L.check(_lib().llx_skinny_tn_reduce_many(n, WS, OUT, LD, MM, NN, RR, SC, TR, AC, SG, NS, L.stream()), "llx_skinny_tn_reduce_many")
+        chunk, pending[:] = pending[:cap], pending[cap:]
+        first = [q for q in chunk if isinstance(q, TnQueued) and q.u is not None]
+        for i in range(0, len(first), TN_FIRST_MAX):
+            _tn_first_many(first[i : i + TN_FIRST_MAX])
+        prods = [q for q in chunk if isinstance(q, TnQueued)]
+        sums = [q for q in chunk if isinstance(q, ColsumQueued)]
+        n, nc = len(prods), len(sums)
+        arr = lambda ctype, vals, k: (ctype * max(k, 1))(*vals)
+        L.check(_lib().llx_skinny_tn_reduce_many_cs(
+            n, arr(ctypes.c_void_p, [q.ws.data_ptr() for q in prods], n), arr(ctypes.c_void_p, [q.out.data_ptr() for q in prods], n),
+            arr(ctypes.c_int64, [q.out_ld for q in prods], n), arr(ctypes.c_int64, [q.M for q in prods], n), arr(ctypes.c_int64, [q.N for q in prods], n),
+            arr(ctypes.c_int64, [q.R for q in prods], n), arr(ctypes.c_float, [q.scale for q in prods], n), arr(ctypes.c_int, [q.transpose_out for q in prods], n),
+            arr(ctypes.c_int, [q.accumulate for q in prods], n),
+            arr(ctypes.c_void_p, [ctypes.cast(q.segs, ctypes.c_void_p).value if q.segs is not None else None for q in prods], n),
+            arr(ctypes.c_int, [q.n_segs for q in prods], n),
+            nc, arr(ctypes.c_void_p, [q.ws.data_ptr() for q in sums], nc), arr(ctypes.c_void_p, [q.out.data_ptr() for q in sums], nc),
+            arr(ctypes.c_int64, [q.nparts for q in sums], nc), arr(ctypes.c_int64, [q.dim for q in sums], nc), arr(ctypes.c_int, [q.accumulate for q in sums], nc),
+            L.stream()), "llx_skinny_tn_reduce_many")
diff --git a/llama-x_amd/llx/ops.py b/llama-x_amd/llx/ops.py
--- a/llama-x_amd/llx/ops.py
+++ b/llama-x_amd/llx/ops.py
@@ -107,7 +107,8 @@
         return y, t
 
     def backward(self, dy: Tensor, x: Tensor, t: Optional[Tensor], needs: Sequence[bool], need_dx: bool = True,
-                 dx_out: Optional[Tensor] = None, dx_accum: bool = False):
+                 dx_out: Optional[Tensor] = None, dx_accum: bool = False, pending: Optional[list] = None):
+        tail = pending if isinstance(pending, K.TailQueue) else None
         grads: list[Optional[Tensor]] = []
         ni = iter(needs)
         u = None
@@ -130,12 +131,16 @@
                 ga = _grad_dst([self.lora_a], (self.rank, self.K))
                 if ga is None:
                     ga = torch.empty(self.rank, self.K, device=dy.device, dtype=BF16)
-                K.skinny_tn(u, x, self.rank, self.scale, ga, transpose_out=False)
+                    K.skinny_tn(u, x, self.rank, self.scale, ga, transpose_out=False)
+                else:
+                    K.skinny_tn(u, x, self.rank, self.scale, ga, transpose_out=False, pending=tail, defer=tail is not None)
             if need_b:
                 gb = _grad_dst([self.lora_b], (self.N, self.rank))
                 if gb is None:
                     gb = torch.empty(self.N, self.rank, device=dy.device, dtype=BF16)
-                K.skinny_tn(t, dy, self.rank, self.scale, gb, transpose_out=True)
+                    K.skinny_tn(t, dy, self.rank, self.scale, gb, transpose_out=True)
+                else:
+                    K.skinny_tn(t, dy, self.rank, self.scale, gb, transpose_out=True, pending=tail, defer=tail is not None)
             grads += [ga, gb]
         if self.dora_m is not None:
             grads.append(gm)
@@ -345,6 +350,7 @@
                 flat = _grad_dst([m.lora_b for m in self.members if m.rank > 0])
                 if flat is None:
                     flat = torch.empty(sum((b - a) * (d - c_) for a, b, c_, d in segs), device=dy.device, dtype=BF16)
+                    _tail_must_flush(pending)
                 sc = None
                 if self.int8 and need_dx:
                     g_scaled = torch.empty_like(dy)
@@ -369,7 +375,8 @@
                 gA = _grad_dst([m.lora_a for m in self.members if m.rank > 0], (self.R, self.K))
                 if gA is None:
                     gA = torch.empty(self.R, self.K, device=dy.device, dtype=BF16)
-                K.skinny_tn(u, x, self.R, self.scale, gA, transpose_out=False, pending=pending)
+                    _tail_must_flush(pending)
+                K.skinny_tn(u, x, self.R, self.scale, gA, transpose_out=False, pending=pending, defer=isinstance(pending, K.TailQueue))
         dx = None
         if need_dx:
             if self.int8:
@@ -404,6 +411,8 @@
     g0 = first = end = None
     for p in params:
         slot = getattr(p, "_llx_slot", None)
+        if slot is not None and getattr(p, "_llx_claimed", False):
+            tail_flush()
         if slot is None or p.grad is not None or getattr(p, "_llx_claimed", False):
             return None
         G, off, n = slot
@@ -420,6 +429,45 @@
     return out.view(shape) if shape is not None else out
 
 
+_TAIL_DEFER = True
+_TAIL = K.TailQueue()
+_TAIL_PASS = -1
+
+
+def tail_flush() -> None:
+    if _TAIL:
+        K.skinny_tn_flush(_TAIL)
+
+
+def _tail_finish() -> None:
+    global _TAIL_PASS
+    _TAIL_PASS = -1
+    tail_flush()
+
+
+def _tail_begin() -> list:
+    global _TAIL_PASS
+    if not _TAIL_DEFER:
+        return []
+    task = torch._C._current_graph_task_id()
+    if task != _TAIL_PASS:
+        tail_flush()
+        _TAIL_PASS = task
+        if task >= 0:
+            torch.autograd.Variable._execution_engine.queue_callback(_tail_finish)
+    return _TAIL
+
+
+def _tail_must_flush(pending) -> None:
+    if isinstance(pending, K.TailQueue):
+        pending.must_flush = True
+
+
+def _tail_end(pending: list, last_of_layer: bool) -> None:
+    if not isinstance(pending, K.TailQueue) or last_of_layer or pending.must_flush or _TAIL_PASS < 0:
+        K.skinny_tn_flush(pending)
+
+
 def _enc(o, flat: list):
     if isinstance(o, Tensor):
         flat.append(o)
@@ -474,12 +522,21 @@
 
 
 def _norm_epilogue(dxn: Optional[Tensor], x2: Tensor, norm_w: Optional[Tensor], rstd: Optional[Tensor], need_dnw: bool,
-                   dres: Optional[Tensor] = None, fuse_norm: bool = True):
+                   dres: Optional[Tensor] = None, fuse_norm: bool = True, pending: Optional[list] = None):
     if dxn is None:
         return None, None
     if fuse_norm:
-        return K.rmsnorm_bwd(dxn, x2, norm_w.detach(), rstd, need_dnw, dres, dw_out=_grad_dst([norm_w]))
+        dst = _grad_dst([norm_w]) if need_dnw else None
+        tail = pending if (dst is not None and isinstance(pending, K.TailQueue)) else None
+        return K.rmsnorm_bwd(dxn, x2, norm_w.detach(), rstd, need_dnw, dres, dw_out=dst, pending=tail)
     return (K.add(dxn, dres) if dres is not None else dxn), None
+
+
+def _head_norm_epilogue(dxn, x2, norm_w, rstd, need_dnw):
+    pend = _tail_begin()
+    out = _norm_epilogue(dxn, x2, norm_w, rstd, need_dnw, pending=pend)
+    _tail_end(pend, last_of_layer=False)
+    return out
 
 
 def _plans_tensors(plans: Sequence[LinearPlan]) -> tuple[list[Tensor], list[int]]:
@@ -508,7 +565,9 @@
         dy2 = K._rows2d(dy)
         needs = ctx.needs_input_grad[2:]
         x2, t = _load(ctx)
-        dx, grads = plan.backward(dy2, x2, t, needs, need_dx=ctx.needs_input_grad[0])
+        pend = _tail_begin()
+        dx, grads = plan.backward(dy2, x2, t, needs, need_dx=ctx.needs_input_grad[0], pending=pend)
+        _tail_end(pend, last_of_layer=False)
         return (dx.view(ctx.xshape) if dx is not None else None, None, *grads)
 
 
@@ -580,7 +639,7 @@
         needs = list(ctx.needs_input_grad[4:])
         n_qkv = len(meta.qkv.tensors())
         nqkv, no = needs[:n_qkv], needs[n_qkv:]
-        pend = []
+        pend = _tail_begin()
         do2, g_o = meta.wo.backward(dy2, o.view(B * S, H * hd), to, no, True, pending=pend)
         W = (H + 2 * KVH) * hd
         dqkv = torch.empty(B, S, W, device=x.device, dtype=BF16)
@@ -596,8 +655,9 @@
         need_dxn = need_dx or (meta.fuse_norm and ctx.needs_input_grad[2])
         dxn = torch.empty(B * S, D, device=x.device, dtype=BF16) if need_dxn else None
         _, g_qkv = meta.qkv.backward(d2, xn, tqkv, nqkv, need_dxn, dxn, pending=pend)
-        K.skinny_tn_flush(pend)
-        dx, dnw = _norm_epilogue(dxn, x2, norm_w, rstd, ctx.needs_input_grad[2], dy2 if (need_dx and meta.fuse_residual) else None, meta.fuse_norm)
+        dx, dnw = _norm_epilogue(dxn, x2, norm_w, rstd, ctx.needs_input_grad[2], dy2 if (need_dx and meta.fuse_residual) else None, meta.fuse_norm,
+                                 pending=pend)
+        _tail_end(pend, last_of_layer=True)
         return (dx.view(B, S, D) if (dx is not None and need_dx) else None, None, dnw, None, *g_qkv, *g_o)
 
 
@@ -645,7 +705,7 @@
         n_13 = len(meta.w13.tensors())
         n13, n2 = needs[:n_13], needs[n_13:]
         dgu = torch.empty(T, 2 * I, device=x.device, dtype=BF16)
-        pend = []
+        pend = _tail_begin()
         if meta.w2.fused:
             _, g_2 = meta.w2.backward(dy2, h, t2, n2, True, swiglu=(gu, dgu), pending=pend)
         else:
@@ -655,8 +715,9 @@
         need_dxn = need_dx or (meta.fuse_norm and ctx.needs_input_grad[1])
         dxn = torch.empty_like(x2) if need_dxn else None
         _, g_13 = meta.w13.backward(dgu, xn, t13, n13, need_dxn, dxn, pending=pend)
-        K.skinny_tn_flush(pend)
-        dx, dnw = _norm_epilogue(dxn, x2, norm_w, rstd, ctx.needs_input_grad[1], dy2 if (need_dx and meta.fuse_residual) else None, meta.fuse_norm)
+        dx, dnw = _norm_epilogue(dxn, x2, norm_w, rstd, ctx.needs_input_grad[1], dy2 if (need_dx and meta.fuse_residual) else None, meta.fuse_norm,
+                                 pending=pend)
+        _tail_end(pend, last_of_layer=False)
         return (dx.view(x.shape) if (dx is not None and need_dx) else None, dnw, None, *g_13, *g_2)
 
 
@@ -734,7 +795,7 @@
                         part = K.gemm_nt_splitk(dl, wt, _HEAD_SPLITK, m_valid=cnt_c) if split else K.gemm_nt(dl, wt, m_valid=cnt_c)
                         dxc[r0 : r0 + dl.shape[0]].copy_(part)
                     dxn = K.scatter_rows(dxc, inv, g32) if inv is not None else K.scale(dxc, dev_scalar=g32)
-                    dx, dnw = _norm_epilogue(dxn, x2, norm_w, rstd, ctx.needs_input_grad[1])
+                    dx, dnw = _head_norm_epilogue(dxn, x2, norm_w, rstd, ctx.needs_input_grad[1])
                 return (dx.view(x.shape) if dx is not None else None, dnw, None, None, None, *([None] * len(needs)))
             inv, cnt = t if ctx.compact else (None, None)
             dx = dnw = None
@@ -746,7 +807,7 @@
                     dxn = K.scatter_rows(K.gemm_nt(dlogits, wt, m_valid=cnt, m_expect=ctx.m_expect), inv, g32)
                 else:
                     dxn = K.scale(K.gemm_nt(dlogits, wt), dev_scalar=g32)
-                dx, dnw = _norm_epilogue(dxn, x2, norm_w, rstd, ctx.needs_input_grad[1])
+                dx, dnw = _head_norm_epilogue(dxn, x2, norm_w, rstd, ctx.needs_input_grad[1])
             gw = None
             if ctx.plain_trainable:
                 gw = K.scale(K.gemm_tn(dlogits, xn, m_valid=cnt, m_expect=ctx.m_expect), dev_scalar=g32)
@@ -755,5 +816,5 @@
         grads = [None if g is None else K.scale(g, dev_scalar=g32) for g in grads]
         if dxn is not None:
             K.scale(dxn, dev_scalar=g32, out=dxn)
-        dx, dnw = _norm_epilogue(dxn, x2, norm_w, rstd, ctx.needs_input_grad[1])
+        dx, dnw = _head_norm_epilogue(dxn, x2, norm_w, rstd, ctx.needs_input_grad[1])
         return (dx.view(x.shape) if dx is not None else None, dnw, None, None, None, *grads)
```

Result: no change. 32140 tokens/s, median of 6 (+0.4%).
